# YaqiXia/Voltrix-SpMM

Hardware: AMD Instinct MI355X
Metric: spmm_gflops (higher is better)
Workload: dtype f16

## Files before the change

### include/voltrix_capi.h

```cpp
#ifndef VOLTRIX_CAPI_H_
#define VOLTRIX_CAPI_H_

#include <stdint.h>

#ifdef __cplusplus
extern "C" {
#endif

#define VOLTRIX_ABI_VERSION 2

#define VOLTRIX_CSR_AUTO (-1)
#define VOLTRIX_SLAB_AUTO (-1)
#define VOLTRIX_BLK_H 16
#define VOLTRIX_BLK_W 8

enum voltrix_rc {
  VOLTRIX_OK = 0,
  VOLTRIX_ERR_BAD_SHAPE = 1,
  VOLTRIX_ERR_LAUNCH = 2,
  VOLTRIX_ERR_BAD_CONFIG = 3,
  VOLTRIX_ERR_OVERFLOW = 4,
  VOLTRIX_ERR_DUPLICATE = 5
};

// ... 18 lines not shown
                                  int embedding_dim, void* input, void* output, int fs, int depth, int waves,
                                  void* window_order, void* out_scale, void* stream, int* return_code);

void voltrix_launch_spmm_f16(void* blk_offsets, void* hspa_packed, void* hind, int num_nodes, int num_edges,
                             int embedding_dim, void* input, void* output, void* stream, int* return_code);
void voltrix_launch_spmm_f16_tile(void* blk_offsets, void* hspa_packed, void* hind, int num_nodes, int num_edges,
                                  int embedding_dim, void* input, void* output, int fs, int depth, int waves,
                                  void* window_order, void* out_scale, void* stream, int* return_code);

int64_t voltrix_spmm_f32_workspace_bytes(int64_t input_rows, int embedding_dim);
void voltrix_launch_spmm_f32_as_f16(void* blk_offsets, void* hspa_packed, void* hind, int num_nodes, int num_edges,
                                    int embedding_dim, void* input, int64_t input_rows, void* output, void* workspace,
                                    void* stream, int* return_code);

void voltrix_launch_spmm_bf16(void* blk_offsets, void* hspa_packed, void* hind, int num_nodes, int num_edges,
                              int embedding_dim, void* input, void* output, void* stream, int* return_code);
void voltrix_launch_spmm_bf16_tile(void* blk_offsets, void* hspa_packed, void* hind, int num_nodes, int num_edges,
                                   int embedding_dim, void* input, void* output, int fs, int depth, int waves,
                                   void* window_order, void* out_scale, void* stream, int* return_code);

void voltrix_launch_spmm_f16_sched(void* blk_offsets, void* hspa_packed, void* hind, int num_nodes, int num_edges,
                                   int embedding_dim, void* input, void* output, int fs, int depth, int waves,
                                   void* window_order, void* out_scale, int atomic_out, void* units, void* unit_ptr,
                                   int max_units_per_xcd, void* partials, void* row_map, int units_per_wave, void* stream,
                                   int* return_code);
void voltrix_launch_spmm_bf16_sched(void* blk_offsets, void* hspa_packed, void* hind, int num_nodes, int num_edges,
                                    int embedding_dim, void* input, void* output, int fs, int depth, int waves,
                                    void* window_order, void* out_scale, int atomic_out, void* units, void* unit_ptr,
                                    int max_units_per_xcd, void* partials, void* row_map, int units_per_wave, void* stream,
                                    int* return_code);
void voltrix_launch_combine_partials(void* cuts, int num_cuts, void* partials, void* output, int num_nodes,
                                     int embedding_dim, int accumulate, void* row_map, void* stream, int* return_code);

int64_t voltrix_unit_table_workspace_bytes(int num_nodes);
int64_t voltrix_unit_table_fill_workspace_bytes(int64_t num_units);
void voltrix_launch_unit_table_count(void* blk_offsets, int num_nodes, int max_stages, void* xcd_ptr, void* workspace,
                                     void* header, void* stream, int* return_code);
void voltrix_launch_unit_table_fill(void* blk_offsets, int num_nodes, void* xcd_ptr, void* workspace, void* fill_workspace,
                                    int num_units, int num_cuts, int top, void* units, void* unit_ptr, void* cuts,
                                    void* stream, int* return_code);

int64_t voltrix_stream_table_workspace_bytes(int num_nodes);
int64_t voltrix_stream_table_fill_workspace_bytes(int64_t num_units);
void voltrix_launch_stream_table_count(void* blk_offsets, void* hspa_packed, void* hind, int num_nodes, int run_cost,
                                       int cut_stages, void* workspace, void* header, void* stream, int* return_code);
void voltrix_launch_stream_table_fill(void* blk_offsets, int num_nodes, void* workspace, void* fill_workspace, int num_units,
                                      int num_cuts, int run_bound, int run_cost, void* units, void* cuts, void* runs,
                                      void* run_ptr, void* header2, void* stream, int* return_code);
void voltrix_launch_spmm_stream_f16(void* hspa_packed, void* hind, int num_nodes, int embedding_dim, void* input,
                                    int64_t input_rows, void* output, void* units, void* runs, void* run_ptr,
                                    int max_runs_per_xcd, void* partials, void* out_scale, int fs, int depth, int waves,
                                    int slab_policy, void* stream, int* return_code);
void voltrix_launch_spmm_stream_bf16(void* hspa_packed, void* hind, int num_nodes, int embedding_dim, void* input,
                                     int64_t input_rows, void* output, void* units, void* runs, void* run_ptr,
                                     int max_runs_per_xcd, void* partials, void* out_scale, int fs, int depth, int waves,
                                     int slab_policy, void* stream, int* return_code);

void voltrix_launch_window_order(void* blk_offsets, int num_nodes, int chunk, void* order_out, void* stream,
                                 int* return_code);

#define VOLTRIX_PANEL_KSTEPS_PIPELINED 17
void voltrix_launch_spmm_panel_f16(void* panel_ptr, void* panel_cols, void* panel_bits, void* panel_order, void* xcd_ptr,
                                   int max_panels_per_xcd, int num_nodes, int embedding_dim, void* input, int64_t input_rows, void* output,
                                   int accumulate, int fs, int depth, int waves, int row_blocks, int ksteps,
                                   int slab_policy, void* out_scale, void* stream, int* return_code);
void voltrix_launch_spmm_panel_bf16(void* panel_ptr, void* panel_cols, void* panel_bits, void* panel_order, void* xcd_ptr,
                                    int max_panels_per_xcd, int num_nodes, int embedding_dim, void* input, int64_t input_rows, void* output,
                                    int accumulate, int fs, int depth, int waves, int row_blocks, int ksteps,
                                    int slab_policy, void* out_scale, void* stream, int* return_code);

void voltrix_launch_spmm_panel_parts_f16(void* panel_ptr, void* panel_cols, void* panel_bits, void* parts, int num_parts,
                                         void* xcd_ptr, int max_parts_per_xcd, void* partials, int num_nodes, int embedding_dim,
                                         void* input, int64_t input_rows, void* output, int accumulate, int fs, int depth,
                                         int waves, int row_blocks, int ksteps, int slab_policy, void* out_scale, void* stream,
                                         int* return_code);
void voltrix_launch_spmm_panel_parts_bf16(void* panel_ptr, void* panel_cols, void* panel_bits, void* parts, int num_parts,
                                          void* xcd_ptr, int max_parts_per_xcd, void* partials, int num_nodes, int embedding_dim,
                                          void* input, int64_t input_rows, void* output, int accumulate, int fs, int depth,
                                          int waves, int row_blocks, int ksteps, int slab_policy, void* out_scale, void* stream,
                                          int* return_code);
void voltrix_launch_combine_panel_partials(void* cuts, int num_cuts, void* partials, void* output, int num_nodes,
                                           int embedding_dim, int panel_rows, int accumulate, void* stream, int* return_code);

void voltrix_launch_xcd_ranges_of_work(void* work, int num_items, int align, void* xcd_ptr, void* stream, int* return_code);
void voltrix_launch_xcd_ranges_of_windows(void* blk_offsets, int num_nodes, int align, void* xcd_ptr, void* stream,
                                          int* return_code);
void voltrix_launch_xcd_ranges_of_panels(void* panel_ptr, void* resid_blk_offsets, int num_nodes, int panel_rows,
                                         int kstep_cost_x10, void* xcd_ptr, void* window_xcd_ptr, void* stream,
                                         int* return_code);
int64_t voltrix_panel_parts_workspace_bytes(int num_panels);
void voltrix_launch_panel_parts_count(void* panel_ptr, int num_panels, int cap, void* panel_xcd_ptr, void* workspace,
                                      void* header, void* stream, int* return_code);
void voltrix_launch_panel_parts_fill(void* panel_ptr, int num_panels, int cap, void* panel_xcd_ptr, void* workspace,
                                     void* parts, void* part_xcd_ptr, void* cuts, void* stream, int* return_code);

void voltrix_launch_spmm_fused_f16(void* panel_ptr, void* panel_cols, void* panel_bits, void* panel_order, void* xcd_ptr,
                                   int max_panels_per_xcd, void* wave_ptr, void* records, int num_nodes, int embedding_dim, void* input,
                                   void* output, int fs, int depth, int pace_blocks, void* out_scale, void* stream,
                                   int* return_code);
void voltrix_launch_spmm_fused_bf16(void* panel_ptr, void* panel_cols, void* panel_bits, void* panel_order, void* xcd_ptr,
                                    int max_panels_per_xcd, void* wave_ptr, void* records, int num_nodes, int embedding_dim, void* input,
                                    void* output, int fs, int depth, int pace_blocks, void* out_scale, void* stream,
                                   int* return_code);

void voltrix_fused_panel_geometry(int* waves, int* row_blocks);
int64_t voltrix_fused_records_workspace_bytes(int num_nodes);
void voltrix_launch_fused_records_count(void* blk_offsets, void* hspa_packed, int num_nodes, void* workspace, void* wave_ptr,
                                        void* stream, int* return_code);
void voltrix_launch_fused_records_fill(void* blk_offsets, void* hspa_packed, void* hind, int num_nodes, void* wave_ptr,
                                       int64_t num_records, void* records, void* stream, int* return_code);

int64_t voltrix_panel_plan_workspace_bytes(int num_nodes, int waves, int row_blocks);
void voltrix_launch_panel_plan_count(void* node_pointer, void* edge_list, int num_nodes, int num_cols, int64_t num_edges,
                                     int waves, int row_blocks, int tau, void* workspace, void* panel_ptr,
                                     void* resid_node_pointer, void* status, void* stream, int* return_code);
void voltrix_launch_panel_plan_fill(void* node_pointer, void* edge_list, int num_nodes, int num_cols, int64_t num_edges,
                                    int waves, int row_blocks, int tau, void* workspace, void* panel_ptr,
                                    void* resid_node_pointer, int64_t total_ksteps, void* resid_edge_list,
                                    void* panel_cols, void* panel_bits, void* stream, int* return_code);

void voltrix_launch_panel_order(void* panel_ptr, int num_panels, int group, void* xcd_ptr, void* order_out, void* stream,
                                int* return_code);

void voltrix_spmm_default_tile(int embedding_dim, int is_f16, int* fs, int* depth, int* waves);

int voltrix_spmm_num_tiles(int is_f16);
void voltrix_spmm_tile_at(int is_f16, int index, int* fs, int* depth, int* waves);

void voltrix_launch_cast_f32_f16(void* src, void* dst, int64_t count, void* stream, int* return_code);

void voltrix_launch_cast_f32_f16_scaled(void* src, void* dst, int64_t count, void* scale, void* stream,
                                        int* return_code);

void voltrix_launch_spmm_csr_rows(void* indptr, void* indices, int num_rows, int embedding_dim, void* input, int dtype, void* output,
                                  int xcd_ranges, void* stream, int* return_code);

void voltrix_launch_spmm_csr_rows_weighted(void* indptr, void* indices, void* values, int num_rows, int embedding_dim, void* input, int dtype,
                                           void* output, int xcd_ranges, void* stream, int* return_code);

void voltrix_launch_scatter_values(void* values, void* slots, void* plane, int64_t count, int dtype, void* stream, int* return_code);

void voltrix_launch_sddmm_csr(void* indptr, void* indices, int num_rows, int64_t nnz, int embedding_dim, void* x, int x_dtype, void* y,
                              int y_dtype, void* out, void* stream, int* return_code);

int64_t voltrix_edge_softmax_workspace_bytes(int num_rows, int64_t nnz);
void voltrix_launch_edge_softmax_csr(void* indptr, int num_rows, int64_t nnz, void* scores, float scale, void* out, void* workspace,
                                     void* stream, int* return_code);

void voltrix_launch_edge_softmax_backward_csr(void* indptr, int num_rows, int64_t nnz, void* alpha, void* grad_alpha, float scale,
                                              void* grad_scores, void* workspace, void* stream, int* return_code);

void voltrix_launch_sddmm_heads_csr(void* indptr, void* indices, int num_rows, int64_t nnz, int heads, int head_dim, void* x, int x_dtype,
                                    void* y, int y_dtype, void* out, void* stream, int* return_code);

int64_t voltrix_edge_softmax_heads_workspace_bytes(int num_rows, int64_t nnz, int heads);
void voltrix_launch_edge_softmax_heads_csr(void* indptr, int num_rows, int64_t nnz, int heads, void* scores, float scale, void* out,
                                           void* workspace, void* stream, int* return_code);
void voltrix_launch_edge_softmax_heads_backward_csr(void* indptr, int num_rows, int64_t nnz, int heads, void* alpha, void* grad_alpha,
                                                    float scale, void* grad_scores, void* workspace, void* stream, int* return_code);

void voltrix_launch_spmm_csr_heads(void* indptr, void* indices, void* values, int num_rows, int heads, int head_dim, void* input,
                                   int dtype, void* output, void* stream, int* return_code);

void voltrix_launch_gat_score_csr(void* indptr, void* indices, int num_rows, int64_t nnz, int heads, void* el, void* er, float slope,
                                  void* out, void* stream, int* return_code);

// ... 99 lines not shown
```

### voltrix-spmm_amd/csrc/capi_common.hpp

```cpp
#pragma once

#include <hip/hip_runtime.h>

#include "voltrix/spmm_kernels.hpp"
#include "voltrix_capi.h"

namespace voltrix_capi {

template <int FS, int D, int W, int EB>
constexpr bool tile_ok() {
  const int stage = 32 * FS * EB;
  const int wave_lds = D * stage + (2 * D + 1) * 256;
  return (long long)W * wave_lds <= 160 * 1024 && (1 + stage / 1024) * (D - 1) <= 63 && !(EB == 4 && FS == 256);
}

struct TileId {
  int fs, depth, waves;
};

#define VOLTRIX_TILE_SPACE(X)                                                                          \
  X(32, 2, 1) X(32, 2, 2) X(32, 2, 4) X(32, 3, 1) X(32, 3, 2) X(32, 3, 4) X(32, 4, 1) X(32, 4, 2) X(32, 4, 4)       \
  X(64, 2, 1) X(64, 2, 2) X(64, 2, 4) X(64, 3, 1) X(64, 3, 2) X(64, 3, 4) X(64, 4, 1) X(64, 4, 2) X(64, 4, 4)       \
  X(128, 2, 1) X(128, 2, 2) X(128, 2, 4) X(128, 3, 1) X(128, 3, 2) X(128, 3, 4) X(128, 4, 1) X(128, 4, 2) X(128, 4, 4) \
  X(256, 2, 1) X(256, 2, 2) X(256, 2, 4) X(256, 3, 1) X(256, 3, 2) X(256, 3, 4) X(256, 4, 1) X(256, 4, 2) X(256, 4, 4) \
  X(32, 2, 8) X(32, 3, 8) X(32, 4, 8) X(64, 2, 8) X(64, 3, 8) X(64, 4, 8) X(128, 2, 8) X(128, 3, 8) X(128, 4, 8)

template <int EB>
inline int num_tiles() {
  int n = 0;
#define X(FS, D, W) n += tile_ok<FS, D, W, EB>() ? 1 : 0;
  VOLTRIX_TILE_SPACE(X)
#undef X
  return n;
}

template <int EB>
inline bool tile_at(int index, TileId* out) {
  int n = 0;
#define X(FS, D, W)                      \
  if (tile_ok<FS, D, W, EB>()) {         \
    if (n == index) {                    \
      *out = TileId{FS, D, W};           \
      return true;                       \
    }                                    \
    ++n;                                 \
  }
  VOLTRIX_TILE_SPACE(X)
#undef X
  return false;
}

template <int FS, int D, int W, int EB, class In, bool BF16 = false>
inline int launch_if_ok(const int* blk_offsets, const uint32_t* hspa_packed, const int* hind, int num_nodes,
                        int embedding_dim, const In* input, float* output, hipStream_t stream, const int* order,
                        const float* out_scale, int atomic_out, const int* units, const int* unit_ptr,
                        int max_units_per_xcd, float* partials, const int* row_map, int units_per_wave) {
  if constexpr (tile_ok<FS, D, W, EB>()) {
    return voltrix::launch_spmm_tc16<voltrix::SpmmTile<FS, D, W, EB, BF16>>(blk_offsets, hspa_packed, hind, num_nodes,
                                                                       embedding_dim, input, output, stream, order,
                                                                       out_scale, atomic_out, units, unit_ptr,
                                                                       max_units_per_xcd, partials, row_map, nullptr,
                                                                       units_per_wave);
  } else {
    return voltrix::kErrBadConfig;
  }
}

template <int EB, class In, bool BF16 = false>
inline int dispatch_spmm(int fs, int depth, int waves, const int* blk_offsets, const uint32_t* hspa_packed,
                         const int* hind, int num_nodes, int embedding_dim, const In* input, float* output,
                         hipStream_t stream, const int* order, const float* out_scale = nullptr,
                         int atomic_out = 0, const int* units = nullptr, const int* unit_ptr = nullptr,
                         int max_units_per_xcd = 0, float* partials = nullptr, const int* row_map = nullptr,
                         int units_per_wave = 1) {
#define X(FS, D, W)                                  \
  if (fs == FS && depth == D && waves == W)          \
    return launch_if_ok<FS, D, W, EB, In, BF16>(blk_offsets, hspa_packed, hind, num_nodes, embedding_dim, input, output, stream, order, out_scale, atomic_out, units, unit_ptr, max_units_per_xcd, partials, row_map, units_per_wave);
  VOLTRIX_TILE_SPACE(X)
#undef X
  return voltrix::kErrBadConfig;
}

inline TileId default_tile(int embedding_dim, bool is_f16) {
  TileId t;
  if (is_f16) {
    t.fs = embedding_dim <= 32 ? 32 : (embedding_dim <= 64 ? 64 : 128);
    t.depth = t.fs == 32 ? 4 : 3;
    t.waves = 4;
  } else {
    t.fs = embedding_dim <= 32 ? 32 : 64;
    t.depth = 3;
    t.waves = 1;
  }
  return t;
}

}
```

### voltrix-spmm_amd/csrc/capi_spmm_bf16.hip

```cpp
#include "capi_common.hpp"

using namespace voltrix_capi;

extern "C" {

void voltrix_launch_spmm_bf16_tile(void* blk_offsets, void* hspa_packed, void* hind, int num_nodes, int num_edges,
                                   int embedding_dim, void* input, void* output, int fs, int depth, int waves,
                                   void* window_order, void* out_scale, void* stream, int* return_code) {
  (void)num_edges;
  *return_code = dispatch_spmm<2, voltrix::bfloat16_bits, true>(
      fs, depth, waves, static_cast<const int*>(blk_offsets), static_cast<const uint32_t*>(hspa_packed),
      static_cast<const int*>(hind), num_nodes, embedding_dim, static_cast<const voltrix::bfloat16_bits*>(input),
      static_cast<float*>(output), static_cast<hipStream_t>(stream), static_cast<const int*>(window_order),
      static_cast<const float*>(out_scale));
}

void voltrix_launch_spmm_bf16_sched(void* blk_offsets, void* hspa_packed, void* hind, int num_nodes, int num_edges,
                                    int embedding_dim, void* input, void* output, int fs, int depth, int waves,
                                    void* window_order, void* out_scale, int atomic_out,
                                    void* units, void* unit_ptr, int max_units_per_xcd, void* partials, void* row_map,
                                   int units_per_wave, void* stream,
                                    int* return_code) {
  (void)num_edges;
  *return_code = dispatch_spmm<2, voltrix::bfloat16_bits, true>(
      fs, depth, waves, static_cast<const int*>(blk_offsets), static_cast<const uint32_t*>(hspa_packed),
      static_cast<const int*>(hind), num_nodes, embedding_dim, static_cast<const voltrix::bfloat16_bits*>(input),
      static_cast<float*>(output), static_cast<hipStream_t>(stream), static_cast<const int*>(window_order),
      static_cast<const float*>(out_scale), atomic_out,
                                            static_cast<const int*>(units), static_cast<const int*>(unit_ptr),
                                            max_units_per_xcd, static_cast<float*>(partials), static_cast<const int*>(row_map),
                                            units_per_wave);
}

void voltrix_launch_spmm_bf16(void* blk_offsets, void* hspa_packed, void* hind, int num_nodes, int num_edges,
                              int embedding_dim, void* input, void* output, void* stream, int* return_code) {
  const TileId t = default_tile(embedding_dim, true);
  voltrix_launch_spmm_bf16_tile(blk_offsets, hspa_packed, hind, num_nodes, num_edges, embedding_dim, input, output,
                                t.fs, t.depth, t.waves, nullptr, nullptr, stream, return_code);
}

}
```

### voltrix-spmm_amd/csrc/capi_spmm_f16.hip

```cpp
#include "capi_common.hpp"

using namespace voltrix_capi;

extern "C" {

void voltrix_launch_spmm_f16_tile(void* blk_offsets, void* hspa_packed, void* hind, int num_nodes, int num_edges,
                                  int embedding_dim, void* input, void* output, int fs, int depth, int waves,
                                  void* window_order, void* out_scale, void* stream, int* return_code) {
  (void)num_edges;
  *return_code = dispatch_spmm<2, _Float16>(fs, depth, waves, static_cast<const int*>(blk_offsets),
                                            static_cast<const uint32_t*>(hspa_packed), static_cast<const int*>(hind),
                                            num_nodes, embedding_dim, static_cast<const _Float16*>(input),
                                            static_cast<float*>(output), static_cast<hipStream_t>(stream),
                                            static_cast<const int*>(window_order),
                                            static_cast<const float*>(out_scale));
}

void voltrix_launch_spmm_f16_sched(void* blk_offsets, void* hspa_packed, void* hind, int num_nodes, int num_edges,
                                   int embedding_dim, void* input, void* output, int fs, int depth, int waves,
                                   void* window_order, void* out_scale, int atomic_out,
                                   void* units, void* unit_ptr, int max_units_per_xcd, void* partials, void* row_map,
                                   int units_per_wave, void* stream,
                                   int* return_code) {
  (void)num_edges;
  *return_code = dispatch_spmm<2, _Float16>(fs, depth, waves, static_cast<const int*>(blk_offsets),
                                            static_cast<const uint32_t*>(hspa_packed), static_cast<const int*>(hind),
                                            num_nodes, embedding_dim, static_cast<const _Float16*>(input),
                                            static_cast<float*>(output), static_cast<hipStream_t>(stream),
                                            static_cast<const int*>(window_order),
                                            static_cast<const float*>(out_scale), atomic_out,
                                            static_cast<const int*>(units), static_cast<const int*>(unit_ptr),
                                            max_units_per_xcd, static_cast<float*>(partials), static_cast<const int*>(row_map),
                                            units_per_wave);
}

void voltrix_launch_combine_partials(void* cuts, int num_cuts, void* partials, void* output, int num_nodes,
                                     int embedding_dim, int accumulate, void* row_map, void* stream, int* return_code) {
  *return_code = voltrix::combine_partials(static_cast<const int*>(cuts), num_cuts, static_cast<const float*>(partials),
                                           static_cast<float*>(output), num_nodes, embedding_dim, accumulate,
                                           static_cast<hipStream_t>(stream), static_cast<const int*>(row_map));
}

void voltrix_launch_spmm_f16(void* blk_offsets, void* hspa_packed, void* hind, int num_nodes, int num_edges,
                             int embedding_dim, void* input, void* output, void* stream, int* return_code) {
  const TileId t = default_tile(embedding_dim, true);
  voltrix_launch_spmm_f16_tile(blk_offsets, hspa_packed, hind, num_nodes, num_edges, embedding_dim, input, output, t.fs,
                               t.depth, t.waves, nullptr, nullptr, stream, return_code);
}

int64_t voltrix_spmm_f32_workspace_bytes(int64_t input_rows, int embedding_dim) {
  if (input_rows < 0 || embedding_dim < 0) return -1;
  return 16 + input_rows * (int64_t)embedding_dim * 2;
}

void voltrix_launch_spmm_f32_as_f16(void* blk_offsets, void* hspa_packed, void* hind, int num_nodes, int num_edges,
                                    int embedding_dim, void* input, int64_t input_rows, void* output, void* workspace,
                                    void* stream, int* return_code) {
  if (input_rows < 0 || workspace == nullptr || ((uintptr_t)workspace & 15) || embedding_dim % 8 != 0) {
    *return_code = voltrix::kErrBadShape;
    return;
  }
  float* const scale = static_cast<float*>(workspace);
  _Float16* const operand = reinterpret_cast<_Float16*>(static_cast<char*>(workspace) + 16);
  *return_code = voltrix::cast_f32_to_f16_scaled(static_cast<const float*>(input), operand,
                                                 input_rows * (int64_t)embedding_dim, scale,
                                                 static_cast<hipStream_t>(stream));
  if (*return_code != voltrix::kOk) return;
  const TileId t = default_tile(embedding_dim, true);
  voltrix_launch_spmm_f16_tile(blk_offsets, hspa_packed, hind, num_nodes, num_edges, embedding_dim, operand, output, t.fs,
                               t.depth, t.waves, nullptr, scale, stream, return_code);
}

void voltrix_launch_window_order(void* blk_offsets, int num_nodes, int chunk, void* order_out, void* stream,
                                 int* return_code) {
  *return_code = voltrix::launch_window_order(static_cast<const int*>(blk_offsets), num_nodes, chunk,
                                              static_cast<int*>(order_out), static_cast<hipStream_t>(stream));
}

void voltrix_launch_cast_f32_f16(void* src, void* dst, int64_t count, void* stream, int* return_code) {
  *return_code = voltrix::cast_f32_to_f16(static_cast<const float*>(src), static_cast<_Float16*>(dst), count,
                                          static_cast<hipStream_t>(stream));
}

void voltrix_launch_cast_f32_f16_scaled(void* src, void* dst, int64_t count, void* scale, void* stream,
                                        int* return_code) {
  *return_code = voltrix::cast_f32_to_f16_scaled(static_cast<const float*>(src), static_cast<_Float16*>(dst), count,
                                                 static_cast<float*>(scale), static_cast<hipStream_t>(stream));
}

void voltrix_launch_scale_rows(void* src, void* scale, void* dst, int64_t rows, int num_feats, int dtype, void* stream,
                               int* return_code) {
  *return_code = voltrix::scale_rows(src, static_cast<const float*>(scale), dst, rows, num_feats, dtype,
                                     static_cast<hipStream_t>(stream));
}

}

namespace voltrix_capi {
int num_tiles_f16() { return num_tiles<2>(); }
bool tile_at_f16(int i, TileId* t) { return tile_at<2>(i, t); }
}
```

### voltrix-spmm_amd/csrc/capi_spmm_panel.hip

```cpp
#include <hip/hip_runtime.h>

#include "voltrix/panel_plan.hpp"
#include "voltrix/spmm_panel_kernels.hpp"
#include "voltrix_capi.h"

namespace {

#define VOLTRIX_PANEL_SPACE(X)                                                                       \
  X(128, 3, 8, 4, 1) X(128, 4, 8, 4, 1) X(128, 6, 8, 4, 1) X(128, 8, 8, 4, 1) X(128, 4, 4, 4, 1) X(128, 6, 4, 4, 1) X(128, 8, 4, 4, 1) \
  X(128, 4, 8, 2, 1) X(128, 6, 8, 2, 1) X(128, 8, 8, 2, 1) X(128, 6, 4, 2, 1)                                    \
  X(64, 4, 4, 4, 1) X(64, 6, 4, 4, 1) X(64, 4, 8, 4, 2) X(64, 6, 8, 4, 2) X(64, 6, 4, 4, 2)                      \
  X(32, 4, 4, 4, 2) X(32, 6, 4, 4, 2) X(32, 6, 8, 4, 2) X(64, 6, 4, 2, 2) X(64, 6, 8, 2, 2) X(32, 6, 4, 2, 2) X(32, 6, 8, 2, 2) \
  X(128, 3, 4, 4, 1) X(128, 4, 4, 2, 1)

constexpr int kPipelined = 17;
static_assert(kPipelined == VOLTRIX_PANEL_KSTEPS_PIPELINED, "include/voltrix_capi.h");
#define VOLTRIX_PANEL_PIPE_SPACE(X) X(128, 3, 8, 4) X(128, 4, 8, 4) X(128, 4, 8, 2) X(128, 6, 8, 2) X(64, 4, 8, 4) X(64, 6, 8, 4)

template <bool BF16>
int dispatch(int fs, int depth, int waves, int rb, int ks, const int* panel_ptr, const int* panel_cols,
             const uint32_t* panel_bits, const int* panel_order, int num_nodes, int embedding_dim, const void* input,
             float* output, int accumulate, const float* out_scale, hipStream_t stream, int64_t input_rows,
             int slab_policy, const int* xcd_ptr, int max_panels_per_xcd, const int* parts = nullptr, int num_parts = 0,
             float* partials = nullptr) {
#define X(FS, D, W, RB, KS)                                                                                          \
  if (fs == FS && depth == D && waves == W && rb == RB && ks == KS)                                                  \
    return voltrix::launch_spmm_panel<voltrix::PanelTile<FS, D, W, RB, KS, BF16>>(                                   \
        panel_ptr, panel_cols, panel_bits, panel_order, num_nodes, embedding_dim, input, output, accumulate, out_scale, \
        stream, 0, 0, input_rows, slab_policy, xcd_ptr, max_panels_per_xcd, parts, num_parts, partials);
  VOLTRIX_PANEL_SPACE(X)
#undef X
#define X(FS, D, W, RB)                                                                                              \
  if (fs == FS && depth == D && waves == W && rb == RB && ks == kPipelined)                                           \
    return voltrix::launch_spmm_panel<voltrix::PanelTile<FS, D, W, RB, 1, BF16, true>>(                               \
        panel_ptr, panel_cols, panel_bits, panel_order, num_nodes, embedding_dim, input, output, accumulate, out_scale, \
        stream, 0, 0, input_rows, slab_policy, xcd_ptr, max_panels_per_xcd, parts, num_parts, partials);
  VOLTRIX_PANEL_PIPE_SPACE(X)
#undef X
  return voltrix::kErrBadConfig;
}

}

extern "C" {

void voltrix_launch_spmm_panel_f16(void* panel_ptr, void* panel_cols, void* panel_bits, void* panel_order, void* xcd_ptr,
                                   int max_panels_per_xcd, int num_nodes, int embedding_dim, void* input, int64_t input_rows, void* output,
                                   int accumulate, int fs, int depth, int waves, int row_blocks, int ksteps,
                                   int slab_policy, void* out_scale, void* stream, int* return_code) {
  *return_code = dispatch<false>(fs, depth, waves, row_blocks, ksteps, static_cast<const int*>(panel_ptr),
                                 static_cast<const int*>(panel_cols), static_cast<const uint32_t*>(panel_bits),
                                 static_cast<const int*>(panel_order), num_nodes, embedding_dim, input,
                                 static_cast<float*>(output), accumulate, static_cast<const float*>(out_scale),
                                 static_cast<hipStream_t>(stream), input_rows, slab_policy,
                                 static_cast<const int*>(xcd_ptr), max_panels_per_xcd);
}

void voltrix_launch_spmm_panel_bf16(void* panel_ptr, void* panel_cols, void* panel_bits, void* panel_order, void* xcd_ptr,
                                    int max_panels_per_xcd, int num_nodes, int embedding_dim, void* input, int64_t input_rows, void* output,
                                    int accumulate, int fs, int depth, int waves, int row_blocks, int ksteps,
                                    int slab_policy, void* out_scale, void* stream, int* return_code) {
  *return_code = dispatch<true>(fs, depth, waves, row_blocks, ksteps, static_cast<const int*>(panel_ptr),
                                static_cast<const int*>(panel_cols), static_cast<const uint32_t*>(panel_bits),
                                static_cast<const int*>(panel_order), num_nodes, embedding_dim, input,
                                static_cast<float*>(output), accumulate, static_cast<const float*>(out_scale),
                                static_cast<hipStream_t>(stream), input_rows, slab_policy,
                                static_cast<const int*>(xcd_ptr), max_panels_per_xcd);
}

void voltrix_launch_spmm_panel_parts_f16(void* panel_ptr, void* panel_cols, void* panel_bits, void* parts, int num_parts,
                                         void* xcd_ptr, int max_parts_per_xcd, void* partials, int num_nodes, int embedding_dim,
                                         void* input, int64_t input_rows, void* output, int accumulate, int fs, int depth,
                                         int waves, int row_blocks, int ksteps, int slab_policy, void* out_scale, void* stream,
                                         int* return_code) {
  *return_code = parts == nullptr ? voltrix::kErrBadShape
                                  : dispatch<false>(fs, depth, waves, row_blocks, ksteps, static_cast<const int*>(panel_ptr),
                                                    static_cast<const int*>(panel_cols), static_cast<const uint32_t*>(panel_bits),
                                                    nullptr, num_nodes, embedding_dim, input, static_cast<float*>(output),
                                                    accumulate, static_cast<const float*>(out_scale),
                                                    static_cast<hipStream_t>(stream), input_rows, slab_policy,
                                                    static_cast<const int*>(xcd_ptr), max_parts_per_xcd,
                                                    static_cast<const int*>(parts), num_parts, static_cast<float*>(partials));
}

void voltrix_launch_spmm_panel_parts_bf16(void* panel_ptr, void* panel_cols, void* panel_bits, void* parts, int num_parts,
                                          void* xcd_ptr, int max_parts_per_xcd, void* partials, int num_nodes, int embedding_dim,
                                          void* input, int64_t input_rows, void* output, int accumulate, int fs, int depth,
                                          int waves, int row_blocks, int ksteps, int slab_policy, void* out_scale, void* stream,
                                          int* return_code) {
  *return_code = parts == nullptr ? voltrix::kErrBadShape
                                  : dispatch<true>(fs, depth, waves, row_blocks, ksteps, static_cast<const int*>(panel_ptr),
                                                   static_cast<const int*>(panel_cols), static_cast<const uint32_t*>(panel_bits),
                                                   nullptr, num_nodes, embedding_dim, input, static_cast<float*>(output),
                                                   accumulate, static_cast<const float*>(out_scale),
                                                   static_cast<hipStream_t>(stream), input_rows, slab_policy,
                                                   static_cast<const int*>(xcd_ptr), max_parts_per_xcd,
                                                   static_cast<const int*>(parts), num_parts, static_cast<float*>(partials));
}

void voltrix_launch_combine_panel_partials(void* cuts, int num_cuts, void* partials, void* output, int num_nodes,
                                           int embedding_dim, int panel_rows, int accumulate, void* stream, int* return_code) {
  *return_code = voltrix::launch_combine_panel_partials(static_cast<const int*>(cuts), num_cuts,
                                                        static_cast<const float*>(partials), static_cast<float*>(output),
                                                        num_nodes, embedding_dim, panel_rows, accumulate,
                                                        static_cast<hipStream_t>(stream));
}

void voltrix_launch_panel_order(void* panel_ptr, int num_panels, int group, void* xcd_ptr, void* order_out, void* stream,
                                int* return_code) {
  *return_code = voltrix::panel_order(static_cast<const int*>(panel_ptr), num_panels, group, static_cast<int*>(order_out),
                                      static_cast<hipStream_t>(stream), static_cast<const int*>(xcd_ptr));
}

int64_t voltrix_panel_plan_workspace_bytes(int num_nodes, int waves, int row_blocks) {
  return voltrix::panel_plan_workspace_bytes(num_nodes, waves, row_blocks);
}

void voltrix_launch_panel_plan_count(void* node_pointer, void* edge_list, int num_nodes, int num_cols, int64_t num_edges,
                                     int waves, int row_blocks, int tau, void* workspace, void* panel_ptr,
                                     void* resid_node_pointer, void* status, void* stream, int* return_code) {
  *return_code = voltrix::panel_plan_count(static_cast<const int*>(node_pointer), static_cast<const int*>(edge_list),
                                           num_nodes, num_cols, num_edges, waves, row_blocks, tau, workspace,
                                           static_cast<int*>(panel_ptr), static_cast<int*>(resid_node_pointer),
                                           static_cast<int*>(status), static_cast<hipStream_t>(stream));
}

void voltrix_launch_panel_plan_fill(void* node_pointer, void* edge_list, int num_nodes, int num_cols, int64_t num_edges,
                                    int waves, int row_blocks, int tau, void* workspace, void* panel_ptr,
                                    void* resid_node_pointer, int64_t total_ksteps, void* resid_edge_list,
                                    void* panel_cols, void* panel_bits, void* stream, int* return_code) {
  *return_code = voltrix::panel_plan_fill(static_cast<const int*>(node_pointer), static_cast<const int*>(edge_list),
                                          num_nodes, num_cols, num_edges, waves, row_blocks, tau, workspace,
                                          static_cast<const int*>(panel_ptr), static_cast<const int*>(resid_node_pointer),
                                          total_ksteps, static_cast<int*>(resid_edge_list), static_cast<int*>(panel_cols),
                                          static_cast<uint32_t*>(panel_bits), static_cast<hipStream_t>(stream));
}

}
```

### voltrix-spmm_amd/voltrix/capi.py

```python
from __future__ import annotations

import ctypes
import os
import subprocess

_PKG = os.path.dirname(os.path.abspath(__file__))
_ROOT = os.path.dirname(_PKG)
LIB_PATH = os.path.join(_ROOT, "lib", "libvoltrix_hip.so")
CSRC_DIR = os.path.join(_ROOT, "csrc")

_lib = None

_P, _I, _L, _F, _D, _RC_P = ctypes.c_void_p, ctypes.c_int, ctypes.c_int64, ctypes.c_float, ctypes.c_double, ctypes.POINTER(ctypes.c_int)
_U32, _U64 = ctypes.c_uint32, ctypes.c_uint64
SIGNATURES = {
    "voltrix_abi_version": (_I, []),
    "voltrix_launch_preprocess": (None, [_P, _P, _I, _P, _P, _P, _P, _RC_P]),
    "voltrix_launch_hmat_gen": (None, [_P, _P, _P, _P, _P, _P, _I, _I, _I, _P, _P, _RC_P]),
    "voltrix_launch_hmat_packed_swizzle": (None, [_I, _P, _P, _P, _RC_P]),
    "voltrix_launch_spmm": (None, [_P, _P, _P, _I, _I, _I, _P, _P, _P, _RC_P]),
    "voltrix_launch_spmm_f32_tile": (None, [_P, _P, _P, _I, _I, _I, _P, _P, _I, _I, _I, _P, _P, _P, _RC_P]),
    "voltrix_launch_spmm_f16": (None, [_P, _P, _P, _I, _I, _I, _P, _P, _P, _RC_P]),
    "voltrix_launch_spmm_f16_tile": (None, [_P, _P, _P, _I, _I, _I, _P, _P, _I, _I, _I, _P, _P, _P, _RC_P]),
    "voltrix_spmm_f32_workspace_bytes": (_L, [_L, _I]),
    "voltrix_launch_spmm_f32_as_f16": (None, [_P, _P, _P, _I, _I, _I, _P, _L, _P, _P, _P, _RC_P]),
    "voltrix_launch_spmm_f16_sched": (None, [_P, _P, _P, _I, _I, _I, _P, _P, _I, _I, _I, _P, _P, _I, _P, _P, _I, _P, _P, _I, _P, _RC_P]),
    "voltrix_launch_spmm_bf16_sched": (None, [_P, _P, _P, _I, _I, _I, _P, _P, _I, _I, _I, _P, _P, _I, _P, _P, _I, _P, _P, _I, _P, _RC_P]),
    "voltrix_launch_combine_partials": (None, [_P, _I, _P, _P, _I, _I, _I, _P, _P, _RC_P]),
    "voltrix_stream_table_workspace_bytes": (_L, [_I]),
    "voltrix_stream_table_fill_workspace_bytes": (_L, [_L]),
    "voltrix_launch_stream_table_count": (None, [_P, _P, _P, _I, _I, _I, _P, _P, _P, _RC_P]),
    "voltrix_launch_stream_table_fill": (None, [_P, _I, _P, _P, _I, _I, _I, _I, _P, _P, _P, _P, _P, _P, _RC_P]),
    "voltrix_launch_spmm_stream_f16": (None, [_P, _P, _I, _I, _P, _L, _P, _P, _P, _P, _I, _P, _P, _I, _I, _I, _I, _P, _RC_P]),
    "voltrix_launch_spmm_stream_bf16": (None, [_P, _P, _I, _I, _P, _L, _P, _P, _P, _P, _I, _P, _P, _I, _I, _I, _I, _P, _RC_P]),
    "voltrix_launch_spmm_panel_f16": (None, [_P, _P, _P, _P, _P, _I, _I, _I, _P, _L, _P, _I, _I, _I, _I, _I, _I, _I, _P, _P, _RC_P]),
    "voltrix_launch_spmm_panel_bf16": (None, [_P, _P, _P, _P, _P, _I, _I, _I, _P, _L, _P, _I, _I, _I, _I, _I, _I, _I, _P, _P, _RC_P]),
    "voltrix_launch_spmm_panel_parts_f16": (None, [_P, _P, _P, _P, _I, _P, _I, _P, _I, _I, _P, _L, _P, _I, _I, _I, _I, _I, _I, _I, _P, _P, _RC_P]),
    "voltrix_launch_spmm_panel_parts_bf16": (None, [_P, _P, _P, _P, _I, _P, _I, _P, _I, _I, _P, _L, _P, _I, _I, _I, _I, _I, _I, _I, _P, _P, _RC_P]),
    "voltrix_launch_combine_panel_partials": (None, [_P, _I, _P, _P, _I, _I, _I, _I, _P, _RC_P]),
    "voltrix_launch_xcd_ranges_of_work": (None, [_P, _I, _I, _P, _P, _RC_P]),
    "voltrix_launch_xcd_ranges_of_windows": (None, [_P, _I, _I, _P, _P, _RC_P]),
    "voltrix_launch_xcd_ranges_of_panels": (None, [_P, _P, _I, _I, _I, _P, _P, _P, _RC_P]),
    "voltrix_panel_parts_workspace_bytes": (_L, [_I]),
    "voltrix_launch_panel_parts_count": (None, [_P, _I, _I, _P, _P, _P, _P, _RC_P]),
    "voltrix_launch_panel_parts_fill": (None, [_P, _I, _I, _P, _P, _P, _P, _P, _P, _RC_P]),
    "voltrix_launch_spmm_fused_f16": (None, [_P, _P, _P, _P, _P, _I, _P, _P, _I, _I, _P, _P, _I, _I, _I, _P, _P, _RC_P]),
    "voltrix_launch_spmm_fused_bf16": (None, [_P, _P, _P, _P, _P, _I, _P, _P, _I, _I, _P, _P, _I, _I, _I, _P, _P, _RC_P]),
    "voltrix_fused_panel_geometry": (None, [_RC_P, _RC_P]),
    "voltrix_fused_records_workspace_bytes": (_L, [_I]),
    "voltrix_launch_fused_records_count": (None, [_P, _P, _I, _P, _P, _P, _RC_P]),
    "voltrix_launch_fused_records_fill": (None, [_P, _P, _P, _I, _P, _L, _P, _P, _RC_P]),
    "voltrix_panel_plan_workspace_bytes": (_L, [_I, _I, _I]),
    "voltrix_launch_panel_plan_count": (None, [_P, _P, _I, _I, _L, _I, _I, _I, _P, _P, _P, _P, _P, _RC_P]),
    "voltrix_launch_panel_plan_fill": (None, [_P, _P, _I, _I, _L, _I, _I, _I, _P, _P, _P, _L, _P, _P, _P, _P, _RC_P]),
    "voltrix_launch_panel_order": (None, [_P, _I, _I, _P, _P, _P, _RC_P]),
    "voltrix_spmm_default_tile": (None, [_I, _I, _RC_P, _RC_P, _RC_P]),
    "voltrix_spmm_num_tiles": (_I, [_I]),
    "voltrix_spmm_tile_at": (None, [_I, _I, _RC_P, _RC_P, _RC_P]),
    "voltrix_launch_window_order": (None, [_P, _I, _I, _P, _P, _RC_P]),
    "voltrix_launch_spmm_bf16": (None, [_P, _P, _P, _I, _I, _I, _P, _P, _P, _RC_P]),
    "voltrix_launch_spmm_bf16_tile": (None, [_P, _P, _P, _I, _I, _I, _P, _P, _I, _I, _I, _P, _P, _P, _RC_P]),
    "voltrix_launch_cast_f32_f16": (None, [_P, _P, _L, _P, _RC_P]),
    "voltrix_launch_cast_f32_f16_scaled": (None, [_P, _P, _L, _P, _P, _RC_P]),
    "voltrix_launch_scale_rows": (None, [_P, _P, _P, _L, _I, _I, _P, _RC_P]),
    "voltrix_launch_spmm_csr_rows": (None, [_P, _P, _I, _I, _P, _I, _P, _I, _P, _RC_P]),
    "voltrix_launch_spmm_csr_rows_weighted": (None, [_P, _P, _P, _I, _I, _P, _I, _P, _I, _P, _RC_P]),
    "voltrix_launch_scatter_values": (None, [_P, _P, _P, _L, _I, _P, _RC_P]),
    "voltrix_launch_sddmm_csr": (None, [_P, _P, _I, _L, _I, _P, _I, _P, _I, _P, _P, _RC_P]),
    "voltrix_edge_softmax_workspace_bytes": (_L, [_I, _L]),
    "voltrix_launch_edge_softmax_csr": (None, [_P, _I, _L, _P, _F, _P, _P, _P, _RC_P]),
    "voltrix_launch_edge_softmax_backward_csr": (None, [_P, _I, _L, _P, _P, _F, _P, _P, _P, _RC_P]),
    "voltrix_launch_sddmm_heads_csr": (None, [_P, _P, _I, _L, _I, _I, _P, _I, _P, _I, _P, _P, _RC_P]),
    "voltrix_edge_softmax_heads_workspace_bytes": (_L, [_I, _L, _I]),
    "voltrix_launch_edge_softmax_heads_csr": (None, [_P, _I, _L, _I, _P, _F, _P, _P, _P, _RC_P]),
    "voltrix_launch_edge_softmax_heads_backward_csr": (None, [_P, _I, _L, _I, _P, _P, _F, _P, _P, _P, _RC_P]),
    "voltrix_launch_spmm_csr_heads": (None, [_P, _P, _P, _I, _I, _I, _P, _I, _P, _P, _RC_P]),
    "voltrix_launch_gat_score_csr": (None, [_P, _P, _I, _L, _I, _P, _P, _F, _P, _P, _RC_P]),
    "voltrix_gat_score_workspace_bytes": (_L, [_I, _L, _I]),
    "voltrix_launch_gat_score_rowsum_csr": (None, [_P, _P, _P, _I, _L, _I, _P, _P, _P, _F, _P, _P, _P, _RC_P]),
    "voltrix_launch_gatv2_score_csr": (None, [_P, _P, _I, _L, _I, _I, _P, _P, _I, _P, _F, _P, _P, _RC_P]),
    "voltrix_launch_gatv2_rowsum_csr": (None, [_P, _P, _P, _I, _L, _I, _I, _P, _P, _I, _P, _F, _P, _P, _RC_P]),
    "voltrix_launch_attn_aggregate_csr": (None, [_P, _P, _P, _I, _L, _I, _I, _P, _I, _F, _P, _P, _P, _P, _RC_P]),
    "voltrix_launch_attn_aggregate_grad_scores_csr": (None, [_P, _P, _I, _L, _I, _I, _P, _P, _I, _P, _P, _P, _P, _F, _P, _P, _RC_P]),
    "voltrix_launch_attn_aggregate_grad_feat_csr": (None, [_P, _P, _P, _I, _L, _I, _I, _P, _I, _P, _P, _P, _F, _P, _P, _RC_P]),
    "voltrix_launch_dropout_mask": (None, [_L, _I, _U32, _U64, _U64, _P, _P, _RC_P]),
    "voltrix_launch_attn_aggregate_dropout_csr": (None, [_P, _P, _P, _I, _L, _I, _I, _P, _I, _F, _P, _P, _P, _P, _F, _P, _RC_P]),
    "voltrix_launch_attn_aggregate_dropout_grad_scores_csr": (None, [_P, _P, _I, _L, _I, _I, _P, _P, _I, _P, _P, _P, _P, _F, _P, _P, _F, _P, _RC_P]),
    "voltrix_launch_attn_aggregate_dropout_grad_feat_csr": (None, [_P, _P, _P, _I, _L, _I, _I, _P, _I, _P, _P, _P, _F, _P, _P, _F, _P, _RC_P]),
    "voltrix_launch_spmm_csr_reduce": (None, [_P, _P, _I, _I, _P, _I, _I, _P, _P, _P, _RC_P]),
    "voltrix_launch_spmm_csr_reduce_backward": (None, [_P, _P, _P, _I, _L, _I, _P, _P, _P, _P, _RC_P]),
    "voltrix_launch_sample_neighbors": (None, [_P, _P, _I, _P, _I, _P, _L, _I, _I, _U64, _U64, _P, _P, _P, _RC_P]),
    "voltrix_launch_block_mark": (None, [_P, _L, _I, _P, _P, _RC_P]),
    "voltrix_launch_block_mark_seeds": (None, [_P, _I, _I, _P, _P, _RC_P]),
    "voltrix_launch_block_relabel": (None, [_P, _L, _P, _I, _P, _P, _I, _I, _P, _P, _P, _RC_P]),
    "voltrix_launch_subgraph_count": (None, [_P, _P, _I, _P, _I, _P, _I, _I, _P, _P, _RC_P]),
    "voltrix_launch_subgraph_fill": (None, [_P, _P, _I, _P, _I, _P, _I, _I, _P, _L, _P, _P, _P, _RC_P]),
    "voltrix_launch_random_walk": (None, [_P, _P, _I, _P, _I, _I, _U64, _U64, _P, _P, _I, _P, _RC_P]),
    "voltrix_launch_negative_sample": (None, [_P, _P, _I, _I, _L, _P, _I, _I, _I, _I, _I, _U64, _U64, _P, _P, _RC_P]),
    "voltrix_launch_edge_endpoints": (None, [_P, _P, _I, _L, _P, _I, _P, _P, _P, _RC_P]),
    "voltrix_csr_preprocess_workspace_bytes": (_L, [_I, _I, _L, _I]),
    "voltrix_launch_csr_window_count": (None, [_P, _P, _I, _I, _L, _I, _P, _P, _P, _P, _P, _RC_P]),
    "voltrix_launch_csr_fill": (None, [_P, _P, _I, _I, _L, _I, _P, _P, _P, _P, _P, _RC_P]),
    "voltrix_unit_table_workspace_bytes": (_L, [_I]),
    "voltrix_unit_table_fill_workspace_bytes": (_L, [_L]),
    "voltrix_launch_unit_table_count": (None, [_P, _I, _I, _P, _P, _P, _P, _RC_P]),
    "voltrix_launch_unit_table_fill": (None, [_P, _I, _P, _P, _P, _I, _I, _I, _P, _P, _P, _P, _RC_P]),
    "voltrix_csr_transpose_workspace_bytes": (_L, [_L]),
    "voltrix_launch_csr_transpose": (None, [_P, _P, _I, _I, _L, _P, _P, _P, _P, _RC_P]),
    "voltrix_launch_bfs_seed": (None, [_I, _I, _P, _P, _P, _P, _P, _RC_P]),
    "voltrix_launch_bfs_levels": (None, [_P, _P, _P, _P, _I, _I, _P, _P, _P, _P, _I, _P, _RC_P]),
    "voltrix_cm_rank_workspace_bytes": (_L, [_L]),
    "voltrix_launch_cm_rank": (None, [_P, _P, _P, _P, _I, _I, _P, _P, _P, _P, _P, _RC_P, _I, _I, _P, _P, _RC_P]),
    "voltrix_launch_chol_inv_transposed": (None, [_P, _I, _D, _P, _P, _RC_P]),
}
SYMBOLS = tuple(SIGNATURES)


def build(force: bool = False) -> str:
    cmd = ["make", "-s", "-C", CSRC_DIR, "-j4"]
    if force:
        subprocess.check_call(["make", "-s", "-C", CSRC_DIR, "clean"])
    subprocess.check_call(cmd)
# ... 62 lines not shown
    import torch

    global _CODES
    if _CODES is None:
        _CODES = {torch.float32: 0, torch.float16: 1, torch.bfloat16: 2}
    return _CODES[dtype]


def _timed(label: str):
    import functools
    import inspect

    def decorate(fn):
        stream_index = list(inspect.signature(fn).parameters).index("stream")

        @functools.wraps(fn)
        def wrapper(*args, **kwargs):
            from .utils import KernelTimer

            if KernelTimer.active is None:
                return fn(*args, **kwargs)
            stream = kwargs.get("stream")
            if stream is None and len(args) > stream_index:
                stream = args[stream_index]
            with KernelTimer.active.bracket(label, stream):
                return fn(*args, **kwargs)

        wrapper.timer_label, wrapper.stream_index = label, stream_index
        return wrapper

    return decorate


def default_tile(embedding_dim: int, is_f16: bool):
    fs, d, w = ctypes.c_int(), ctypes.c_int(), ctypes.c_int()
    lib().voltrix_spmm_default_tile(embedding_dim, int(is_f16), fs, d, w)
    return fs.value, d.value, w.value


def tiles(is_f16: bool):
    out = []
    for i in range(lib().voltrix_spmm_num_tiles(int(is_f16))):
        fs, d, w = ctypes.c_int(), ctypes.c_int(), ctypes.c_int()
        lib().voltrix_spmm_tile_at(int(is_f16), i, fs, d, w)
        out.append((fs.value, d.value, w.value))
    return out


CSR_PATHS = {None: -1, "auto": -1, "sort": 0, "bitmap": 1, "mixed": 2}
SLAB_AUTO, SLAB_ONE_GRID, SLAB_LAUNCHES = -1, 0, 1


def csr_preprocess_workspace_bytes(num_nodes: int, num_cols: int, num_edges: int, path=None) -> int:
    return int(lib().voltrix_csr_preprocess_workspace_bytes(num_nodes, num_cols, num_edges, CSR_PATHS[path]))


@_timed("csr_window_count")
def launch_csr_window_count(indptr, indices, num_nodes, num_cols, workspace, block_partition, pointer1, status,
                            stream, path=None) -> None:
    _checked("voltrix_launch_csr_window_count", indptr.data_ptr(), indices.data_ptr(), num_nodes, num_cols, indices.numel(),
             CSR_PATHS[path], workspace.data_ptr(), block_partition.data_ptr(), pointer1.data_ptr(), status.data_ptr(), stream)


@_timed("csr_fill")
def launch_csr_fill(indptr, indices, num_nodes, num_cols, workspace, pointer1, hspa_packed, hind, stream, path=None) -> None:
    _checked("voltrix_launch_csr_fill", indptr.data_ptr(), indices.data_ptr(), num_nodes, num_cols, indices.numel(), CSR_PATHS[path],
             workspace.data_ptr(), pointer1.data_ptr(), hspa_packed.data_ptr(), hind.data_ptr(), stream)


@_timed("spmm")
def launch_spmm(blk_offsets, hspa_packed, hind, num_nodes, num_edges, embedding_dim, input_ptr, output_ptr, is_f16,
                tile, stream, window_order=0, out_scale=0) -> int:
    if is_f16 == "bf16":
        name = "voltrix_launch_spmm_bf16_tile"
    else:
        name = "voltrix_launch_spmm_f16_tile" if is_f16 else "voltrix_launch_spmm_f32_tile"
    return _call(name, blk_offsets, hspa_packed, hind, num_nodes, num_edges, embedding_dim, input_ptr, output_ptr, tile[0], tile[1],
                 tile[2], window_order, out_scale, stream)


@_timed("spmm")
def launch_spmm_sched(blk_offsets, hspa_packed, hind, num_nodes, num_edges, embedding_dim, input_ptr, output_ptr, tile,
                      stream, window_order=0, out_scale=0, atomic_out=False, bf16=False, table=None, partials=0,
                      row_map=0, units_per_wave=1) -> int:
    units, unit_ptr, max_units = (table.units.data_ptr(), table.unit_ptr.data_ptr(), table.max_units_per_xcd) if table is not None \
        else (None, None, 0)
    return _call("voltrix_launch_spmm_bf16_sched" if bf16 else "voltrix_launch_spmm_f16_sched", blk_offsets, hspa_packed, hind,
                 num_nodes, num_edges, embedding_dim, input_ptr, output_ptr, tile[0], tile[1], tile[2], window_order, out_scale,
                 int(atomic_out), units, unit_ptr, max_units, partials, row_map, int(units_per_wave), stream)


@_timed("combine_partials")
def launch_combine_partials(table, partials_ptr, output_ptr, num_nodes, embedding_dim, accumulate, stream,
                            row_map=0) -> int:
    return _call("voltrix_launch_combine_partials", table.cuts.data_ptr(), table.num_cuts, partials_ptr, output_ptr, num_nodes,
                 embedding_dim, int(accumulate), row_map, stream)


def build_unit_table(blk_offsets, num_nodes: int, max_stages: int = 0, stream=None, xcd_ptr=None):
    import torch

    dev = blk_offsets.device
    stream = _stream_of(stream)
    workspace = torch.empty(max(16, int(lib().voltrix_unit_table_workspace_bytes(num_nodes))), dtype=torch.uint8, device=dev)
    header = torch.empty(8, dtype=torch.int32, device=dev)
    _checked("voltrix_launch_unit_table_count", blk_offsets.data_ptr(), num_nodes, int(max_stages), _opt(xcd_ptr),
             workspace.data_ptr(), header.data_ptr(), stream)
    head = [int(v) for v in header.tolist()]
    num_units, num_cuts, top = head[0], head[1], head[5]
    units = torch.empty((num_units, 4), dtype=torch.int32, device=dev)
    cuts = torch.empty((num_cuts, 4), dtype=torch.int32, device=dev)
    unit_ptr = torch.empty(9, dtype=torch.int32, device=dev)
    fill_ws = torch.empty(max(16, int(lib().voltrix_unit_table_fill_workspace_bytes(num_units))), dtype=torch.uint8, device=dev)
    _checked("voltrix_launch_unit_table_fill", blk_offsets.data_ptr(), num_nodes, _opt(xcd_ptr), workspace.data_ptr(),
             fill_ws.data_ptr(), num_units, num_cuts, top, units.data_ptr(), unit_ptr.data_ptr(), cuts.data_ptr(), stream)
    return units, unit_ptr, cuts, head


def build_stream_table(blk_offsets, hspa_packed, hind, num_nodes: int, run_cost: int = 0, cut_stages: int = 0, stream=None):
    import torch

    dev = blk_offsets.device
    stream = _stream_of(stream)
    workspace = torch.empty(max(16, int(lib().voltrix_stream_table_workspace_bytes(num_nodes))), dtype=torch.uint8, device=dev)
    header = torch.empty(8, dtype=torch.int32, device=dev)
    _checked("voltrix_launch_stream_table_count", blk_offsets.data_ptr(), hspa_packed.data_ptr(), hind.data_ptr(), num_nodes,
             int(run_cost), int(cut_stages), workspace.data_ptr(), header.data_ptr(), stream)
    num_units, num_cuts, num_slots, run_bound, rcost, cut = [int(v) for v in header.tolist()][:6]
    units = torch.empty((num_units, 8), dtype=torch.int32, device=dev)
    cuts = torch.empty((num_cuts, 4), dtype=torch.int32, device=dev)
    runs = torch.empty((max(1, run_bound), 4), dtype=torch.int32, device=dev)
    run_ptr = torch.empty(9, dtype=torch.int32, device=dev)
    header2 = torch.empty(4, dtype=torch.int32, device=dev)
    fill_ws = torch.empty(max(16, int(lib().voltrix_stream_table_fill_workspace_bytes(num_units))), dtype=torch.uint8, device=dev)
    _checked("voltrix_launch_stream_table_fill", blk_offsets.data_ptr(), num_nodes, workspace.data_ptr(), fill_ws.data_ptr(),
             num_units, num_cuts, run_bound, max(2, rcost), units.data_ptr(), cuts.data_ptr(), runs.data_ptr(), run_ptr.data_ptr(),
             header2.data_ptr(), stream)
    num_runs, max_runs, oversized = [int(v) for v in header2.tolist()][:3]
    assert oversized == 0, "stream table with a run of more than 64 units (run_cost > 128?): the kernel cannot walk it"
    return units, runs[:num_runs], run_ptr, cuts, (num_units, num_cuts, num_slots, num_runs, max_runs, rcost, cut)


def launch_spmm_stream(hspa_packed, hind, num_nodes: int, embedding_dim: int, feat, output, table, partials, out_scale=None,
                       tile=(0, 0, 0), stream=None, input_rows: int = 0, slab_policy: int = -1) -> int:
    import torch

    stream = _stream_of(stream)
    name = "voltrix_launch_spmm_stream_bf16" if feat.dtype == torch.bfloat16 else "voltrix_launch_spmm_stream_f16"
    from .utils import timed_launch

    with timed_launch("spmm_stream", stream):
        return _call(name, hspa_packed.data_ptr(), hind.data_ptr(), num_nodes, embedding_dim, feat.data_ptr(), int(input_rows),
                     output.data_ptr(), table.units.data_ptr(), table.runs.data_ptr(), table.run_ptr.data_ptr(),
                     table.max_runs_per_xcd, partials.data_ptr(), _opt(out_scale), tile[0], tile[1], tile[2], int(slab_policy), stream)


def xcd_ranges_of_work(work, align: int = 1, stream=None):
    import torch

    out = torch.empty(9, dtype=torch.int32, device=work.device)
    _checked("voltrix_launch_xcd_ranges_of_work", work.data_ptr(), work.numel(), int(align), out.data_ptr(), _stream_of(stream))
    return out


def xcd_ranges_of_windows(blk_offsets, num_nodes: int, align: int = 1, stream=None):
    import torch

    out = torch.empty(9, dtype=torch.int32, device=blk_offsets.device)
    _checked("voltrix_launch_xcd_ranges_of_windows", blk_offsets.data_ptr(), num_nodes, int(align), out.data_ptr(), _stream_of(stream))
    return out


def xcd_ranges_of_panels(panel_ptr, resid_blk_offsets, num_nodes: int, panel_rows: int, kstep_cost_x10: int, stream=None):
    import torch

    dev = panel_ptr.device
    out, out_w = torch.empty(9, dtype=torch.int32, device=dev), torch.empty(9, dtype=torch.int32, device=dev)
    _checked("voltrix_launch_xcd_ranges_of_panels", panel_ptr.data_ptr(), resid_blk_offsets.data_ptr(), num_nodes, panel_rows,
             int(kstep_cost_x10), out.data_ptr(), out_w.data_ptr(), _stream_of(stream))
    return out, out_w


def build_panel_parts(panel_ptr, cap: int, panel_xcd_ptr=None, stream=None):
    import torch

    dev = panel_ptr.device
    num_panels = panel_ptr.numel() - 1
    stream = _stream_of(stream)
    workspace = torch.empty(max(16, int(lib().voltrix_panel_parts_workspace_bytes(num_panels))), dtype=torch.uint8, device=dev)
    header = torch.empty(8, dtype=torch.int32, device=dev)
    _checked("voltrix_launch_panel_parts_count", panel_ptr.data_ptr(), num_panels, int(cap), _opt(panel_xcd_ptr), workspace.data_ptr(),
             header.data_ptr(), stream)
    head = [int(v) for v in header.tolist()]
    parts = torch.empty((head[0], 4), dtype=torch.int32, device=dev)
    cuts = torch.empty((max(1, head[1]), 4), dtype=torch.int32, device=dev)
    part_xcd_ptr = torch.empty(9, dtype=torch.int32, device=dev)
    _checked("voltrix_launch_panel_parts_fill", panel_ptr.data_ptr(), num_panels, int(cap), _opt(panel_xcd_ptr), workspace.data_ptr(),
             parts.data_ptr(), part_xcd_ptr.data_ptr(), cuts.data_ptr(), stream)
    return parts, part_xcd_ptr, cuts[:head[1]], head


def spmm_f32_workspace_bytes(input_rows: int, embedding_dim: int) -> int:
    return int(lib().voltrix_spmm_f32_workspace_bytes(input_rows, embedding_dim))


@_timed("spmm_f32_as_f16")
def launch_spmm_f32_as_f16(blk_offsets, hspa_packed, hind, num_nodes, num_edges, embedding_dim, feat, output, workspace,
                           stream) -> int:
    return _call("voltrix_launch_spmm_f32_as_f16", blk_offsets.data_ptr(), hspa_packed.data_ptr(), hind.data_ptr(), num_nodes,
                 num_edges, embedding_dim, feat.data_ptr(), feat.shape[0], output.data_ptr(), workspace.data_ptr(), stream)


@_timed("spmm_panel")
def launch_spmm_panel(plan, input_ptr, output_ptr, embedding_dim, accumulate, bf16, tile, out_scale, stream,
                      input_rows: int = 0, slab_policy: int = SLAB_AUTO, partials_ptr: int = 0) -> int:
    panel = (plan.panel_ptr.data_ptr(), plan.panel_cols.data_ptr(), plan.panel_bits.data_ptr())
    launch = (plan.num_nodes, embedding_dim, input_ptr, input_rows, output_ptr, int(accumulate), tile[0], tile[1], plan.waves,
              plan.row_blocks, tile[2], slab_policy, out_scale, stream)
    parts = getattr(plan, "parts", None)
    if parts is not None:
        return _call("voltrix_launch_spmm_panel_parts_bf16" if bf16 else "voltrix_launch_spmm_panel_parts_f16", *panel,
                     parts.parts.data_ptr(), parts.num_parts, parts.xcd_ptr.data_ptr(), parts.max_parts_per_xcd, partials_ptr, *launch)
    xcd_ptr = getattr(plan, "xcd_ptr", None)
    return _call("voltrix_launch_spmm_panel_bf16" if bf16 else "voltrix_launch_spmm_panel_f16", *panel, _opt(plan.panel_order),
                 _opt(xcd_ptr), plan.max_panels_per_xcd if xcd_ptr is not None else 0, *launch)


def launch_combine_panel_partials(parts, partials_ptr, output_ptr, num_nodes, embedding_dim, panel_rows, accumulate,
                                  stream) -> int:
    return _call("voltrix_launch_combine_panel_partials", parts.cuts.data_ptr(), parts.num_cuts, partials_ptr, output_ptr, num_nodes,
                 embedding_dim, panel_rows, int(accumulate), stream)


@_timed("spmm_fused")
def launch_spmm_fused(plan, fused, input_ptr, output_ptr, embedding_dim, bf16, tile, out_scale, stream,
                      pace_blocks: int = 0) -> int:
    xcd_ptr = getattr(plan, "xcd_ptr", None)
    return _call("voltrix_launch_spmm_fused_bf16" if bf16 else "voltrix_launch_spmm_fused_f16", plan.panel_ptr.data_ptr(),
                 plan.panel_cols.data_ptr(), plan.panel_bits.data_ptr(), _opt(plan.panel_order), _opt(xcd_ptr),
                 plan.max_panels_per_xcd if xcd_ptr is not None else 0, fused.wave_ptr.data_ptr(), fused.records.data_ptr(),
                 plan.num_nodes, embedding_dim, input_ptr, output_ptr, tile[0], tile[1], int(pace_blocks), out_scale, stream)


def fused_panel_geometry():
    waves, row_blocks = ctypes.c_int(0), ctypes.c_int(0)
    lib().voltrix_fused_panel_geometry(waves, row_blocks)
    assert waves.value * row_blocks.value * 16 == 512, (waves.value, row_blocks.value)
    return waves.value, row_blocks.value


def build_fused_records(blk_offsets, hspa_packed, hind, num_nodes: int, stream=None):
    import torch

    dev = blk_offsets.device
    stream = _stream_of(stream)
    num_waves = fused_panel_geometry()[0] * ((num_nodes + 511) // 512)
    workspace = torch.empty(max(16, int(lib().voltrix_fused_records_workspace_bytes(num_nodes))), dtype=torch.uint8, device=dev)
    wave_ptr = torch.empty(num_waves + 1, dtype=torch.int32, device=dev)
    _checked("voltrix_launch_fused_records_count", blk_offsets.data_ptr(), hspa_packed.data_ptr(), num_nodes, workspace.data_ptr(),
             wave_ptr.data_ptr(), stream)
    num_records = int(wave_ptr[-1])
    assert 0 <= num_records <= 4 * (hspa_packed.numel() // 16 + 1), num_records
    records = torch.empty((num_records + 1, 64), dtype=torch.int32, device=dev).view(torch.uint32)
    _checked("voltrix_launch_fused_records_fill", blk_offsets.data_ptr(), hspa_packed.data_ptr(), hind.data_ptr(), num_nodes,
             wave_ptr.data_ptr(), num_records, records.data_ptr(), stream)
    return wave_ptr, records, num_records


def launch_panel_order(panel_ptr, num_panels: int, order_out, stream, group: int = 1, xcd_ptr=None) -> None:
    _checked("voltrix_launch_panel_order", panel_ptr.data_ptr(), num_panels, group, _opt(xcd_ptr), order_out.data_ptr(), stream)


def panel_plan_workspace_bytes(num_nodes: int, waves: int, row_blocks: int) -> int:
    return int(lib().voltrix_panel_plan_workspace_bytes(num_nodes, waves, row_blocks))


def launch_panel_plan_count(indptr, indices, num_nodes, num_cols, waves, row_blocks, tau, workspace, panel_ptr,
                            resid_indptr, status, stream) -> int:
    return _call("voltrix_launch_panel_plan_count", indptr.data_ptr(), indices.data_ptr(), num_nodes, num_cols, indices.numel(), waves,
                 row_blocks, tau, workspace.data_ptr(), panel_ptr.data_ptr(), resid_indptr.data_ptr(), status.data_ptr(), stream)


def launch_panel_plan_fill(indptr, indices, num_nodes, num_cols, waves, row_blocks, tau, workspace, panel_ptr,
                           resid_indptr, total_ksteps, resid_indices, panel_cols, panel_bits, stream) -> None:
    _checked("voltrix_launch_panel_plan_fill", indptr.data_ptr(), indices.data_ptr(), num_nodes, num_cols, indices.numel(), waves,
             row_blocks, tau, workspace.data_ptr(), panel_ptr.data_ptr(), resid_indptr.data_ptr(), total_ksteps,
             resid_indices.data_ptr(), panel_cols.data_ptr(), panel_bits.data_ptr(), stream)


@_timed("window_order")
def launch_window_order(blk_offsets, num_nodes, order_out, stream, chunk: int = 256) -> None:
    _checked("voltrix_launch_window_order", blk_offsets.data_ptr(), num_nodes, chunk, order_out.data_ptr(), stream)


@_timed("cast_f32_f16")
def launch_cast_f32_f16(src, dst, stream) -> None:
    _checked("voltrix_launch_cast_f32_f16", src.data_ptr(), dst.data_ptr(), src.numel(), stream)


@_timed("cast_f32_f16_scaled")
def launch_cast_f32_f16_scaled(src, dst, scale, stream) -> None:
    _checked("voltrix_launch_cast_f32_f16_scaled", src.data_ptr(), dst.data_ptr(), src.numel(), scale.data_ptr(), stream)




@_timed("spmm_csr_rows")
def launch_spmm_csr_rows(indptr, indices, num_rows: int, feat, output, stream, xcd_ranges: int = 0, values=None) -> None:
    import torch

    assert indptr.dtype == torch.int32 and indices.dtype == torch.int32 and indptr.numel() == num_rows + 1
    assert feat.dim() == 2 and feat.is_contiguous() and output.is_contiguous() and output.dtype == torch.float32
# ... 477 lines not shown
```

### voltrix-spmm_amd/voltrix/hybrid.py

```python
from __future__ import annotations

import contextlib
import contextvars
import dataclasses
import os

import torch

from . import capi

DEFAULT_WAVES = 8
DEFAULT_ROW_BLOCKS = 4
DEFAULT_TAU = 3
KSTEP = 32
FUSED_WAVES = 4
FUSED_ROW_BLOCKS = 8


@dataclasses.dataclass
class PanelParts:
    parts: torch.Tensor
    cuts: torch.Tensor
    xcd_ptr: torch.Tensor
    max_parts_per_xcd: int
# ... 327 lines not shown
                     num_nodes=num_nodes, waves=waves, row_blocks=row_blocks, tau=tau, num_ksteps=total_ksteps,
                     num_shared_edges=indices.numel() - num_resid, num_resid_edges=num_resid)
    return resid_indptr, resid_indices, plan


def build_panel_plan_torch(indptr: torch.Tensor, indices: torch.Tensor, num_nodes: int, num_cols: int = None,
                           waves: int = DEFAULT_WAVES, row_blocks: int = DEFAULT_ROW_BLOCKS, tau: int = DEFAULT_TAU):
    assert indptr.device == indices.device and indptr.dtype == torch.int32 and indices.dtype == torch.int32
    assert waves in (4, 8) and row_blocks in (2, 4) and tau >= 1
    device = indptr.device
    num_cols = num_nodes if num_cols is None else int(num_cols)
    p = waves * row_blocks * 16
    num_panels = (num_nodes + p - 1) // p
    resid_indptr, resid_indices, pc, rp, inv = split_shared_columns(indptr, indices, num_nodes, num_cols, p, tau)

    su_panel = pc // num_cols
    su_col = pc % num_cols
    cnt = torch.bincount(su_panel, minlength=num_panels)
    nks = (cnt + KSTEP - 1) // KSTEP
    panel_ptr = torch.zeros(num_panels + 1, dtype=torch.int64, device=device)
    panel_ptr[1:] = torch.cumsum(nks, 0)
    total_ksteps = int(panel_ptr[-1].item())
    assert total_ksteps < 2 ** 26, "k-step offsets are int32 (x 32 columns)"
    col_start = torch.cumsum(cnt, 0) - cnt
    rank = torch.arange(pc.numel(), device=device, dtype=torch.int64) - col_start[su_panel]
    slot = (panel_ptr[su_panel] + rank // KSTEP) * KSTEP + rank % KSTEP

    panel_of_kstep = torch.repeat_interleave(torch.arange(num_panels, device=device), nks)
    first_col = torch.zeros(num_panels, dtype=torch.int64, device=device)
    has = cnt > 0
    first_col[has] = su_col[col_start[has]]
    panel_cols = torch.zeros(KSTEP * (total_ksteps + 2), dtype=torch.int64, device=device)
    panel_cols[:KSTEP * total_ksteps] = first_col[panel_of_kstep].repeat_interleave(KSTEP)
    panel_cols[slot] = su_col

    e_slot = slot[inv]
    k = e_slot % KSTEP
    v = rp // (16 * row_blocks)
    j = (rp % (16 * row_blocks)) // 16
    word = (e_slot // KSTEP) * (waves * 64) + v * 64 + (k // 8) * 16 + (rp % 16)
    bits = torch.zeros((total_ksteps + 1) * waves * 64, dtype=torch.int64, device=device)
    bits.index_add_(0, word, torch.ones_like(word) << (16 * (k % 2) + 4 * j + (k % 8) // 2))
    panel_bits = ((bits + 2 ** 31) % 2 ** 32 - 2 ** 31).to(torch.int32).view(torch.uint32)

    plan = PanelPlan(panel_ptr=panel_ptr.to(torch.int32), panel_cols=panel_cols.to(torch.int32), panel_bits=panel_bits,
                     panel_order=None, num_nodes=num_nodes, waves=waves, row_blocks=row_blocks, tau=tau,
                     num_ksteps=total_ksteps, num_shared_edges=int(rp.numel()),
                     num_resid_edges=int(resid_indices.numel()))
    return resid_indptr, resid_indices, plan


KSTEPS_PIPELINED = 17


def default_panel_tile(embedding_dim: int, waves: int, row_blocks: int = DEFAULT_ROW_BLOCKS):
    if embedding_dim <= 32:
        return (32, 6, 2)
    if embedding_dim <= 64:
        return (64, 6, 2)
    if waves == 8:
        return (128, 3, 1) if row_blocks == 4 else (128, 4, KSTEPS_PIPELINED)
    return (128, 4, 1)


PANEL_DOMINATED_RATIO = 2.0
PANEL_DOMINATED_ROW_BLOCKS = 2


def panel_dominated(plan: "PanelPlan") -> bool:
    resid_stages = max(1.0, plan.num_resid_edges / 32.0)
    return plan.num_ksteps * KSTEP_COST_IN_STAGES >= PANEL_DOMINATED_RATIO * resid_stages


_SIDE_STREAMS = {}


def side_stream(device) -> "torch.cuda.Stream":
    key = device.index if device.index is not None else torch.cuda.current_device()
    if key not in _SIDE_STREAMS:
        _SIDE_STREAMS[key] = torch.cuda.Stream(device=device)
    return _SIDE_STREAMS[key]


def run_two_level(plan: PanelPlan, operand: torch.Tensor, output: torch.Tensor, run_window, out_scale=None,
                  tile=None, concurrent: bool = True) -> None:
    def finish(pending):
        if pending is not None:
            pending.run()

    if plan.num_ksteps == 0:
        finish(run_window(False))
        return
    if not concurrent:
        finish(run_window(False))
        launch_panel(plan, operand, output, accumulate=1, out_scale=out_scale, tile=tile)
        return
    from .utils import timed_launch

    main = torch.cuda.current_stream()
    side = side_stream(operand.device)
    with timed_launch("zero_fill", main):
        output.zero_()
    fork = torch.cuda.Event()
    fork.record(main)
    side.wait_event(fork)
    pending_panel = launch_panel(plan, operand, output, accumulate=2, out_scale=out_scale, tile=tile,
                                 stream=side.cuda_stream, defer_combine=True)
    join = torch.cuda.Event()
    join.record(side)
    pending = run_window(True)
    main.wait_event(join)
    finish(pending)
    finish(pending_panel)


class PendingPanelCombine:

    def __init__(self, plan, partials, output, num_feats, accumulate):
        self.plan, self.partials, self.output, self.num_feats, self.accumulate = plan, partials, output, num_feats, accumulate

    def run(self, raw_stream: int = None):
        from .utils import timed_launch

        current = torch.cuda.current_stream()
        with timed_launch("combine_panel_partials", current) if raw_stream is None else contextlib.nullcontext():
            rc = capi.launch_combine_panel_partials(self.plan.parts, self.partials.data_ptr(), self.output.data_ptr(),
                                                    self.plan.num_nodes, self.num_feats, self.plan.panel_rows,
                                                    self.accumulate, current.cuda_stream if raw_stream is None else raw_stream)
        capi.check(rc, "voltrix_launch_combine_panel_partials")
        self.partials = None


def launch_panel(plan: PanelPlan, feat: torch.Tensor, output: torch.Tensor, accumulate, out_scale=None,
                 tile=None, stream=None, slab_policy: int = None, defer_combine: bool = False):
    assert feat.is_cuda and feat.is_contiguous() and feat.dtype in (torch.float16, torch.bfloat16)
    assert output.is_cuda and output.is_contiguous() and output.dtype == torch.float32
    f = feat.shape[1]
    assert output.shape == (plan.num_nodes, f)
    tile = tile or default_panel_tile(f, plan.waves, plan.row_blocks)
    assert tile is not None, f"no panel tile for F={f} with {plan.waves} waves"
    stream = torch.cuda.current_stream().cuda_stream if stream is None else stream
    if slab_policy is None:
        from .jit_kernels import spmm as _spmm_wrapper

        slab_policy = _spmm_wrapper.SLAB_POLICY
    parts = plan.parts
    partials = None
    if parts is not None and parts.num_slots > 0:
        partials = torch.empty(parts.num_slots * plan.panel_rows * f, dtype=torch.float32, device=feat.device)
    rc = capi.launch_spmm_panel(plan, feat.data_ptr(), output.data_ptr(), f, int(accumulate),
                                feat.dtype == torch.bfloat16, tile, out_scale.data_ptr() if out_scale is not None else 0,
                                stream, input_rows=feat.shape[0], slab_policy=slab_policy,
                                partials_ptr=partials.data_ptr() if partials is not None else 0)
    capi.check(rc, "voltrix_launch_spmm_panel")
    if partials is None:
        return None
    pending = PendingPanelCombine(plan, partials, output, f, 1 if int(accumulate) else 0)
    if defer_combine:
        return pending
    pending.run(None if stream == torch.cuda.current_stream().cuda_stream else stream)
    return None


def default_fused_tile(embedding_dim: int):
    if embedding_dim <= 32:
        return (32, 4)
    if embedding_dim <= 64:
        return (64, 4)
    return (128, 3)


FUSED_PACE_BLOCKS = 0


def fused_enabled() -> bool:
    return os.getenv("VOLTRIX_FUSED", "0") in ("1", "on")


def launch_fused(plan: PanelPlan, fused: FusedRecords, feat: torch.Tensor, output: torch.Tensor, out_scale=None,
                 tile=None, stream=None, pace_blocks: int = None) -> None:
    assert feat.is_cuda and feat.is_contiguous() and feat.dtype in (torch.float16, torch.bfloat16)
    assert output.is_cuda and output.is_contiguous() and output.dtype == torch.float32
    assert plan.waves == DEFAULT_WAVES and plan.row_blocks == DEFAULT_ROW_BLOCKS, "the fused kernel owns 8 x 4 x 16-row panels"
    f = feat.shape[1]
    assert output.shape == (plan.num_nodes, f)
    tile = tile or default_fused_tile(f)
    stream = torch.cuda.current_stream().cuda_stream if stream is None else stream
    pace_blocks = FUSED_PACE_BLOCKS if pace_blocks is None else pace_blocks
    rc = capi.launch_spmm_fused(plan, fused, feat.data_ptr(), output.data_ptr(), f, feat.dtype == torch.bfloat16, tile,
                                out_scale.data_ptr() if out_scale is not None else 0, stream, pace_blocks)
    capi.check(rc, "voltrix_launch_spmm_fused")


def min_shared_fraction() -> float:
    default = "0.38" if hybrid_mode() == "auto" else "0.2"
    return float(os.getenv("VOLTRIX_HYBRID_MIN_SHARE", default))


_MODE_OVERRIDE = contextvars.ContextVar("voltrix_hybrid_mode", default=None)


@contextlib.contextmanager
def mode_override(value: str):
    token = _MODE_OVERRIDE.set(value)
    try:
        yield
    finally:
        _MODE_OVERRIDE.reset(token)


def hybrid_mode() -> str:
    v = _MODE_OVERRIDE.get()
    v = os.getenv("VOLTRIX_HYBRID", "auto") if v is None else v
    if v in ("0", "", "off"):
        return "off"
    if v in ("1", "on"):
        return "on"
    return "tune" if v == "tune" else "auto"


AUTO_MIN_EDGES = 1 << 22
AUTO_MIN_MEAN_DEGREE = 64
AUTO_MIN_ROWS = 110_000


def handle_bytes(tensors) -> int:
    return int(sum(t.numel() * t.element_size() for t in tensors if isinstance(t, torch.Tensor)))


def two_level_bytes(two: "TwoLevelHandle") -> int:
    plan = two.plan
    total = handle_bytes((two.blk_offsets, two.hspa_packed, two.hind, plan.panel_ptr, plan.panel_cols, plan.panel_bits,
                          plan.panel_order))
    if two.fused is not None:
        total += two.fused.nbytes()
    return total
```

### voltrix-spmm_amd/voltrix/include/voltrix/spmm_kernels.hpp

```cpp
#pragma once

#include <hip/hip_runtime.h>

#include <cstdint>
#include <cstdlib>
#include <mutex>
#include <type_traits>
#include <utility>
#include <vector>

#include "voltrix/traits.hpp"

#ifndef VOLTRIX_DIAG
#define VOLTRIX_DIAG 0
#endif


namespace voltrix {

typedef _Float16 half8_t __attribute__((ext_vector_type(8)));
typedef __bf16 bf16x8_t __attribute__((ext_vector_type(8)));
typedef uint16_t bfloat16_bits;
typedef float float4_t __attribute__((ext_vector_type(4)));
typedef unsigned uint2_t __attribute__((ext_vector_type(2)));
// ... 85 lines not shown
               : [m] "s"(m)
               : "vcc", "scc", "memory");
  __builtin_amdgcn_sched_barrier(0);
}

__device__ __forceinline__ void wait_lgkmcnt0() {
  asm volatile("s_waitcnt lgkmcnt(0)" ::: "memory");
  __builtin_amdgcn_sched_barrier(0);
}
__device__ __forceinline__ unsigned lds_read_b32(unsigned addr) {
  unsigned v;
  asm volatile("ds_read_b32 %0, %1" : "=v"(v) : "v"(addr) : "memory");
  return v;
}
template <int OFF>
__device__ __forceinline__ unsigned lds_read_b32_off(unsigned addr) {
  unsigned v;
  asm volatile("ds_read_b32 %0, %1 offset:%2" : "=v"(v) : "v"(addr), "n"(OFF) : "memory");
  return v;
}
template <int STRIDE, int N, int... I>
__device__ __forceinline__ void lds_read_b32_strided(unsigned addr, int (&out)[N], std::integer_sequence<int, I...>) {
  ((out[I] = (int)lds_read_b32_off<STRIDE * I>(addr)), ...);
}
__device__ __forceinline__ uint2_t lds_read_b64(unsigned addr) {
  uint2_t v;
  asm volatile("ds_read_b64 %0, %1" : "=v"(v) : "v"(addr) : "memory");
  return v;
}
__device__ __forceinline__ uint4_t lds_read_b128(unsigned addr) {
  uint4_t v;
  asm volatile("ds_read_b128 %0, %1" : "=v"(v) : "v"(addr) : "memory");
  return v;
}
template <int OFF>
__device__ __forceinline__ uint2_t lds_read_tr16_b64(unsigned addr) {
  uint2_t v;
  asm volatile("ds_read_b64_tr_b16 %0, %1 offset:%2" : "=v"(v) : "v"(addr), "n"(OFF) : "memory");
  return v;
}
__device__ __forceinline__ void dma_b128(const void* src, unsigned lds_byte_addr) {
  __builtin_amdgcn_global_load_lds((gas_ptr)src, (lds_ptr)(uintptr_t)lds_byte_addr, 16, 0, 0);
}
__device__ __forceinline__ void dma_b32(const void* src, unsigned lds_byte_addr) {
  __builtin_amdgcn_global_load_lds((gas_ptr)src, (lds_ptr)(uintptr_t)lds_byte_addr, 4, 0, 0);
}
__device__ __forceinline__ void dma_b32_nt(const void* src, unsigned lds_byte_addr) {
  __builtin_amdgcn_global_load_lds((gas_ptr)src, (lds_ptr)(uintptr_t)lds_byte_addr, 4, 0, 2);
}
__device__ __forceinline__ void dma_b128_nt(const void* src, unsigned lds_byte_addr) {
  __builtin_amdgcn_global_load_lds((gas_ptr)src, (lds_ptr)(uintptr_t)lds_byte_addr, 16, 0, 2);
}

template <int SLOTS>
__device__ __forceinline__ constexpr int slot_swizzle(int r) {
  const int ident = (r & 3) | (((r >> 3) & 1) << 2);
  return SLOTS >= 8 ? ident : (SLOTS == 4 ? (ident >> 1) : (ident >> 2));
}

constexpr float kAScaleInv = 0.5f;
__device__ __forceinline__ half8_t nibbles_to_half8_x2(unsigned nl, unsigned nh) {
  unsigned zl, zh;
  asm("v_lshl_or_b32 %0, %1, 15, %1" : "=v"(zl) : "v"(nl));
  asm("v_lshl_or_b32 %0, %1, 15, %1" : "=v"(zh) : "v"(nh));
  uint4_t r;
  r[0] = (zl << 14) & 0x40004000u;
  r[1] = (zl << 12) & 0x40004000u;
  r[2] = (zh << 14) & 0x40004000u;
  r[3] = (zh << 12) & 0x40004000u;
  return __builtin_bit_cast(half8_t, r);
}

template <int OFF, int AUX = 0>
__device__ __forceinline__ void dma_b128_off(const void* src, unsigned lds_byte_addr) {
  __builtin_amdgcn_global_load_lds((gas_ptr)((const char*)src - OFF), (lds_ptr)(uintptr_t)lds_byte_addr, 16, OFF, AUX);
}

__device__ __forceinline__ float lds_read_f32(unsigned addr) {
  float v;
  asm volatile("ds_read_b32 %0, %1" : "=v"(v) : "v"(addr) : "memory");
  return v;
}

template <class Tag = void>
inline int ensure_dynamic_lds(const void* kernel, int bytes) {
  if (bytes <= 64 * 1024) return kOk;
  struct Seen { const void* k; int dev; };
  static std::mutex mu;
  static std::vector<Seen> seen;
  int dev = 0;
  if (hipGetDevice(&dev) != hipSuccess) return kErrLaunch;
  static thread_local Seen last = {nullptr, -1};
  if (last.k == kernel && last.dev == dev) return kOk;
  std::lock_guard<std::mutex> lock(mu);
  for (const Seen& s : seen)
    if (s.k == kernel && s.dev == dev) {
      last = s;
      return kOk;
    }
  if (hipFuncSetAttribute(kernel, hipFuncAttributeMaxDynamicSharedMemorySize, bytes) != hipSuccess) return kErrBadConfig;
  seen.push_back(Seen{kernel, dev});
  last = seen.back();
  return kOk;
}

template <class T>
struct SpmmArgs {
  using in_t = typename std::conditional<T::EB == 4, float,
                                         typename std::conditional<T::BF16, bfloat16_bits, _Float16>::type>::type;
  const int* blk_offsets;
  const uint32_t* hspa_packed;
  const int* hind;
  const in_t* input;
  float* output;
  int num_nodes;
  int num_windows;
  int F;
  int num_slabs;
  int windows_per_xcd;
  const int* window_order;
  const float* out_scale;
  const int4* units;
  const int* unit_ptr;
  float* partials;
  const in_t* values;
  const int* row_map;
  int slab_major;
  int slab_first;
  int meta_nt;
  int atomic_out;
};

template <int I, int N, class Fn>
__device__ __forceinline__ void static_for(Fn&& fn) {
  if constexpr (I < N) {
    fn(std::integral_constant<int, I>{});
    static_for<I + 1, N>(fn);
  }
}

template <class T, int NU>
__device__ __forceinline__ void spmm_tc16_body(const SpmmArgs<T>& a) {
  static_assert(NU == 1 || NU == 2, "units per wave");
  constexpr int FS = T::FS, D = T::DEPTH, MS = T::META_SLOTS, EB = T::EB;
  constexpr int ROW_BYTES = T::ROW_BYTES, STAGE_BYTES = T::STAGE_BYTES, NDMA = T::DMA_PER_STAGE;
  constexpr int RPD = T::ROWS_PER_DMA, LPR = T::LANES_PER_ROW, SLOTS = T::SLOTS;

  extern __shared__ __attribute__((aligned(16))) char smem[];
  const int lane = threadIdx.x & (kWave - 1);
  const int wave = __builtin_amdgcn_readfirstlane((int)(threadIdx.x / kWave));
  const unsigned long long diag_t0 = (VOLTRIX_DIAG & 8) ? __builtin_amdgcn_s_memrealtime() : 0ull;

  const int xcd = blockIdx.x % kNumXcd;
  int w_begin = xcd * a.windows_per_xcd;
  int w_count = (a.num_windows - w_begin) < a.windows_per_xcd ? (a.num_windows - w_begin) : a.windows_per_xcd;
  if (a.units) {
    w_begin = a.unit_ptr[xcd];
    w_count = a.unit_ptr[xcd + 1] - w_begin;
  }
  __builtin_amdgcn_s_setprio(3);
  const int wave_pos = (int)(blockIdx.x / kNumXcd) * T::WAVES + wave;
  const int pairs_per_slab = (w_count + 1) / 2;
  if (w_count <= 0 || (NU == 1 ? wave_pos >= w_count * a.num_slabs : wave_pos >= pairs_per_slab * a.num_slabs)) return;
  const int lu = NU == 1 ? wave_pos : (wave_pos / pairs_per_slab) * w_count + 2 * (wave_pos % pairs_per_slab);
  int w[NU], st0[NU], st_step[NU], slot[NU];
  int kb0[NU], kb1[NU], nst_u[NU], h_safe[NU];
  bool present[NU];
  int nst_max = 0;
#pragma unroll
  for (int p = 0; p < NU; ++p) {
    present[p] = NU == 1 || (lu % w_count) + p < w_count;
    const int lup = present[p] ? lu + p : lu;
    const int wpos = w_begin + ((a.slab_major || NU == 2) ? lup % w_count : lup / a.num_slabs);
    st0[p] = 0;
    st_step[p] = 1;
    slot[p] = -1;
    if (a.units) {
      const int4 u = a.units[wpos];
      w[p] = u.x;
      st0[p] = u.y;
      st_step[p] = u.z;
      slot[p] = u.w;
    } else {
      w[p] = a.window_order ? a.window_order[wpos] : wpos;
    }
    kb0[p] = a.blk_offsets[w[p]];
    kb1[p] = a.blk_offsets[w[p] + 1];
    const int nblk = kb1[p] - kb0[p];
    const int nst_window = (nblk + kTcbPerStage - 1) / kTcbPerStage;
    nst_u[p] = st0[p] < nst_window ? (nst_window - st0[p] + st_step[p] - 1) / st_step[p] : 0;
    if (nblk == 1) {
      const uint4 w4 = *reinterpret_cast<const uint4*>(a.hspa_packed + 4ll * kb0[p]);
      if ((w4.x | w4.y | w4.z | w4.w) == 0u) nst_u[p] = 0;
    }
    if (!present[p]) nst_u[p] = 0;
    h_safe[p] = a.hind[8ll * kb0[p]];
    nst_max = nst_u[p] > nst_max ? nst_u[p] : nst_max;
  }
  const int nst = NU * nst_max;
  const int fs0 = (a.slab_first + (int)((a.slab_major || NU == 2) ? lu / w_count : lu % a.num_slabs)) * FS;
  const int F = a.F;
  auto stage_of = [&](int t) -> int { return st0[t % NU] + st_step[t % NU] * (t / NU); };
  auto stage_block = [&](int t) -> int { return kb0[t % NU] + kTcbPerStage * stage_of(t); };
  auto stage_end = [&](int t) -> int { return kb1[t % NU]; };

  float4_t acc[NU][SLOTS];
#pragma unroll
  for (int p = 0; p < NU; ++p)
#pragma unroll
    for (int s = 0; s < SLOTS; ++s) acc[p][s] = float4_t{0.f, 0.f, 0.f, 0.f};

  const unsigned lds0 = (unsigned)(uintptr_t)(lds_ptr)smem + (unsigned)wave * T::WAVE_LDS;
  const unsigned meta0 = lds0 + D * STAGE_BYTES;

  if (nst > 0) {

    const int k32 = lane & 31;
    const int kblk = k32 >> 3, kcol = k32 & 7;
    const unsigned colmask = 0x11111111u << (kcol & 3);
    const unsigned vword_off = 128 + 4 * (4 * kblk + 2 * (kcol >> 2));
    const int g = lane >> 4, R = lane & 15;
    const unsigned a_shift = 4 * (R & 7);
// ... 208 lines not shown
          wlo[bm] = lds_read_b32(mt + 128 + 4 * (4 * bm + (R >> 3)));
          whi[bm] = lds_read_b32(mt + 128 + 4 * (4 * bm + 2 + (R >> 3)));
        }
        const int z = g & 1;
        const unsigned lbase = lds0 + dslot * STAGE_BYTES + g * ROW_BYTES + 4 * R;
        const unsigned base_e = lbase + 64 * z, base_o = lbase - 64 * z;
        float bv[8][SLOTS];
#pragma unroll
        for (int m = 0; m < 8; ++m) {
#pragma unroll
          for (int s = 0; s < SLOTS; ++s) {
            bv[m][s] = lds_read_f32(((s & 1) ? base_o : base_e) + (4 * m * ROW_BYTES + 64 * s));
          }
        }
        wait_lgkmcnt0();

        issue_meta(t + 2 * D, mslot_2d);
        if (more) {
          if (tail_stage) rows_from_columns(sanitise(t + D, hraw, vw), hr);
          issue_data(dslot, hr);
        }

#pragma unroll
        for (int m = 0; m < 8; ++m) {
          const int bm = m >> 1;
          unsigned word = (m & 1) ? whi[bm] : wlo[bm];
          if (stage_block(t) + bm >= kb1 || !live) word = 0u;
          const float av = ((word >> (a_shift + g)) & 1u) ? 1.0f : 0.0f;
#pragma unroll
          for (int s = 0; s < SLOTS; ++s) acc[P][s] = __builtin_amdgcn_mfma_f32_16x16x4f32(av, bv[m][s], acc[P][s], 0, 0, 0);
        }
      }

      dslot = dslot + 1 == D ? 0 : dslot + 1;
      mslot = mslot + 1 == MS ? 0 : mslot + 1;
      mslot_d = mslot_d + 1 == MS ? 0 : mslot_d + 1;
      mslot_2d = mslot_2d + 1 == MS ? 0 : mslot_2d + 1;
    };
    int t = 0;
    if constexpr (NU == 2) {
      for (; t + 1 < nst - D; t += 2) {
        wait_vmcnt<T::vm_behind(D - 1)>();
        step(t, std::true_type{}, std::integral_constant<int, 0>{});
        wait_vmcnt<T::vm_behind(D - 1)>();
        step(t + 1, std::true_type{}, std::integral_constant<int, 1>{});
      }
      if (t < nst - D) {
        wait_vmcnt<T::vm_behind(D - 1)>();
        step(t, std::true_type{}, std::integral_constant<int, 0>{});
      }
      static_for<0, D>([&](auto ic) {
        constexpr int I = decltype(ic)::value;
        if (nst - D + I >= 0) {
          wait_vmcnt<T::vm_behind(D - 1 - I)>();
          step(nst - D + I, std::false_type{}, std::integral_constant<int, (D + I) & 1>{});
        }
      });
    } else {
      for (; t < nst - D; ++t) {
        wait_vmcnt<T::vm_behind(D - 1)>();
        step(t, std::true_type{}, std::integral_constant<int, 0>{});
      }
      for (; t < nst; ++t) {
        switch (nst - 1 - t) {
          case 0: wait_vmcnt<T::vm_behind(0)>(); break;
          case 1: wait_vmcnt<T::vm_behind(1)>(); break;
          case 2: wait_vmcnt<T::vm_behind(2)>(); break;
          case 3: wait_vmcnt<T::vm_behind(3)>(); break;
          case 4: wait_vmcnt<T::vm_behind(4)>(); break;
          default: wait_vmcnt<T::vm_behind(D - 1)>(); break;
        }
        step(t, std::false_type{}, std::integral_constant<int, 0>{});
      }
    }
    wait_vmcnt<0>();
  }

  if (VOLTRIX_DIAG & 4) {
    if (acc[0][0][0] == 12345.678f) a.output[0] = acc[0][0][0];
    return;
  }
  const float oscale = ((EB == 2 && !T::WEIGHTED) ? kAScaleInv : 1.0f) * (a.out_scale ? *a.out_scale : 1.0f);
  const int ocol0 = fs0 + (lane & 15);
#pragma unroll
  for (int p = 0; p < NU; ++p) {
    if (!present[p]) continue;
    const bool dead = NU > 1 && nst_u[p] == 0;
    if (slot[p] >= 0) {
      float* const tile = a.partials + (long long)slot[p] * (kBlkH * (long long)F) + (long long)(4 * (lane >> 4)) * F;
#pragma unroll
      for (int s = 0; s < SLOTS; ++s) {
        const int col = ocol0 + 16 * s;
        if (col < F) {
#pragma unroll
          for (int j = 0; j < 4; ++j) tile[(long long)j * F + col] = dead ? 0.f : acc[p][s][j] * oscale;
        }
      }
      continue;
    }
    const int orow0 = w[p] * kBlkH + 4 * (lane >> 4);
    int orow[4];
#pragma unroll
    for (int j = 0; j < 4; ++j) {
      orow[j] = orow0 + j;
      if (a.row_map && !(VOLTRIX_DIAG & 8)) orow[j] = a.row_map[orow[j]];
      if (orow[j] >= a.num_nodes) orow[j] = -1;
    }
#pragma unroll
    for (int s = 0; s < SLOTS; ++s) {
      const int col = ocol0 + 16 * s;
      if (col < F) {
#pragma unroll
        for (int j = 0; j < 4; ++j) {
          const int row = orow[j];
          if (row >= 0) {
            float* const dst = a.output + ((long long)row * F + col);
            const float v = dead ? 0.f : acc[p][s][j] * oscale;
            if (a.atomic_out)
              unsafeAtomicAdd(dst, v);
            else
              *dst = v;
          }
        }
      }
    }
  }
  if ((VOLTRIX_DIAG & 8) && a.row_map && lane == 0) {
    int* const stamp = const_cast<int*>(a.row_map) + 4ll * ((long long)blockIdx.x * T::WAVES + wave);
    stamp[0] = (int)__builtin_amdgcn_s_getreg((31 << 11) | 20);
    stamp[1] = (int)__builtin_amdgcn_s_getreg((31 << 11) | 4);
    stamp[2] = (int)(unsigned)diag_t0;
    stamp[3] = (int)(unsigned)__builtin_amdgcn_s_memrealtime();
  }
}

template <class T>
static __global__ __launch_bounds__(T::THREADS) void spmm_tc16_kernel(const SpmmArgs<T> a) {
  spmm_tc16_body<T, 1>(a);
}

template <class T>
static __global__ __launch_bounds__(T::THREADS) __attribute__((amdgpu_num_vgpr(160)))
void spmm_tc16_pair_kernel(const SpmmArgs<T> a) {
  spmm_tc16_body<T, 2>(a);
}

inline int slab_major_order(int num_slabs, int slab_row_bytes) { return num_slabs > 1 && slab_row_bytes >= 128; }

enum SlabPolicy : int { kSlabAuto = -1, kSlabOneGrid = 0, kSlabLaunches = 1 };
inline int slab_launch_group(int num_slabs, int slab_row_bytes, long long rows, int policy = kSlabAuto) {
  if (policy == kSlabOneGrid || slab_row_bytes < 128) return 0;
  if (policy == kSlabAuto && rows * 256 > (256ll << 20)) return 0;
  const int group = slab_row_bytes >= 256 ? 1 : 256 / slab_row_bytes;
  return num_slabs > group ? group : 0;
}

template <class T>
inline int launch_spmm_tc16(const int* blk_offsets, const uint32_t* hspa_packed, const int* hind, int num_nodes,
                            int embedding_dim, const void* input ,
                            float* output, hipStream_t stream, const int* window_order = nullptr,
                            const float* out_scale = nullptr, int atomic_out = 0,
                            const int* units = nullptr , const int* unit_ptr = nullptr ,
                            int max_units_per_xcd = 0, float* partials = nullptr, const int* row_map = nullptr,
                            const void* values = nullptr ,
                            int units_per_wave = 1 ,
                            int slab_first = 0, int slab_count = 0 ,
                            long long input_rows = 0 ,
                            int slab_policy = kSlabAuto) {
  if (num_nodes < 0 || embedding_dim < 0) return kErrBadShape;
  if (num_nodes == 0 || embedding_dim == 0) return kOk;
  if (embedding_dim % (16 / T::EB) != 0) return kErrBadShape;
  if (((uintptr_t)input & 15) || ((uintptr_t)hspa_packed & 15)) return kErrBadShape;
  SpmmArgs<T> a;
  a.blk_offsets = blk_offsets;
  a.hspa_packed = hspa_packed;
  a.hind = hind;
  a.input = static_cast<const typename SpmmArgs<T>::in_t*>(input);
  a.output = output;
  a.num_nodes = num_nodes;
  a.num_windows = (num_nodes + kBlkH - 1) / kBlkH;
  a.F = embedding_dim;
  const int total_slabs = (embedding_dim + T::FS - 1) / T::FS;
  if (slab_first < 0 || slab_count < 0 || slab_first + slab_count > total_slabs) return kErrBadShape;
  if (const int group = slab_count == 0 ? slab_launch_group(total_slabs, T::FS * T::EB,
                                                            input_rows > 0 ? input_rows : (long long)num_nodes, slab_policy)
                                        : 0) {
    for (int s = 0; s < total_slabs; s += group) {
      const int rc = launch_spmm_tc16<T>(blk_offsets, hspa_packed, hind, num_nodes, embedding_dim, input, output, stream,
                                         window_order, out_scale, atomic_out, units, unit_ptr, max_units_per_xcd, partials,
                                         row_map, values, units_per_wave, s, total_slabs - s < group ? total_slabs - s : group);
      if (rc != kOk) return rc;
    }
    return kOk;
  }
  a.slab_first = slab_count > 0 ? slab_first : 0;
  a.num_slabs = slab_count > 0 ? slab_count : total_slabs;
  a.windows_per_xcd = (a.num_windows + kNumXcd - 1) / kNumXcd;
  a.window_order = window_order;
  a.out_scale = out_scale;
  a.atomic_out = atomic_out;
  a.meta_nt = total_slabs == 1;
  a.slab_major = slab_major_order(a.num_slabs, T::FS * T::EB);
  a.units = reinterpret_cast<const int4*>(units);
  a.unit_ptr = unit_ptr;
  a.partials = partials;
  a.row_map = row_map;
  a.values = static_cast<const typename SpmmArgs<T>::in_t*>(values);
  if (T::WEIGHTED && (values == nullptr || ((uintptr_t)values & 15))) return kErrBadShape;
  if (units != nullptr) {
    if (unit_ptr == nullptr || max_units_per_xcd < 0 || ((uintptr_t)units & 15)) return kErrBadShape;
    if (max_units_per_xcd == 0) return kOk;
    a.windows_per_xcd = max_units_per_xcd;
  }
  if ((long long)a.windows_per_xcd * a.num_slabs > 0x3FFFFFFFll) return kErrBadShape;
  if constexpr (T::EB == 2 && !T::WEIGHTED && T::FS <= 128) {
    if (units_per_wave == 2 && units != nullptr && (a.num_slabs == 1 || a.slab_major)) {
      const long long pairs = ((long long)a.windows_per_xcd + 1) / 2 * a.num_slabs;
      const long long blocks_per_xcd = (pairs + T::WAVES - 1) / T::WAVES;
      const long long grid = blocks_per_xcd * kNumXcd;
      if (grid > 0x7FFFFFFFll) return kErrBadShape;
      const int lds_rc = ensure_dynamic_lds(reinterpret_cast<const void*>(&spmm_tc16_pair_kernel<T>), T::BLOCK_LDS);
      if (lds_rc != kOk) return lds_rc;
      hipLaunchKernelGGL(spmm_tc16_pair_kernel<T>, dim3((unsigned)grid), dim3(T::THREADS), T::BLOCK_LDS, stream, a);
      return hipGetLastError() == hipSuccess ? kOk : kErrLaunch;
    }
  }
  const long long blocks_per_xcd = ((long long)a.windows_per_xcd * a.num_slabs + T::WAVES - 1) / T::WAVES;
  const long long grid = blocks_per_xcd * kNumXcd;
  if (grid > 0x7FFFFFFFll) return kErrBadShape;
  const int lds_rc = ensure_dynamic_lds(reinterpret_cast<const void*>(&spmm_tc16_kernel<T>), T::BLOCK_LDS);
  if (lds_rc != kOk) return lds_rc;
  hipLaunchKernelGGL(spmm_tc16_kernel<T>, dim3((unsigned)grid), dim3(T::THREADS), T::BLOCK_LDS, stream, a);
  return hipGetLastError() == hipSuccess ? kOk : kErrLaunch;
}

static __global__ __launch_bounds__(256) void combine_partials_kernel(const int4* __restrict__ cuts,
                                                                     const float* __restrict__ partials,
                                                                     float* __restrict__ output, const int num_nodes,
                                                                     const int F, const int accumulate,
                                                                     const int* __restrict__ row_map) {
  const int4 c = cuts[blockIdx.x];
  const int f4 = F / 4;
  const long long tile4 = (long long)kBlkH * f4;
  const float4* src = reinterpret_cast<const float4*>(partials) + (long long)c.y * tile4;
  for (int i = threadIdx.x; i < (int)tile4; i += 256) {
    int row = c.x * kBlkH + i / f4;
    if (row_map) row = row_map[row];
    if (row < 0 || row >= num_nodes) continue;
    float4 sum = src[i];
    int u = 1;
    for (; u + 8 <= c.z; u += 8) {
      float4 p[8];
#pragma unroll
      for (int k = 0; k < 8; ++k) p[k] = src[(long long)(u + k) * tile4 + i];
#pragma unroll
      for (int k = 0; k < 8; ++k) {
        sum.x += p[k].x;
        sum.y += p[k].y;
        sum.z += p[k].z;
        sum.w += p[k].w;
      }
    }
    for (; u < c.z; ++u) {
      const float4 p = src[(long long)u * tile4 + i];
      sum.x += p.x;
      sum.y += p.y;
      sum.z += p.z;
      sum.w += p.w;
    }
    float4* const dst = reinterpret_cast<float4*>(output + (long long)row * F) + (i % f4);
    if (accumulate) {
      const float4 d = *dst;
      sum.x += d.x;
      sum.y += d.y;
      sum.z += d.z;
      sum.w += d.w;
    }
    *dst = sum;
  }
}

inline int combine_partials(const int* cuts, int num_cuts, const float* partials, float* output, int num_nodes,
                            int embedding_dim, int accumulate, hipStream_t stream, const int* row_map = nullptr) {
  if (num_cuts < 0 || num_nodes < 0 || embedding_dim < 0 || (embedding_dim % 4) != 0) return kErrBadShape;
  if (num_cuts == 0 || num_nodes == 0 || embedding_dim == 0) return kOk;
  if (((uintptr_t)cuts & 15) || ((uintptr_t)partials & 15) || ((uintptr_t)output & 15)) return kErrBadShape;
  hipLaunchKernelGGL(combine_partials_kernel, dim3((unsigned)num_cuts), dim3(256), 0, stream,
                     reinterpret_cast<const int4*>(cuts), partials, output, num_nodes, embedding_dim, accumulate, row_map);
  return hipGetLastError() == hipSuccess ? kOk : kErrLaunch;
}

constexpr int kOrderMaxChunk = 4096;

static __global__ __launch_bounds__(256) void window_order_kernel(const int* __restrict__ blk_offsets,
                                                                 const int num_windows, const int windows_per_xcd,
                                                                 const int chunk, const int chunks_per_xcd,
                                                                 int* __restrict__ order) {
  __shared__ unsigned long long keys[kOrderMaxChunk];
  const int xcd = blockIdx.x / chunks_per_xcd, c = blockIdx.x % chunks_per_xcd;
  const int x_begin = xcd * windows_per_xcd;
  const int x_end = (x_begin + windows_per_xcd < num_windows) ? x_begin + windows_per_xcd : num_windows;
  const int begin = x_begin + c * chunk;
  const int end = (begin + chunk < x_end) ? begin + chunk : x_end;
  const int n = end - begin;
  if (n <= 0) return;
  int P = 1;
  while (P < n) P <<= 1;
  for (int i = threadIdx.x; i < P; i += 256) {
    unsigned long long k = ~0ull;
    if (i < n) {
      const unsigned nblk = (unsigned)(blk_offsets[begin + i + 1] - blk_offsets[begin + i]);
      k = ((unsigned long long)(0xFFFFFFFFu - nblk) << 32) | (unsigned)i;
    }
    keys[i] = k;
  }
  __syncthreads();
  for (int k = 2; k <= P; k <<= 1) {
    for (int j = k >> 1; j > 0; j >>= 1) {
      for (int i = threadIdx.x; i < P; i += 256) {
        const int l = i ^ j;
        if (l > i) {
          const unsigned long long x = keys[i], y = keys[l];
          const bool up = (i & k) == 0;
          if ((x > y) == up) {
            keys[i] = y;
            keys[l] = x;
          }
        }
      }
      __syncthreads();
    }
  }
  for (int i = threadIdx.x; i < n; i += 256) order[begin + i] = begin + (int)(keys[i] & 0xFFFFFFFFu);
}

inline int launch_window_order(const int* blk_offsets, int num_nodes, int chunk, int* order, hipStream_t stream) {
  if (num_nodes < 0 || chunk < 1 || chunk > kOrderMaxChunk) return kErrBadShape;
  const int num_windows = (num_nodes + kBlkH - 1) / kBlkH;
  if (num_windows == 0) return kOk;
  const int windows_per_xcd = (num_windows + kNumXcd - 1) / kNumXcd;
  const int chunks_per_xcd = (windows_per_xcd + chunk - 1) / chunk;
  hipLaunchKernelGGL(window_order_kernel, dim3(kNumXcd * chunks_per_xcd), dim3(256), 0, stream, blk_offsets, num_windows,
                     windows_per_xcd, chunk, chunks_per_xcd, order);
  return hipGetLastError() == hipSuccess ? kOk : kErrLaunch;
}

static __global__ __launch_bounds__(256) void cast_f32_to_f16_kernel(const float* __restrict__ src, _Float16* __restrict__ dst,
                                                              const long long n8) {
  typedef _Float16 h8 __attribute__((ext_vector_type(8)));
  const long long stride = (long long)gridDim.x * blockDim.x;
  for (long long i = (long long)blockIdx.x * blockDim.x + threadIdx.x; i < n8; i += stride) {
    const float4 x = reinterpret_cast<const float4*>(src)[2 * i];
    const float4 y = reinterpret_cast<const float4*>(src)[2 * i + 1];
    h8 o = {(_Float16)x.x, (_Float16)x.y, (_Float16)x.z, (_Float16)x.w,
            (_Float16)y.x, (_Float16)y.y, (_Float16)y.z, (_Float16)y.w};
    reinterpret_cast<h8*>(dst)[i] = o;
  }
}

inline int cast_f32_to_f16(const float* src, _Float16* dst, long long n, hipStream_t stream) {
  if (n < 0 || (n % 8) != 0 || ((uintptr_t)src & 15) || ((uintptr_t)dst & 15)) return kErrBadShape;
  if (n == 0) return kOk;
  const long long n8 = n / 8;
  const int blocks = (int)(n8 / 256 + 1 < 256 * 16 ? n8 / 256 + 1 : 256 * 16);
  hipLaunchKernelGGL(cast_f32_to_f16_kernel, dim3(blocks), dim3(256), 0, stream, src, dst, n8);
  return hipGetLastError() == hipSuccess ? kOk : kErrLaunch;
}

template <typename T, int V>
static __global__ __launch_bounds__(256) void scale_rows_kernel(const T* __restrict__ src, const float* __restrict__ scale,
                                                                T* __restrict__ dst, const long long chunks, const int chunks_per_row) {
// ... 140 lines not shown
```

### voltrix-spmm_amd/voltrix/include/voltrix/spmm_panel_kernels.hpp

```cpp
#pragma once

#include <hip/hip_runtime.h>

#include <cstdint>
#include <type_traits>

#include "voltrix/spmm_kernels.hpp"

#ifndef VOLTRIX_PANEL_DIAG
#define VOLTRIX_PANEL_DIAG 0
#endif
namespace voltrix {


template <int FS_, int DEPTH_, int WAVES_, int RB_, int KS_ = 1, bool BF16_ = false, bool PIPE_ = false>
struct PanelTile {
  static constexpr int FS = FS_, DEPTH = DEPTH_, WAVES = WAVES_, RB = RB_, KS = KS_;
  static constexpr bool BF16 = BF16_, PIPE = PIPE_;
  static_assert(!PIPE || (KS == 1 && FS >= 32), "pipelined loop: one k-step per ring slot");
  static_assert(FS == 32 || FS == 64 || FS == 128, "feature slab");
  static_assert(RB >= 1 && RB <= 4, "a lane's adjacency word holds four row blocks");
  static_assert(KS == 1 || KS == 2, "one index DMA covers 64 columns");
  static_assert(DEPTH >= 3 && DEPTH <= 8, "ring depth");
  static constexpr int PANEL_ROWS = WAVES * RB * 16;
  static constexpr int THREADS = WAVES * kWave;
  static constexpr int ROW_BYTES = FS * 2;
  static constexpr int KSTEP_BYTES = kStageK * ROW_BYTES;
  static constexpr int STAGE_BYTES = KS * KSTEP_BYTES;
  static constexpr int NDMA = STAGE_BYTES / 1024;
  static_assert(NDMA % WAVES == 0 || WAVES % NDMA == 0, "row DMAs per step vs waves");
  static constexpr int DPW = NDMA >= WAVES ? NDMA / WAVES : 1;
  static constexpr int ROWS_PER_DMA = 1024 / ROW_BYTES;
  static constexpr int LANES_PER_ROW = ROW_BYTES / 16;
  static constexpr int SLOTS = FS / 16;
  static constexpr int BITS_BYTES = KS * WAVES * 256;
  static constexpr int META_BYTES = BITS_BYTES + 256;
  static constexpr int META_SLOTS = PIPE ? 2 * DEPTH : 2 * DEPTH - 1;
  static constexpr int NBITS_DMA = BITS_BYTES / 1024;
  static_assert(BITS_BYTES % 1024 == 0 && NBITS_DMA + 1 <= WAVES, "metadata DMA roles");
  static constexpr int VM_PER_STEP = DPW + 1;
  static constexpr int VM_PER_STEP_PLAIN = DPW;
  static constexpr int DATA_LDS = DEPTH * STAGE_BYTES;
  static constexpr int BLOCK_LDS = DATA_LDS + META_SLOTS * META_BYTES;
  static_assert(BLOCK_LDS <= 160 * 1024, "LDS per CU");
  static_assert(VM_PER_STEP * (DEPTH - 2) <= 63, "vmcnt is a 6-bit counter on gfx9");
};

__device__ __forceinline__ half8_t adjacency_to_half8_x2(unsigned w, int p0) {
  uint4_t r;
#pragma unroll
  for (int i = 0; i < 4; ++i) {
    const int p = p0 + i;
    r[i] = (p <= 14 ? (w << (14 - p)) : (w >> (p - 14))) & 0x40004000u;
  }
  return __builtin_bit_cast(half8_t, r);
}

template <class T>
struct PanelArgs {
  using in_t = typename std::conditional<T::BF16, bfloat16_bits, _Float16>::type;
  const int* panel_ptr;
  const int* panel_cols;
  const uint32_t* panel_bits;
  const int* panel_order;
  const int* xcd_ptr;
  const int* parts;
  float* partials;
  const in_t* input;
  float* output;
  const float* out_scale;
  int num_nodes;
  int num_panels;
  int panels_per_xcd;
  int F;
  int meta_nt;
  int slab_first;
  int accumulate;
};

template <class T>
static __global__ __launch_bounds__(T::THREADS) void spmm_panel_kernel(const PanelArgs<T> a) {
  constexpr int FS = T::FS, D = T::DEPTH, MS = T::META_SLOTS, KS = T::KS, RB = T::RB;
  constexpr int ROW_BYTES = T::ROW_BYTES, STAGE_BYTES = T::STAGE_BYTES, DPW = T::DPW;
  constexpr int RPD = T::ROWS_PER_DMA, LPR = T::LANES_PER_ROW, SLOTS = T::SLOTS;

  extern __shared__ __attribute__((aligned(16))) char smem[];
  const int wave = __builtin_amdgcn_readfirstlane((int)(threadIdx.x / kWave));

  const int xcd = blockIdx.x % kNumXcd;
  const int pos = (a.xcd_ptr ? a.xcd_ptr[xcd] : xcd * a.panels_per_xcd) + (int)(blockIdx.x / kNumXcd);
  const int pos_end = a.xcd_ptr ? a.xcd_ptr[xcd + 1]
                                : ((xcd + 1) * a.panels_per_xcd < a.num_panels ? (xcd + 1) * a.panels_per_xcd : a.num_panels);
  if (pos >= pos_end) return;
  int panel, ks0, nks, slot = -1;
  if (a.parts) {
    const int4_t part = *reinterpret_cast<const int4_t*>(a.parts + 4 * (long long)pos);
    panel = part[0];
    ks0 = a.panel_ptr[panel] + part[1];
    nks = part[2];
    slot = part[3];
  } else {
    panel = a.panel_order ? a.panel_order[pos] : pos;
    ks0 = a.panel_ptr[panel];
    nks = a.panel_ptr[panel + 1] - ks0;
  }
  const int fs0 = (a.slab_first + blockIdx.y) * FS;
  const int F = a.F;
  const int lane = threadIdx.x & (kWave - 1);

  const int ngroups = (nks + KS - 1) / KS;
  if (ngroups == 0 && a.accumulate && slot < 0) return;

  float4_t acc[RB][SLOTS];
#pragma unroll
  for (int j = 0; j < RB; ++j)
#pragma unroll
    for (int s = 0; s < SLOTS; ++s) acc[j][s] = float4_t{0.f, 0.f, 0.f, 0.f};

  const unsigned data0 = (unsigned)(uintptr_t)(lds_ptr)smem;
  const unsigned meta0 = data0 + T::DATA_LDS;
  const bool meta_wave = wave <= T::NBITS_DMA;

  if (ngroups > 0) {
    const unsigned row_bytes = (unsigned)F * 2u;
    const int dma0 = (wave * DPW) % T::NDMA;
    const char* cbase[DPW];
    unsigned hr_off[DPW];
#pragma unroll
    for (int d = 0; d < DPW; ++d) {
      const int r = (dma0 + d) * RPD + lane / LPR;
      const int c = lane % LPR;
      int col = fs0 + (((c >> 1) ^ slot_swizzle<SLOTS>(r & 31)) * 16) + (c & 1) * 8;
      col = col < F ? col : fs0;
      unsigned long long cb = (unsigned long long)((const char*)a.input + (long long)col * 2);
      asm volatile("" : "+v"(cb));
      cbase[d] = (const char*)cb;
      hr_off[d] = T::BITS_BYTES + 4 * r;
    }
    const int* const cols_base = a.panel_cols + (long long)ks0 * kStageK;
    auto issue_meta = [&](int s, int ms) {
      const int sc = s < ngroups ? s : ngroups - 1;
      const unsigned dst = meta0 + (unsigned)ms * T::META_BYTES;
      int ml = lane;
      asm volatile("" : "+v"(ml));
      if (wave < T::NBITS_DMA) {
        const char* src = (const char*)(a.panel_bits + (long long)(ks0 + sc * KS) * (T::WAVES * kWave)) + wave * 1024 + ml * 16;
        if (a.meta_nt) dma_b128_nt(src, dst + wave * 1024); else dma_b128(src, dst + wave * 1024);
      } else if (wave == T::NBITS_DMA) {
        const int* src = cols_base + (long long)sc * (KS * kStageK) + ml;
        if (a.meta_nt) dma_b32_nt(src, dst + T::BITS_BYTES); else dma_b32(src, dst + T::BITS_BYTES);
      }
    };
    auto issue_rows = [&](int ms, int ds) {
      const unsigned mslot = meta0 + (unsigned)ms * T::META_BYTES;
      const unsigned dst = data0 + (unsigned)ds * STAGE_BYTES + (unsigned)dma0 * 1024u;
      unsigned hrow[DPW];
#pragma unroll
      for (int d = 0; d < DPW; ++d) hrow[d] = lds_read_b32(mslot + hr_off[d]);
      wait_lgkmcnt0();
#pragma unroll
// ... 169 lines not shown
      };
      if (meta_wave) wait_steps(std::integral_constant<int, T::VM_PER_STEP>{});
      else wait_steps(std::integral_constant<int, T::VM_PER_STEP_PLAIN>{});
      if (!(VOLTRIX_PANEL_DIAG & 4))
        __builtin_amdgcn_s_barrier();
      __builtin_amdgcn_sched_barrier(0);

      if (t + D - 1 < ngroups) {
        issue_rows(ms_r, ds_r);
        if (!(VOLTRIX_PANEL_DIAG & 16)) issue_meta(t + 2 * D - 2, ms_m);
      }

      const unsigned mt = meta0 + (unsigned)ms_t * T::META_BYTES;
      const unsigned dt = data0 + (unsigned)ds_t * STAGE_BYTES + rd_off;
      ds_t = ds_t + 1 == D ? 0 : ds_t + 1;
      ds_r = ds_r + 1 == D ? 0 : ds_r + 1;
      ms_t = ms_t + 1 == MS ? 0 : ms_t + 1;
      ms_r = ms_r + 1 == MS ? 0 : ms_r + 1;
      ms_m = ms_m + 1 == MS ? 0 : ms_m + 1;
#pragma unroll
      for (int k = 0; k < KS; ++k) {
        if (t * KS + k < nks) {
          const unsigned aw = lds_read_b32(mt + 256 * (k * T::WAVES + wave) + 4 * lane);
          unsigned taddr[SLOTS];
          taddr[0] = dt + k * T::KSTEP_BYTES;
#pragma unroll
          for (int b = 0; (1 << b) < SLOTS; ++b)
#pragma unroll
            for (int s = (1 << b); s < (2 << b) && s < SLOTS; ++s) taddr[s] = taddr[s - (1 << b)] + tr_delta[b];
          uint2_t blo[SLOTS], bhi[SLOTS];
#pragma unroll
          for (int s = 0; s < SLOTS; ++s) {
            if (VOLTRIX_PANEL_DIAG & 8) {
              blo[s] = uint2_t{taddr[s], 1u};
              bhi[s] = uint2_t{taddr[s], 2u};
              continue;
            }
            blo[s] = lds_read_tr16_b64<0>(taddr[s]);
            bhi[s] = lds_read_tr16_b64<4 * ROW_BYTES>(taddr[s]);
          }
          wait_lgkmcnt0();
#pragma unroll
          for (int j = 0; j < RB; ++j) {
            const half8_t afrag = adjacency_to_half8_x2(aw, 4 * j);
#pragma unroll
            for (int s = 0; s < SLOTS; ++s) {
              const uint4_t bq = {blo[s][0], blo[s][1], bhi[s][0], bhi[s][1]};
              if (VOLTRIX_PANEL_DIAG & 1) {
                asm volatile("" ::"v"(afrag), "v"(bq));
                continue;
              }
              if constexpr (T::BF16)
                acc[j][s] = __builtin_amdgcn_mfma_f32_16x16x32_bf16(__builtin_bit_cast(bf16x8_t, afrag),
                                                                    __builtin_bit_cast(bf16x8_t, bq), acc[j][s], 0, 0, 0);
              else
                acc[j][s] = __builtin_amdgcn_mfma_f32_16x16x32_f16(afrag, __builtin_bit_cast(half8_t, bq), acc[j][s], 0,
                                                                   0, 0);
            }
          }
        }
      }
    }
    }
    wait_vmcnt<0>();
  }

  const float oscale = kAScaleInv * (a.out_scale ? *a.out_scale : 1.0f);
  const int ocol0 = fs0 + (lane & 15);
  if (slot >= 0) {
    float* const tile = a.partials + (long long)slot * T::PANEL_ROWS * F;
    const int trow0 = wave * (RB * 16) + 4 * (lane >> 4);
#pragma unroll
    for (int j = 0; j < RB; ++j)
#pragma unroll
      for (int s = 0; s < SLOTS; ++s)
#pragma unroll
        for (int i = 0; i < 4; ++i) {
          const int col = ocol0 + 16 * s;
          if (col < F) tile[(long long)(trow0 + 16 * j + i) * F + col] = acc[j][s][i] * oscale;
        }
    return;
  }
  const int prow0 = panel * T::PANEL_ROWS + wave * (RB * 16) + 4 * (lane >> 4);
  if (a.accumulate == 2) {
#pragma unroll
    for (int j = 0; j < RB; ++j) {
#pragma unroll
      for (int s = 0; s < SLOTS; ++s) {
#pragma unroll
        for (int i = 0; i < 4; ++i) {
          const int row = prow0 + 16 * j + i, col = ocol0 + 16 * s;
          if (col < F && row < a.num_nodes) unsafeAtomicAdd(a.output + ((long long)row * F + col), acc[j][s][i] * oscale);
        }
      }
    }
    return;
  }
#pragma unroll
  for (int j = 0; j < RB; ++j) {
    float prev[SLOTS][4];
#pragma unroll
    for (int s = 0; s < SLOTS; ++s) {
#pragma unroll
      for (int i = 0; i < 4; ++i) {
        const int row = prow0 + 16 * j + i, col = ocol0 + 16 * s;
        prev[s][i] = (a.accumulate && col < F && row < a.num_nodes) ? a.output[(long long)row * F + col] : 0.0f;
      }
    }
#pragma unroll
    for (int s = 0; s < SLOTS; ++s) {
#pragma unroll
      for (int i = 0; i < 4; ++i) {
        const int row = prow0 + 16 * j + i, col = ocol0 + 16 * s;
        if (col < F && row < a.num_nodes) a.output[(long long)row * F + col] = prev[s][i] + acc[j][s][i] * oscale;
      }
    }
  }
}

static __global__ __launch_bounds__(256) void combine_panel_partials_kernel(const int* __restrict__ cuts,
                                                                            const float* __restrict__ partials,
                                                                            float* __restrict__ output, int num_nodes, int F,
                                                                            int panel_rows, int accumulate) {
  const int4_t cut = *reinterpret_cast<const int4_t*>(cuts + 4 * (long long)blockIdx.x);
  const int panel = cut[0], first = cut[1], pieces = cut[2];
  const int f4 = F / 4;
  const long long tile = (long long)panel_rows * F;
  for (int e = threadIdx.x; e < 16 * f4; e += 256) {
    const int r = blockIdx.y * 16 + e / f4, c = 4 * (e % f4);
    const long long row = (long long)panel * panel_rows + r;
    if (row >= num_nodes) continue;
    const float* src = partials + (long long)first * tile + (long long)r * F + c;
    float4_t sum = *reinterpret_cast<const float4_t*>(src);
    for (int j = 1; j < pieces; ++j) sum += *reinterpret_cast<const float4_t*>(src + j * tile);
    float4_t* dst = reinterpret_cast<float4_t*>(output + row * F + c);
    *dst = accumulate ? *dst + sum : sum;
  }
}

inline int launch_combine_panel_partials(const int* cuts, int num_cuts, const float* partials, float* output, int num_nodes,
                                         int embedding_dim, int panel_rows, int accumulate, hipStream_t stream) {
  if (num_cuts < 0 || num_nodes < 0 || embedding_dim < 0 || panel_rows < 16 || panel_rows % 16 != 0) return kErrBadShape;
  if (num_cuts == 0 || num_nodes == 0 || embedding_dim == 0) return kOk;
  if (embedding_dim % 4 != 0 || cuts == nullptr || partials == nullptr || output == nullptr) return kErrBadShape;
  hipLaunchKernelGGL(combine_panel_partials_kernel, dim3((unsigned)num_cuts, (unsigned)(panel_rows / 16)), dim3(256), 0, stream,
                     cuts, partials, output, num_nodes, embedding_dim, panel_rows, accumulate);
  return hipGetLastError() == hipSuccess ? kOk : kErrLaunch;
}

template <class T>
inline int launch_spmm_panel(const int* panel_ptr, const int* panel_cols, const uint32_t* panel_bits,
                             const int* panel_order, int num_nodes, int embedding_dim, const void* input, float* output,
                             int accumulate, const float* out_scale, hipStream_t stream, int slab_first = 0,
                             int slab_count = 0 ,
                             long long input_rows = 0 ,
                             int slab_policy = kSlabAuto, const int* xcd_ptr = nullptr ,
                             int max_panels_per_xcd = 0 ,
                             const int* parts = nullptr , int num_parts = 0,
                             float* partials = nullptr) {
  if (num_nodes < 0 || embedding_dim < 0 || accumulate < 0 || accumulate > 2) return kErrBadShape;
  if (parts != nullptr && num_parts < 1) return kErrBadShape;
  if (num_nodes == 0 || embedding_dim == 0) return kOk;
  if (embedding_dim % 8 != 0 || ((uintptr_t)input & 15)) return kErrBadShape;
  PanelArgs<T> a;
  a.panel_ptr = panel_ptr;
  a.panel_cols = panel_cols;
  a.panel_bits = panel_bits;
  a.panel_order = panel_order;
  a.input = static_cast<const typename PanelArgs<T>::in_t*>(input);
  a.output = output;
  a.out_scale = out_scale;
  a.num_nodes = num_nodes;
  a.num_panels = (num_nodes + T::PANEL_ROWS - 1) / T::PANEL_ROWS;
  a.parts = parts;
  a.partials = partials;
  if (parts != nullptr) a.num_panels = num_parts;
  a.panels_per_xcd = (a.num_panels + kNumXcd - 1) / kNumXcd;
  a.xcd_ptr = nullptr;
  if (xcd_ptr != nullptr) {
    if (max_panels_per_xcd < 1 || max_panels_per_xcd > a.num_panels) return kErrBadShape;
    a.xcd_ptr = xcd_ptr;
    a.panels_per_xcd = max_panels_per_xcd;
  }
  a.F = embedding_dim;
  a.accumulate = accumulate;
  const int total_slabs = (embedding_dim + T::FS - 1) / T::FS;
  if (slab_first < 0 || slab_count < 0 || slab_first + slab_count > total_slabs) return kErrBadShape;
  if (const int group = slab_count == 0 ? slab_launch_group(total_slabs, T::ROW_BYTES,
                                                            input_rows > 0 ? input_rows : (long long)num_nodes, slab_policy)
                                        : 0) {
    for (int s = 0; s < total_slabs; s += group) {
      const int rc = launch_spmm_panel<T>(panel_ptr, panel_cols, panel_bits, panel_order, num_nodes, embedding_dim, input,
                                          output, accumulate, out_scale, stream, s,
                                          total_slabs - s < group ? total_slabs - s : group, input_rows, slab_policy, xcd_ptr,
                                          max_panels_per_xcd, parts, num_parts, partials);
      if (rc != kOk) return rc;
    }
    return kOk;
  }
  const int slabs = slab_count > 0 ? slab_count : total_slabs;
  a.slab_first = slab_count > 0 ? slab_first : 0;
  a.meta_nt = total_slabs == 1;
  const int lds_rc = ensure_dynamic_lds(reinterpret_cast<const void*>(&spmm_panel_kernel<T>), T::BLOCK_LDS);
  if (lds_rc != kOk) return lds_rc;
  hipLaunchKernelGGL(spmm_panel_kernel<T>, dim3((unsigned)(a.panels_per_xcd * kNumXcd), (unsigned)slabs),
                     dim3(T::THREADS), T::BLOCK_LDS, stream, a);
  return hipGetLastError() == hipSuccess ? kOk : kErrLaunch;
}

}
```

### voltrix-spmm_amd/voltrix/jit_kernels/spmm.py

```python
import contextlib
import contextvars
import ctypes
import os
import warnings
from typing import Callable, NamedTuple

import torch

from ..jit.compiler import hash_to_hex
from ..jit.template import map_ctype
from ..project import TUNE_SPACE_FLAG
from ..schedule import balanced_xcd_windows, default_max_stages, stream_tables, unit_table
from .tuner import jit_tuner

_TUNE_SPACE_OVERRIDE = contextvars.ContextVar("voltrix_tune_space", default=None)


def tune_space_mode() -> str:
    return _TUNE_SPACE_OVERRIDE.get() or os.getenv(TUNE_SPACE_FLAG, "default")


@contextlib.contextmanager
def tune_space(mode: str):
    token = _TUNE_SPACE_OVERRIDE.set(mode)
# ... 272 lines not shown
        ("cuts_p", torch.int32),
        ("num_cuts_p", int),
        ("partials_p", torch.float32),
        ("combine_now", int),
        ("row_map", torch.int32),
        ("has_row_map", int),
        ("values", dtype),
        ("input_rows", int),
        ("slab_policy", int),
        ("s_units", torch.int32),
        ("s_runs", torch.int32),
        ("s_run_ptr", torch.int32),
        ("s_max_runs", int),
        ("cuts_s", torch.int32),
        ("num_cuts_s", int),
        ("partials_s", torch.float32),
        ("stream", torch.cuda.Stream),
    )


def _pair_max_stages(blk_offsets: torch.Tensor, num_nodes: int) -> int:
    return max(8, int(PAIR_UNIT_FACTOR * default_max_stages(blk_offsets, num_nodes) / 1.5))


def handle_unit_table(blk_offsets: torch.Tensor, hspa_packed: torch.Tensor, num_nodes: int, pairs: bool = False,
                      xcd_ptr: torch.Tensor = None):
    def build():
        ranges = xcd_ptr if xcd_ptr is not None else balanced_xcd_windows(blk_offsets, num_nodes)
        return unit_table(blk_offsets, num_nodes, _pair_max_stages(blk_offsets, num_nodes) if pairs else None, xcd_ptr=ranges)

    key = (blk_offsets.data_ptr(), num_nodes, xcd_ptr.data_ptr() if xcd_ptr is not None else 0)
    return _cached_on(hspa_packed, "_voltrix_unit_table_pairs" if pairs else "_voltrix_unit_table", key, build)


def handle_stream_table(blk_offsets: torch.Tensor, hspa_packed: torch.Tensor, hind: torch.Tensor, num_nodes: int):
    return _cached_on(hspa_packed, "_voltrix_stream_table", (blk_offsets.data_ptr(), num_nodes),
                      lambda: stream_tables(blk_offsets, hspa_packed, hind, num_nodes))


def graph_bucket_keys(blk_offsets: torch.Tensor, num_nodes: int, keys: dict):
    import math

    num_windows = (num_nodes + 15) // 16
    if num_windows == 0:
        return None

    def bucket():
        nblk = (blk_offsets[1:num_windows + 1] - blk_offsets[:num_windows]).float()
        sample = nblk[:: max(1, num_windows // (1 << 20))]
        q = torch.quantile(sample, torch.tensor([0.25, 0.5, 0.75], device=nblk.device))
        stats = torch.cat([q, nblk.mean()[None], nblk.std(unbiased=False)[None]]).tolist()

        def half_octave(v):
            return int(round(2 * math.log2(max(v, 1.0))))

        return {"log2_rows": int(round(math.log2(max(num_nodes, 1)))),
                "log2_mean_blocks_x2": half_octave(stats[3]),
                "quartiles_x2": [half_octave(v) for v in stats[:3]],
                "cv_x4": int(round(4 * stats[4] / max(stats[3], 1e-9)))}

    out = {k: v for k, v in keys.items() if k not in ("feature_hash", "device")}
    try:
        out["arch"] = torch.cuda.get_device_properties(blk_offsets.device).gcnArchName.split(":")[0]
    except (AttributeError, RuntimeError):
        out["arch"] = keys.get("device", "unknown")
    out["graph_bucket"] = str(_cached_on(blk_offsets, "_voltrix_bucket", (blk_offsets.data_ptr(), num_nodes), bucket))
    if isinstance(out.get("embedding_dim"), int) and out["embedding_dim"] > 128:
        return [out, dict(out, embedding_dim="wide")]
    return out


_UNIT_SCALE = {}


def unit_scale(device) -> torch.Tensor:
    key = (device.type, device.index if device.index is not None else torch.cuda.current_device())
    if key not in _UNIT_SCALE:
        _UNIT_SCALE[key] = torch.tensor([1.0, 0.0], dtype=torch.float32, device=device)
    return _UNIT_SCALE[key]


class PendingCombine:

    def __init__(self, table, partials, output, num_nodes, embedding_dim, accumulate, row_map=None):
        self.table, self.partials, self.output, self.row_map = table, partials, output, row_map
        self.num_nodes, self.embedding_dim, self.accumulate = num_nodes, embedding_dim, accumulate

    def run(self, stream=None):
        from .. import capi

        stream = torch.cuda.current_stream().cuda_stream if stream is None else stream
        rc = capi.launch_combine_partials(self.table, self.partials.data_ptr(), self.output.data_ptr(), self.num_nodes,
                                          self.embedding_dim, self.accumulate, stream,
                                          self.row_map.data_ptr() if self.row_map is not None else 0)
        capi.check(rc, "voltrix_launch_combine_partials")


def _raw_stream(device) -> int:
    try:
        return torch._C._cuda_getCurrentRawStream(device.index if device.index is not None else torch.cuda.current_device())
    except AttributeError:
        return torch.cuda.current_stream(device).cuda_stream


class _TableSchedule(NamedTuple):
    fields: tuple
    partials: str
    handle_table: Callable
    range_table: Callable
    combine_rows: bool

    def launch_args(self, table, embedding_dim, device):
        out = {arg: getattr(table, attr) for arg, attr in self.fields}
        out[self.partials] = torch.empty(max(1, table.num_slots) * 16 * embedding_dim, dtype=torch.float32, device=device)
        return out


_UNIT_FIELDS = ("units", "unit_ptr", "max_units_per_xcd", "cuts", "num_cuts")
TABLE_SCHEDULES = {
    SCHED_UNITS: _TableSchedule(
        tuple(zip(_UNIT_FIELDS, _UNIT_FIELDS)), "partials",
        lambda blk, hspa, hind, n, xcd_ptr: handle_unit_table(blk, hspa, n, xcd_ptr=xcd_ptr),
        lambda blk, hspa, hind, n, full: unit_table(blk, n), combine_rows=True),
    SCHED_PAIRS: _TableSchedule(
        tuple((f + "_p", f) for f in _UNIT_FIELDS), "partials_p",
        lambda blk, hspa, hind, n, xcd_ptr: handle_unit_table(blk, hspa, n, pairs=True, xcd_ptr=xcd_ptr),
        lambda blk, hspa, hind, n, full: unit_table(blk, n, _pair_max_stages(blk, n)), combine_rows=True),
    SCHED_STREAM: _TableSchedule(
        (("s_units", "units"), ("s_runs", "runs"), ("s_run_ptr", "run_ptr"), ("s_max_runs", "max_runs_per_xcd"), ("cuts_s", "cuts"),
         ("num_cuts_s", "num_cuts")), "partials_s",
        lambda blk, hspa, hind, n, xcd_ptr: handle_stream_table(blk, hspa, hind, n),
        lambda blk, hspa, hind, n, full: stream_tables(blk, hspa, hind, n, cut_stages=full.cut_stages), combine_rows=False),
}
_ORDER_ARGS = {1: "win_order_a", 2: "win_order_b", 3: "win_order_c"}


def _pack(arg_defs, named):
    names = [name for name, _ in arg_defs]
    assert named.keys() == set(names), f"missing {set(names) - named.keys()}, unknown {named.keys() - set(names)}"
    return tuple(named[name] for name in names)


_NOT_KEPT = frozenset(("input", "output", "out_scale", "values", "hspa_packed") + tuple(s.partials for s in TABLE_SCHEDULES.values()))


def plan_keepalive(named) -> tuple:
    return tuple(value for name, value in named.items() if name not in _NOT_KEPT and isinstance(value, torch.Tensor))


class _LaunchPlan:
    __slots__ = ("fn", "cargs", "generation", "operand_index", "partials_index", "partials_floats", "combine_table", "combine_args",
                 "device", "keepalive")
    PATCHED = ("input", "output", "out_scale", "values", "stream")

    def launch(self, input, output, out_scale, values, defer_combine):
        i_input, i_output, i_scale, i_values, i_stream = self.operand_index
        cargs = list(self.cargs)
        cargs[i_input] = ctypes.c_void_p(input.data_ptr())
        cargs[i_output] = ctypes.c_void_p(output.data_ptr())
        cargs[i_scale] = ctypes.c_void_p(out_scale.data_ptr())
        cargs[i_values] = ctypes.c_void_p((values if values is not None else input).data_ptr())
        partials = None
        if self.partials_index is not None:
            partials = torch.empty(self.partials_floats, dtype=torch.float32, device=input.device)
            cargs[self.partials_index] = ctypes.c_void_p(partials.data_ptr())
        cargs[i_stream] = ctypes.c_void_p(_raw_stream(self.device))
        rc = ctypes.c_int(-1)
        self.fn(*cargs, ctypes.byref(rc))
        assert rc.value == 0, f"spmm_kernel failed with return code {rc.value}"
        if self.combine_table is not None:
            pending = PendingCombine(self.combine_table, partials, output, *self.combine_args)
            if defer_combine:
                return pending
        return None


def spmm_kernel(blk_offsets, hspa_packed, hind, num_nodes, num_edges, embedding_dim, input, output, out_scale=None,
                atomic_out=False, beside_panel=False, defer_combine=False, row_map=None, values=None, xcd_ptr=None):
    from ..utils import KernelTimer

    plan_key = (blk_offsets.data_ptr(), hind.data_ptr(), num_nodes, embedding_dim, input.dtype, input.shape[0], bool(atomic_out),
                bool(beside_panel), bool(defer_combine), row_map.data_ptr() if row_map is not None else 0,
                values.data_ptr() if values is not None else 0, xcd_ptr.data_ptr() if xcd_ptr is not None else 0,
                getattr(hspa_packed, "hash_tag", None), tune_space_mode(), SLAB_POLICY)
    plans = getattr(hspa_packed, "_voltrix_plans", None)
    plan = plans.get(plan_key) if plans is not None else None
    if plan is not None and plan.generation == jit_tuner.generation and KernelTimer.active is None:
        assert input.is_contiguous() and output.is_contiguous() and input.shape[1] == embedding_dim
        assert output.shape[0] == num_nodes and output.shape[1] == embedding_dim and output.dtype == torch.float32
        return plan.launch(input, output, out_scale if out_scale is not None else unit_scale(input.device), values, defer_combine)

    assert blk_offsets.is_cuda and blk_offsets.dtype == torch.int32
    assert hspa_packed.is_cuda and hspa_packed.dtype == torch.uint32
    assert hind.is_cuda and hind.dtype == torch.int32
    assert input.is_cuda and input.dtype in (torch.float, torch.float16, torch.bfloat16) and input.is_contiguous()
    assert output.is_cuda and output.dtype == torch.float and output.is_contiguous()
    assert input.dim() == 2 and input.shape[1] == embedding_dim
    assert output.shape[0] == num_nodes and output.shape[1] == embedding_dim
    elem_bytes = input.element_size()
    assert embedding_dim % (16 // elem_bytes) == 0, "embedding_dim must keep rows 16-byte aligned (voltrix.spmm pads)"
    if out_scale is None:
        out_scale = unit_scale(input.device)
    assert out_scale.is_cuda and out_scale.dtype == torch.float32 and out_scale.numel() >= 1
    if row_map is not None:
        assert row_map.is_cuda and row_map.dtype == torch.int32 and row_map.numel() == 16 * ((num_nodes + 15) // 16)

    if values is not None:
        assert values.is_cuda and values.dtype == input.dtype and elem_bytes == 2 and values.is_contiguous()
        assert values.numel() * 4 == hspa_packed.numel() * 128, "value plane: 128 values per TC block"
    short_windows = hspa_packed.numel() // 4 <= STREAM_MAX_BLOCKS_PER_WINDOW * ((num_nodes + 15) // 16)
    space = tile_space(embedding_dim, elem_bytes, input.dtype == torch.bfloat16,
                       TWO_LEVEL_LDS_BUDGET if beside_panel else None, weighted=values is not None,
                       stream_ok=not atomic_out and row_map is None and (short_windows or tune_space_mode() == "stream"),
                       shallow_ok=short_windows)
    keys = {
        "feature_hash": feature_hash(hspa_packed),
        "embedding_dim": embedding_dim,
        "dtype": str(input.dtype),
        "device": torch.cuda.get_device_name(input.device),
        "two_level": bool(beside_panel),
        "weighted": values is not None,
    }
    if row_map is not None:
        keys["row_map"] = True
    chosen = jit_tuner.tuned_point("spmm_kernel", keys).get("SCHED") if jit_tuner.is_tuned("spmm_kernel", keys) else None
    tables = {sched: desc.handle_table(blk_offsets, hspa_packed, hind, num_nodes, xcd_ptr) for sched, desc in TABLE_SCHEDULES.items()
              if (chosen == sched if chosen is not None else any(p["SCHED"] == sched for p in space))}
    needs_orders = chosen is None or chosen in ORDER_CHUNKS

    def orders(blk, n):
        return {arg: window_order(blk, hspa_packed, n, sched) if needs_orders else blk for sched, arg in _ORDER_ARGS.items()}

    arg_defs = arg_defs_for(input.dtype)
    named = dict(blk_offsets=blk_offsets, hspa_packed=hspa_packed, hind=hind, num_nodes=num_nodes, num_edges=num_edges,
                 embedding_dim=embedding_dim, input=input, output=output, **orders(blk_offsets, num_nodes), out_scale=out_scale,
                 atomic_out=int(bool(atomic_out)), combine_now=int(not defer_combine),
                 row_map=row_map if row_map is not None else blk_offsets, has_row_map=int(row_map is not None),
                 values=values if values is not None else input, input_rows=int(input.shape[0]), slab_policy=int(SLAB_POLICY),
                 stream=torch.cuda.current_stream())
    types = dict(arg_defs)
    for sched, desc in TABLE_SCHEDULES.items():
        if sched in tables:
            named.update(desc.launch_args(tables[sched], embedding_dim, input.device))
        else:
            named.update({arg: 0 if types[arg] is int else blk_offsets for arg, _ in desc.fields}, **{desc.partials: out_scale})
    args = _pack(arg_defs, named)
    tune_named = named
    if len(space) > 1 and chosen is None and (atomic_out or defer_combine):
        tune_named = dict(named, output=torch.zeros_like(output) if atomic_out else output, combine_now=1)
    tune_args = _pack(arg_defs, tune_named)

    def sample_args():
        num_windows = (num_nodes + 15) // 16
        ranges = sample_ranges(num_windows, int(blk_offsets[num_windows]))
        if len(ranges) == 1 and ranges[0] == (0, num_windows):
            return [tune_args], 1.0
        out_full = tune_named["output"]
        launches, covered = [], 0
        for w0, w1 in ranges:
            sub = blk_offsets[w0:w1 + 1]
            n_sub = min(num_nodes, 16 * w1) - 16 * w0
            covered += w1 - w0
            a = dict(tune_named, blk_offsets=sub, num_nodes=n_sub, **orders(sub, n_sub),
                     output=out_full if row_map is not None else out_full[16 * w0:16 * w0 + n_sub],
                     combine_now=1)
            for sched, table in tables.items():
                desc = TABLE_SCHEDULES[sched]
                a.update(desc.launch_args(desc.range_table(sub, hspa_packed, hind, n_sub, table), embedding_dim, input.device))
            if row_map is not None:
                a["row_map"] = row_map[16 * w0:16 * w1]
            launches.append(_pack(arg_defs, a))
        return launches, covered / max(1, num_windows)

    staged = tune_space_mode() != "full"

    def tune(use_store=True):
        return jit_tuner.compile_and_tune(
            name="spmm_kernel", keys=keys, space=space, includes=includes, arg_defs=arg_defs, template=template, args=tune_args,
            kernel_tag="spmm", bench=sweep_bench, bucket_keys=lambda: graph_bucket_keys(blk_offsets, num_nodes, keys),
            use_store=use_store, sample_args=sample_args, stages=sweep_stages if staged else None, budget_s=sweep_budget_s)

    runtime = tune()
    rc = runtime(*args)
    signature = jit_tuner._signature("spmm_kernel", keys)
    if rc != 0 and signature in jit_tuner.unvalidated:
        jit_tuner.forget("spmm_kernel", keys)
        runtime = tune(use_store=False)
        rc = runtime(*args)
    jit_tuner.unvalidated.discard(signature)
    assert rc == 0, f"spmm_kernel failed with return code {rc}"
    sched = jit_tuner.tuned_point("spmm_kernel", keys).get("SCHED")
    table = tables.get(sched)
    combine_args = None
    if defer_combine and table is not None and table.num_cuts > 0:
        combine_args = (num_nodes, embedding_dim) + ((bool(atomic_out), row_map) if TABLE_SCHEDULES[sched].combine_rows else (False, None))
    fn, kernel_args = runtime.launcher()
    names = [name for name, _ in kernel_args]
    plan = _LaunchPlan()
    plan.fn, plan.generation, plan.device = fn, jit_tuner.generation, input.device
    plan.cargs = [map_ctype(named[name]) for name in names]
    plan.operand_index = tuple(names.index(name) for name in _LaunchPlan.PATCHED)
    plan.keepalive = plan_keepalive(named) + tuple(tables.values()) + ((xcd_ptr,) if xcd_ptr is not None else ())
    has_partials = table is not None and table.num_slots > 0
    plan.partials_index = names.index(TABLE_SCHEDULES[sched].partials) if has_partials else None
    plan.partials_floats = table.num_slots * 16 * embedding_dim if has_partials else 0
    plan.combine_table, plan.combine_args = (table, combine_args) if combine_args is not None else (None, None)
    try:
# ... 9 lines not shown
```

### voltrix-spmm_amd/voltrix/spmm/spmm.py

```python
import math
import os

import torch

from ..jit_kernels import (
    csr_fused_preprocess_kernel,
    hmat_gen_kernel,
    hmat_packed_swizzle_kernel,
    preprocess_kernel,
    spmm_kernel,
)
from .. import capi, hybrid, sidecar
from ..project import CSR_PATH_FLAG, FP32_MODE_FLAG, PREPROCESS_FLAG
from ..utils import aligned16, padded_last_dim, piece_width

BLK_H = 16
BLK_W = 8


def csr_preprocess(indptr: torch.Tensor, indices: torch.Tensor, num_nodes: int, num_cols: int = None):
    assert indptr.is_cpu and indptr.dtype == torch.int32
    assert indices.is_cpu and indices.dtype == torch.int32
    assert indptr.numel() == num_nodes + 1

    if preprocess_mode()[0] != "reference":
        return csr_preprocess_device(indptr.contiguous().cuda(), indices.contiguous().cuda(), num_nodes, num_cols)

    num_edges = indices.numel()
    num_row_windows = math.ceil(num_nodes / BLK_H)
    edge_to_column = torch.zeros(num_edges, dtype=torch.int32)
    edge_to_row = torch.zeros(num_edges, dtype=torch.int32)
    block_partition = torch.zeros(num_row_windows, dtype=torch.int32)
    pointer1 = torch.zeros(block_partition.numel() + 1, dtype=torch.int32)
    preprocess_kernel(edge_list=indices.contiguous(), node_pointer=indptr.contiguous(),
                      block_partition=block_partition, edge_to_column=edge_to_column, edge_to_row=edge_to_row,
                      pointer1=pointer1)

    total_blocks = int(pointer1[-1].item())
    hspa = torch.empty(total_blocks * BLK_H * BLK_W, dtype=torch.float32, device="cuda")
    hind = torch.empty(total_blocks * BLK_W, dtype=torch.int32, device="cuda")
    hspa_packed = torch.empty(hspa.numel() // 32, dtype=torch.uint32, device="cuda")

    indptr_d, indices_d = indptr.cuda(), indices.cuda()
    edge_to_column, edge_to_row = edge_to_column.cuda(), edge_to_row.cuda()
    block_partition, pointer1 = block_partition.cuda(), pointer1.cuda()
    hmat_gen_kernel(node_pointer=indptr_d, edge_list=indices_d, block_partition=block_partition,
                    edge_to_column=edge_to_column, edge_to_row=edge_to_row, pointer1=pointer1, hspa=hspa, hind=hind)
    hmat_packed_swizzle_kernel(block_partition=block_partition, pointer1=pointer1, hspa=hspa, hspa_packed=hspa_packed)
    sidecar.register(hspa_packed, None)
    return pointer1, hspa_packed, hind


def preprocess_mode():
    mode, _, path = os.getenv(PREPROCESS_FLAG, "fused").partition(":")
    assert mode in ("fused", "reference") and (path or "auto") in ("auto", "sort", "bitmap", "mixed"), \
        f"{PREPROCESS_FLAG}={os.getenv(PREPROCESS_FLAG)}"
    return mode, (path or None)


def csr_preprocess_device(indptr: torch.Tensor, indices: torch.Tensor, num_nodes: int, num_cols: int = None):
    assert indptr.is_cuda and indptr.dtype == torch.int32 and indices.is_cuda and indices.dtype == torch.int32
    assert indptr.numel() == num_nodes + 1
    indptr, indices = indptr.contiguous(), indices.contiguous()
    path = preprocess_mode()[1]
    pointer1, hspa_packed, hind, _ = csr_fused_preprocess_kernel(indptr, indices, num_nodes, num_cols, path=path)
    mode = hybrid.hybrid_mode()
    big_enough = (indices.numel() >= hybrid.AUTO_MIN_EDGES and num_nodes >= hybrid.AUTO_MIN_ROWS
                  and indices.numel() >= hybrid.AUTO_MIN_MEAN_DEGREE * max(1, num_nodes))
    two = None
    if mode == "on" or (mode in ("auto", "tune") and big_enough):
        two = _build_two_level(indptr, indices, num_nodes, num_cols)
    sidecar.register(hspa_packed, two)
    if two is None:
        _attach_csr_side_car(hspa_packed, indptr, indices, num_nodes, num_cols)
    return pointer1, hspa_packed, hind


CSR_MAX_BLOCKS_PER_WINDOW = 48
CSR_MAX_EDGES = 1 << 26


def csr_path_mode() -> str:
    v = os.getenv(CSR_PATH_FLAG, "auto")
    return "off" if v in ("0", "off") else ("on" if v in ("1", "on") else "auto")


def _attach_csr_side_car(hspa_packed, indptr, indices, num_nodes, num_cols) -> None:
    if csr_path_mode() == "off" or num_nodes == 0 or indices.numel() == 0 or indices.numel() > CSR_MAX_EDGES:
        return
    windows = (num_nodes + 15) // 16
    if hspa_packed.numel() // 4 > CSR_MAX_BLOCKS_PER_WINDOW * windows:
        return
    cols = num_nodes if num_cols is None else int(num_cols)
    deg = (indptr[1:] - indptr[:-1]).long()
    rows = torch.repeat_interleave(torch.arange(num_nodes, device=indptr.device, dtype=torch.int64), deg)
# ... 161 lines not shown
        return "csr"
    from ..jit_kernels.spmm import tune_space_mode

    if (feat.dtype == torch.float32 and os.getenv(FP32_MODE_FLAG, "auto") == "fp16") or tune_space_mode() in ("none", "stream"):
        return "block"
    key = (int(feat.shape[1]), str(feat.dtype))
    if key in csr.choice:
        return csr.choice[key]
    if torch.cuda.is_current_stream_capturing():
        return "block"
    from ..jit_kernels import jit_tuner
    from ..jit_kernels.spmm import feature_hash

    tagged = isinstance(getattr(hspa_packed, "hash_tag", None), str)
    signature = ("spmm_csr_path", f"{{'device': '{torch.cuda.get_device_name(hspa_packed.device)}', 'dtype': '{key[1]}', "
                                  f"'embedding_dim': {key[0]}, 'feature_hash': '{feature_hash(hspa_packed) if tagged else ''}'}}")
    if tagged:
        stored = jit_tuner._load_store().get(f"{signature[0]}|{signature[1]}")
        if stored in ("csr", "block"):
            csr.choice[key] = stored
            return stored
    times = {}
    _CSR_DEPTH[0] += 1
    try:
        for name, fn in (("block", lambda: spmm(blk_offsets, hspa_packed, hind, num_nodes, num_edges, feat)),
                         ("csr", lambda: _spmm_csr(csr, feat))):
            fn()
            fn()
            start, end = torch.cuda.Event(enable_timing=True), torch.cuda.Event(enable_timing=True)
            start.record()
            for _ in range(3):
                fn()
            end.record()
            end.synchronize()
            times[name] = start.elapsed_time(end) / 3
    finally:
        _CSR_DEPTH[0] -= 1
    best = "csr" if times["csr"] < (1.0 - CSR_MIN_GAIN) * times["block"] else "block"
    if os.getenv("VOLTRIX_PRINT_AUTO_TUNE") or os.getenv("VOLTRIX_JIT_DEBUG"):
        print(f"voltrix.spmm path for width {key[0]} {key[1]}: {times} -> {best}")
    csr.choice[key] = best
    if tagged:
        jit_tuner._save_choice(signature, best)
    return best


def _choose_format(hspa_packed, key, window, two_level) -> str:
    from ..jit_kernels import jit_tuner
    from ..jit_kernels.spmm import feature_hash

    signature = ("spmm_format", f"{{'device': '{torch.cuda.get_device_name(hspa_packed.device)}', 'dtype': '{key[1]}', "
                                f"'embedding_dim': {key[0]}, 'feature_hash': '{feature_hash(hspa_packed)}'}}")
    stored = jit_tuner._load_store().get(f"{signature[0]}|{signature[1]}")
    if stored in ("two-level", "window") and hasattr(hspa_packed, "hash_tag"):
        return stored
    times = {}
    for name, fn in (("window", window), ("two-level", two_level)):
        fn()
        start, end = torch.cuda.Event(enable_timing=True), torch.cuda.Event(enable_timing=True)
        start.record()
        for _ in range(3):
            fn()
        end.record()
        end.synchronize()
        times[name] = start.elapsed_time(end)
    best = min(times, key=times.get)
    if os.getenv("VOLTRIX_PRINT_AUTO_TUNE") or os.getenv("VOLTRIX_JIT_DEBUG"):
        print(f"voltrix.spmm format for width {key[0]} {key[1]}: {times} -> {best}")
    if hasattr(hspa_packed, "hash_tag"):
        jit_tuner._save_choice(signature, best)
    return best


def _run_two_level(two, operand, output, out_scale, tag_source=None, concurrent=True):
    if two.fused is not None and hybrid.fused_enabled():
        hybrid.launch_fused(two.plan, two.fused, operand, output, out_scale=out_scale)
        return
    resid = two.hspa_packed
    if getattr(resid, "hash_tag", None) is None:
        tag = two.hash_tag or getattr(tag_source, "hash_tag", None)
        if isinstance(tag, str):
            resid.hash_tag = tag + "/residual"

    def run_window(atomic):
        return spmm_kernel(two.blk_offsets, resid, two.hind, num_nodes=two.num_nodes,
                           num_edges=two.plan.num_resid_edges, embedding_dim=operand.shape[1], input=operand,
                           output=output, out_scale=out_scale, atomic_out=atomic,
                           beside_panel=two.plan.num_ksteps > 0, defer_combine=True, xcd_ptr=two.window_xcd_ptr)

    hybrid.run_two_level(two.plan, operand, output, run_window, out_scale=out_scale, concurrent=concurrent)


def spmm_two_level(handle: "hybrid.TwoLevelHandle", feat: torch.Tensor, concurrent: bool = True):
    assert isinstance(handle, hybrid.TwoLevelHandle)
    num_feats = feat.shape[1]
    operand, out_scale, padded, exact = _operand(feat)
    assert not (exact and handle.plan.num_ksteps > 0), \
        "the panel kernel takes a 16-bit operand (unset VOLTRIX_FP32_MODE=exact or use csr_preprocess)"
    output = torch.empty((handle.num_nodes, padded), dtype=torch.float32, device=feat.device)
    _run_two_level(handle, operand, output, out_scale, concurrent=concurrent)
    return output if padded == num_feats else output[:, :num_feats].contiguous()
```

Measured before the change: 21500.

## Add ticket-based output writes for concurrent two-level panel and window kernels

Adds a ticket mode (accumulate==3 / atomic_out==2) where the panel kernel and the residual window kernel, running concurrently, coordinate through per-row tickets. This lets them write output directly instead of using atomic accumulation or a separate zero-fill and combine ordering. It only applies when the tuner already holds a tuned point whose tile is in the AOT set. The cost is extra ticket memory and a more complex synchronisation protocol. The handshake can go wrong and needs embedding_dim no larger than FS for the panel path.

```diff
diff --git a/include/voltrix_capi.h b/include/voltrix_capi.h
--- a/include/voltrix_capi.h
+++ b/include/voltrix_capi.h
@@ -124,6 +124,30 @@
 void voltrix_launch_combine_panel_partials(void* cuts, int num_cuts, void* partials, void* output, int num_nodes,
                                            int embedding_dim, int panel_rows, int accumulate, void* stream, int* return_code);
 
+void voltrix_launch_spmm_f16_sched_ticket(void* blk_offsets, void* hspa_packed, void* hind, int num_nodes, int num_edges,
+                                          int embedding_dim, void* input, void* output, int fs, int depth, int waves,
+                                          void* out_scale, void* units, void* unit_ptr, int max_units_per_xcd, void* partials,
+                                          int units_per_wave, void* tickets, void* stream, int* return_code);
+void voltrix_launch_spmm_bf16_sched_ticket(void* blk_offsets, void* hspa_packed, void* hind, int num_nodes, int num_edges,
+                                           int embedding_dim, void* input, void* output, int fs, int depth, int waves,
+                                           void* out_scale, void* units, void* unit_ptr, int max_units_per_xcd, void* partials,
+                                           int units_per_wave, void* tickets, void* stream, int* return_code);
+void voltrix_launch_combine_partials_ticket(void* cuts, int num_cuts, void* partials, void* output, int num_nodes,
+                                            int embedding_dim, void* tickets, void* stream, int* return_code);
+void voltrix_launch_spmm_panel_ticket_f16(void* panel_ptr, void* panel_cols, void* panel_bits, void* panel_order, void* parts,
+                                          int num_parts, void* xcd_ptr, int max_per_xcd, void* partials, void* tickets,
+                                          int num_nodes, int embedding_dim, void* input, int64_t input_rows, void* output, int fs,
+                                          int depth, int waves, int row_blocks, int ksteps, int slab_policy, void* out_scale,
+                                          void* stream, int* return_code);
+void voltrix_launch_spmm_panel_ticket_bf16(void* panel_ptr, void* panel_cols, void* panel_bits, void* panel_order, void* parts,
+                                           int num_parts, void* xcd_ptr, int max_per_xcd, void* partials, void* tickets,
+                                           int num_nodes, int embedding_dim, void* input, int64_t input_rows, void* output, int fs,
+                                           int depth, int waves, int row_blocks, int ksteps, int slab_policy, void* out_scale,
+                                           void* stream, int* return_code);
+void voltrix_launch_combine_panel_partials_ticket(void* cuts, int num_cuts, void* partials, void* output, int num_nodes,
+                                                  int embedding_dim, int panel_rows, void* tickets, void* stream,
+                                                  int* return_code);
+
 void voltrix_launch_xcd_ranges_of_work(void* work, int num_items, int align, void* xcd_ptr, void* stream, int* return_code);
 void voltrix_launch_xcd_ranges_of_windows(void* blk_offsets, int num_nodes, int align, void* xcd_ptr, void* stream,
                                           int* return_code);
diff --git a/voltrix-spmm_amd/csrc/capi_common.hpp b/voltrix-spmm_amd/csrc/capi_common.hpp
--- a/voltrix-spmm_amd/csrc/capi_common.hpp
+++ b/voltrix-spmm_amd/csrc/capi_common.hpp
@@ -54,13 +54,14 @@
 inline int launch_if_ok(const int* blk_offsets, const uint32_t* hspa_packed, const int* hind, int num_nodes,
                         int embedding_dim, const In* input, float* output, hipStream_t stream, const int* order,
                         const float* out_scale, int atomic_out, const int* units, const int* unit_ptr,
-                        int max_units_per_xcd, float* partials, const int* row_map, int units_per_wave) {
+                        int max_units_per_xcd, float* partials, const int* row_map, int units_per_wave,
+                        int* tickets) {
   if constexpr (tile_ok<FS, D, W, EB>()) {
     return voltrix::launch_spmm_tc16<voltrix::SpmmTile<FS, D, W, EB, BF16>>(blk_offsets, hspa_packed, hind, num_nodes,
                                                                        embedding_dim, input, output, stream, order,
                                                                        out_scale, atomic_out, units, unit_ptr,
                                                                        max_units_per_xcd, partials, row_map, nullptr,
-                                                                       units_per_wave);
+                                                                       units_per_wave, 0, 0, 0, voltrix::kSlabAuto, tickets);
   } else {
     return voltrix::kErrBadConfig;
   }
@@ -72,10 +73,10 @@
                          hipStream_t stream, const int* order, const float* out_scale = nullptr,
                          int atomic_out = 0, const int* units = nullptr, const int* unit_ptr = nullptr,
                          int max_units_per_xcd = 0, float* partials = nullptr, const int* row_map = nullptr,
-                         int units_per_wave = 1) {
+                         int units_per_wave = 1, int* tickets = nullptr ) {
 #define X(FS, D, W)                                  \
   if (fs == FS && depth == D && waves == W)          \
-    return launch_if_ok<FS, D, W, EB, In, BF16>(blk_offsets, hspa_packed, hind, num_nodes, embedding_dim, input, output, stream, order, out_scale, atomic_out, units, unit_ptr, max_units_per_xcd, partials, row_map, units_per_wave);
+    return launch_if_ok<FS, D, W, EB, In, BF16>(blk_offsets, hspa_packed, hind, num_nodes, embedding_dim, input, output, stream, order, out_scale, atomic_out, units, unit_ptr, max_units_per_xcd, partials, row_map, units_per_wave, tickets);
   VOLTRIX_TILE_SPACE(X)
 #undef X
   return voltrix::kErrBadConfig;
diff --git a/voltrix-spmm_amd/csrc/capi_spmm_bf16.hip b/voltrix-spmm_amd/csrc/capi_spmm_bf16.hip
--- a/voltrix-spmm_amd/csrc/capi_spmm_bf16.hip
+++ b/voltrix-spmm_amd/csrc/capi_spmm_bf16.hip
@@ -32,6 +32,19 @@
                                             units_per_wave);
 }
 
+void voltrix_launch_spmm_bf16_sched_ticket(void* blk_offsets, void* hspa_packed, void* hind, int num_nodes, int num_edges,
+                                           int embedding_dim, void* input, void* output, int fs, int depth, int waves,
+                                           void* out_scale, void* units, void* unit_ptr, int max_units_per_xcd, void* partials,
+                                           int units_per_wave, void* tickets, void* stream, int* return_code) {
+  (void)num_edges;
+  *return_code = dispatch_spmm<2, voltrix::bfloat16_bits, true>(
+      fs, depth, waves, static_cast<const int*>(blk_offsets), static_cast<const uint32_t*>(hspa_packed),
+      static_cast<const int*>(hind), num_nodes, embedding_dim, static_cast<const voltrix::bfloat16_bits*>(input),
+      static_cast<float*>(output), static_cast<hipStream_t>(stream), nullptr, static_cast<const float*>(out_scale),
+      2, static_cast<const int*>(units), static_cast<const int*>(unit_ptr), max_units_per_xcd,
+      static_cast<float*>(partials), nullptr, units_per_wave, static_cast<int*>(tickets));
+}
+
 void voltrix_launch_spmm_bf16(void* blk_offsets, void* hspa_packed, void* hind, int num_nodes, int num_edges,
                               int embedding_dim, void* input, void* output, void* stream, int* return_code) {
   const TileId t = default_tile(embedding_dim, true);
diff --git a/voltrix-spmm_amd/csrc/capi_spmm_f16.hip b/voltrix-spmm_amd/csrc/capi_spmm_f16.hip
--- a/voltrix-spmm_amd/csrc/capi_spmm_f16.hip
+++ b/voltrix-spmm_amd/csrc/capi_spmm_f16.hip
@@ -39,6 +39,30 @@
   *return_code = voltrix::combine_partials(static_cast<const int*>(cuts), num_cuts, static_cast<const float*>(partials),
                                            static_cast<float*>(output), num_nodes, embedding_dim, accumulate,
                                            static_cast<hipStream_t>(stream), static_cast<const int*>(row_map));
+}
+
+void voltrix_launch_spmm_f16_sched_ticket(void* blk_offsets, void* hspa_packed, void* hind, int num_nodes, int num_edges,
+                                          int embedding_dim, void* input, void* output, int fs, int depth, int waves,
+                                          void* out_scale, void* units, void* unit_ptr, int max_units_per_xcd, void* partials,
+                                          int units_per_wave, void* tickets, void* stream, int* return_code) {
+  (void)num_edges;
+  *return_code = dispatch_spmm<2, _Float16>(fs, depth, waves, static_cast<const int*>(blk_offsets),
+                                            static_cast<const uint32_t*>(hspa_packed), static_cast<const int*>(hind),
+                                            num_nodes, embedding_dim, static_cast<const _Float16*>(input),
+                                            static_cast<float*>(output), static_cast<hipStream_t>(stream), nullptr,
+                                            static_cast<const float*>(out_scale), 2,
+                                            static_cast<const int*>(units), static_cast<const int*>(unit_ptr),
+                                            max_units_per_xcd, static_cast<float*>(partials), nullptr, units_per_wave,
+                                            static_cast<int*>(tickets));
+}
+
+void voltrix_launch_combine_partials_ticket(void* cuts, int num_cuts, void* partials, void* output, int num_nodes,
+                                            int embedding_dim, void* tickets, void* stream, int* return_code) {
+  *return_code = tickets == nullptr
+                     ? voltrix::kErrBadShape
+                     : voltrix::combine_partials(static_cast<const int*>(cuts), num_cuts, static_cast<const float*>(partials),
+                                                 static_cast<float*>(output), num_nodes, embedding_dim, 1,
+                                                 static_cast<hipStream_t>(stream), nullptr, static_cast<int*>(tickets));
 }
 
 void voltrix_launch_spmm_f16(void* blk_offsets, void* hspa_packed, void* hind, int num_nodes, int num_edges,
diff --git a/voltrix-spmm_amd/csrc/capi_spmm_panel.hip b/voltrix-spmm_amd/csrc/capi_spmm_panel.hip
--- a/voltrix-spmm_amd/csrc/capi_spmm_panel.hip
+++ b/voltrix-spmm_amd/csrc/capi_spmm_panel.hip
@@ -22,19 +22,21 @@
              const uint32_t* panel_bits, const int* panel_order, int num_nodes, int embedding_dim, const void* input,
              float* output, int accumulate, const float* out_scale, hipStream_t stream, int64_t input_rows,
              int slab_policy, const int* xcd_ptr, int max_panels_per_xcd, const int* parts = nullptr, int num_parts = 0,
-             float* partials = nullptr) {
+             float* partials = nullptr, int* tickets = nullptr) {
 #define X(FS, D, W, RB, KS)                                                                                          \
   if (fs == FS && depth == D && waves == W && rb == RB && ks == KS)                                                  \
     return voltrix::launch_spmm_panel<voltrix::PanelTile<FS, D, W, RB, KS, BF16>>(                                   \
         panel_ptr, panel_cols, panel_bits, panel_order, num_nodes, embedding_dim, input, output, accumulate, out_scale, \
-        stream, 0, 0, input_rows, slab_policy, xcd_ptr, max_panels_per_xcd, parts, num_parts, partials);
+        stream, 0, 0, input_rows, slab_policy, xcd_ptr, max_panels_per_xcd, parts, num_parts, partials, \
+        tickets);
   VOLTRIX_PANEL_SPACE(X)
 #undef X
 #define X(FS, D, W, RB)                                                                                              \
   if (fs == FS && depth == D && waves == W && rb == RB && ks == kPipelined)                                           \
     return voltrix::launch_spmm_panel<voltrix::PanelTile<FS, D, W, RB, 1, BF16, true>>(                               \
         panel_ptr, panel_cols, panel_bits, panel_order, num_nodes, embedding_dim, input, output, accumulate, out_scale, \
-        stream, 0, 0, input_rows, slab_policy, xcd_ptr, max_panels_per_xcd, parts, num_parts, partials);
+        stream, 0, 0, input_rows, slab_policy, xcd_ptr, max_panels_per_xcd, parts, num_parts, partials, \
+        tickets);
   VOLTRIX_PANEL_PIPE_SPACE(X)
 #undef X
   return voltrix::kErrBadConfig;
@@ -106,6 +108,33 @@
                                                         static_cast<hipStream_t>(stream));
 }
 
+#define VOLTRIX_PANEL_TICKET(NAME, BF16)                                                                                      \
+  void NAME(void* panel_ptr, void* panel_cols, void* panel_bits, void* panel_order, void* parts, int num_parts, void* xcd_ptr, \
+            int max_per_xcd, void* partials, void* tickets, int num_nodes, int embedding_dim, void* input, int64_t input_rows, \
+            void* output, int fs, int depth, int waves, int row_blocks, int ksteps, int slab_policy, void* out_scale,         \
+            void* stream, int* return_code) {                                                                                 \
+    *return_code = dispatch<BF16>(fs, depth, waves, row_blocks, ksteps, static_cast<const int*>(panel_ptr),                   \
+                                  static_cast<const int*>(panel_cols), static_cast<const uint32_t*>(panel_bits),              \
+                                  parts != nullptr ? nullptr : static_cast<const int*>(panel_order), num_nodes, embedding_dim, \
+                                  input, static_cast<float*>(output), 3, static_cast<const float*>(out_scale), \
+                                  static_cast<hipStream_t>(stream), input_rows, slab_policy, static_cast<const int*>(xcd_ptr), \
+                                  max_per_xcd, static_cast<const int*>(parts), num_parts, static_cast<float*>(partials),      \
+                                  static_cast<int*>(tickets));                                                                \
+  }
+VOLTRIX_PANEL_TICKET(voltrix_launch_spmm_panel_ticket_f16, false)
+VOLTRIX_PANEL_TICKET(voltrix_launch_spmm_panel_ticket_bf16, true)
+#undef VOLTRIX_PANEL_TICKET
+
+void voltrix_launch_combine_panel_partials_ticket(void* cuts, int num_cuts, void* partials, void* output, int num_nodes,
+                                                  int embedding_dim, int panel_rows, void* tickets, void* stream,
+                                                  int* return_code) {
+  *return_code = tickets == nullptr ? voltrix::kErrBadShape
+                                    : voltrix::launch_combine_panel_partials(
+                                          static_cast<const int*>(cuts), num_cuts, static_cast<const float*>(partials),
+                                          static_cast<float*>(output), num_nodes, embedding_dim, panel_rows, 1,
+                                          static_cast<hipStream_t>(stream), static_cast<int*>(tickets));
+}
+
 void voltrix_launch_panel_order(void* panel_ptr, int num_panels, int group, void* xcd_ptr, void* order_out, void* stream,
                                 int* return_code) {
   *return_code = voltrix::panel_order(static_cast<const int*>(panel_ptr), num_panels, group, static_cast<int*>(order_out),
diff --git a/voltrix-spmm_amd/voltrix/capi.py b/voltrix-spmm_amd/voltrix/capi.py
--- a/voltrix-spmm_amd/voltrix/capi.py
+++ b/voltrix-spmm_amd/voltrix/capi.py
@@ -38,6 +38,12 @@
     "voltrix_launch_spmm_panel_parts_f16": (None, [_P, _P, _P, _P, _I, _P, _I, _P, _I, _I, _P, _L, _P, _I, _I, _I, _I, _I, _I, _I, _P, _P, _RC_P]),
     "voltrix_launch_spmm_panel_parts_bf16": (None, [_P, _P, _P, _P, _I, _P, _I, _P, _I, _I, _P, _L, _P, _I, _I, _I, _I, _I, _I, _I, _P, _P, _RC_P]),
     "voltrix_launch_combine_panel_partials": (None, [_P, _I, _P, _P, _I, _I, _I, _I, _P, _RC_P]),
+    "voltrix_launch_spmm_f16_sched_ticket": (None, [_P, _P, _P, _I, _I, _I, _P, _P, _I, _I, _I, _P, _P, _P, _I, _P, _I, _P, _P, _RC_P]),
+    "voltrix_launch_spmm_bf16_sched_ticket": (None, [_P, _P, _P, _I, _I, _I, _P, _P, _I, _I, _I, _P, _P, _P, _I, _P, _I, _P, _P, _RC_P]),
+    "voltrix_launch_combine_partials_ticket": (None, [_P, _I, _P, _P, _I, _I, _P, _P, _RC_P]),
+    "voltrix_launch_spmm_panel_ticket_f16": (None, [_P, _P, _P, _P, _P, _I, _P, _I, _P, _P, _I, _I, _P, _L, _P, _I, _I, _I, _I, _I, _I, _P, _P, _RC_P]),
+    "voltrix_launch_spmm_panel_ticket_bf16": (None, [_P, _P, _P, _P, _P, _I, _P, _I, _P, _P, _I, _I, _P, _L, _P, _I, _I, _I, _I, _I, _I, _P, _P, _RC_P]),
+    "voltrix_launch_combine_panel_partials_ticket": (None, [_P, _I, _P, _P, _I, _I, _I, _P, _P, _RC_P]),
     "voltrix_launch_xcd_ranges_of_work": (None, [_P, _I, _I, _P, _P, _RC_P]),
     "voltrix_launch_xcd_ranges_of_windows": (None, [_P, _I, _I, _P, _P, _RC_P]),
     "voltrix_launch_xcd_ranges_of_panels": (None, [_P, _P, _I, _I, _I, _P, _P, _P, _RC_P]),
@@ -266,9 +272,14 @@
 @_timed("spmm")
 def launch_spmm_sched(blk_offsets, hspa_packed, hind, num_nodes, num_edges, embedding_dim, input_ptr, output_ptr, tile,
                       stream, window_order=0, out_scale=0, atomic_out=False, bf16=False, table=None, partials=0,
-                      row_map=0, units_per_wave=1) -> int:
+                      row_map=0, units_per_wave=1, tickets=0) -> int:
     units, unit_ptr, max_units = (table.units.data_ptr(), table.unit_ptr.data_ptr(), table.max_units_per_xcd) if table is not None \
         else (None, None, 0)
+    if tickets:
+        assert not window_order and not row_map, "the ticket join takes neither a window order nor a row map"
+        return _call("voltrix_launch_spmm_bf16_sched_ticket" if bf16 else "voltrix_launch_spmm_f16_sched_ticket", blk_offsets,
+                     hspa_packed, hind, num_nodes, num_edges, embedding_dim, input_ptr, output_ptr, tile[0], tile[1], tile[2],
+                     out_scale, units, unit_ptr, max_units, partials, int(units_per_wave), tickets, stream)
     return _call("voltrix_launch_spmm_bf16_sched" if bf16 else "voltrix_launch_spmm_f16_sched", blk_offsets, hspa_packed, hind,
                  num_nodes, num_edges, embedding_dim, input_ptr, output_ptr, tile[0], tile[1], tile[2], window_order, out_scale,
                  int(atomic_out), units, unit_ptr, max_units, partials, row_map, int(units_per_wave), stream)
@@ -276,7 +287,11 @@
 
 @_timed("combine_partials")
 def launch_combine_partials(table, partials_ptr, output_ptr, num_nodes, embedding_dim, accumulate, stream,
-                            row_map=0) -> int:
+                            row_map=0, tickets=0) -> int:
+    if tickets:
+        assert not row_map
+        return _call("voltrix_launch_combine_partials_ticket", table.cuts.data_ptr(), table.num_cuts, partials_ptr, output_ptr,
+                     num_nodes, embedding_dim, tickets, stream)
     return _call("voltrix_launch_combine_partials", table.cuts.data_ptr(), table.num_cuts, partials_ptr, output_ptr, num_nodes,
                  embedding_dim, int(accumulate), row_map, stream)
 
@@ -397,8 +412,17 @@
 
 @_timed("spmm_panel")
 def launch_spmm_panel(plan, input_ptr, output_ptr, embedding_dim, accumulate, bf16, tile, out_scale, stream,
-                      input_rows: int = 0, slab_policy: int = SLAB_AUTO, partials_ptr: int = 0) -> int:
+                      input_rows: int = 0, slab_policy: int = SLAB_AUTO, partials_ptr: int = 0, tickets: int = 0) -> int:
     panel = (plan.panel_ptr.data_ptr(), plan.panel_cols.data_ptr(), plan.panel_bits.data_ptr())
+    if int(accumulate) == 3:
+        parts, xcd_ptr = getattr(plan, "parts", None), getattr(plan, "xcd_ptr", None)
+        if parts is not None:
+            table = (None, parts.parts.data_ptr(), parts.num_parts, parts.xcd_ptr.data_ptr(), parts.max_parts_per_xcd)
+        else:
+            table = (_opt(plan.panel_order), None, 0, _opt(xcd_ptr), plan.max_panels_per_xcd if xcd_ptr is not None else 0)
+        return _call("voltrix_launch_spmm_panel_ticket_bf16" if bf16 else "voltrix_launch_spmm_panel_ticket_f16", *panel, *table,
+                     partials_ptr, tickets, plan.num_nodes, embedding_dim, input_ptr, input_rows, output_ptr, tile[0], tile[1],
+                     plan.waves, plan.row_blocks, tile[2], slab_policy, out_scale, stream)
     launch = (plan.num_nodes, embedding_dim, input_ptr, input_rows, output_ptr, int(accumulate), tile[0], tile[1], plan.waves,
               plan.row_blocks, tile[2], slab_policy, out_scale, stream)
     parts = getattr(plan, "parts", None)
@@ -411,7 +435,10 @@
 
 
 def launch_combine_panel_partials(parts, partials_ptr, output_ptr, num_nodes, embedding_dim, panel_rows, accumulate,
-                                  stream) -> int:
+                                  stream, tickets: int = 0) -> int:
+    if tickets:
+        return _call("voltrix_launch_combine_panel_partials_ticket", parts.cuts.data_ptr(), parts.num_cuts, partials_ptr,
+                     output_ptr, num_nodes, embedding_dim, panel_rows, tickets, stream)
     return _call("voltrix_launch_combine_panel_partials", parts.cuts.data_ptr(), parts.num_cuts, partials_ptr, output_ptr, num_nodes,
                  embedding_dim, panel_rows, int(accumulate), stream)
 
diff --git a/voltrix-spmm_amd/voltrix/hybrid.py b/voltrix-spmm_amd/voltrix/hybrid.py
--- a/voltrix-spmm_amd/voltrix/hybrid.py
+++ b/voltrix-spmm_amd/voltrix/hybrid.py
@@ -433,8 +433,38 @@
     return _SIDE_STREAMS[key]
 
 
+JOIN_MODES = ("atomic", "ticket", "add")
+TICKET_HEADER = 4
+DEFAULT_JOIN = "ticket"
+LAST_JOIN = {"mode": None, "tickets": None}
+
+
+def join_mode(plan: PanelPlan, operand: torch.Tensor, concurrent: bool = True, row_map=None, window_fs: int = None,
+              panel_fs: int = None, binary: bool = True, forced: str = None) -> str:
+    want = forced if forced is not None else os.getenv("VOLTRIX_TWO_LEVEL_JOIN", DEFAULT_JOIN)
+    assert want in JOIN_MODES, f"VOLTRIX_TWO_LEVEL_JOIN={want!r}: one of {JOIN_MODES}"
+    if not concurrent or want == "add":
+        return "add"
+    if want != "ticket":
+        return "atomic"
+    f = operand.shape[1]
+    eligible = (binary and row_map is None and operand.dtype in (torch.float16, torch.bfloat16)
+                and window_fs is not None and panel_fs is not None and window_fs == panel_fs and f <= window_fs and f % 8 == 0)
+    return "ticket" if eligible else "atomic"
+
+
+def new_tickets(num_nodes: int, device) -> torch.Tensor:
+    words = TICKET_HEADER + (num_nodes + 15) // 16
+    return torch.zeros((words + 3) // 4 * 4, dtype=torch.int32, device=device)
+
+
+def join_error_word() -> int:
+    tickets = LAST_JOIN["tickets"]
+    return 0 if tickets is None else int(tickets[0].item())
+
+
 def run_two_level(plan: PanelPlan, operand: torch.Tensor, output: torch.Tensor, run_window, out_scale=None,
-                  tile=None, concurrent: bool = True) -> None:
+                  tile=None, concurrent: bool = True, window_fs: int = None) -> None:
     def finish(pending):
         if pending is not None:
             pending.run()
@@ -442,7 +472,9 @@
     if plan.num_ksteps == 0:
         finish(run_window(False))
         return
-    if not concurrent:
+    panel_tile = tile or default_panel_tile(operand.shape[1], plan.waves, plan.row_blocks)
+    mode = join_mode(plan, operand, concurrent, window_fs=window_fs, panel_fs=panel_tile[0] if panel_tile else None)
+    if mode == "add":
         finish(run_window(False))
         launch_panel(plan, operand, output, accumulate=1, out_scale=out_scale, tile=tile)
         return
@@ -450,16 +482,22 @@
 
     main = torch.cuda.current_stream()
     side = side_stream(operand.device)
-    with timed_launch("zero_fill", main):
-        output.zero_()
+    tickets = None
+    if mode == "ticket":
+        with timed_launch("zero_fill", main):
+            tickets = new_tickets(plan.num_nodes, operand.device)
+    else:
+        with timed_launch("zero_fill", main):
+            output.zero_()
+    LAST_JOIN["mode"], LAST_JOIN["tickets"] = mode, tickets
     fork = torch.cuda.Event()
     fork.record(main)
     side.wait_event(fork)
-    pending_panel = launch_panel(plan, operand, output, accumulate=2, out_scale=out_scale, tile=tile,
-                                 stream=side.cuda_stream, defer_combine=True)
+    pending_panel = launch_panel(plan, operand, output, accumulate=3 if tickets is not None else 2, out_scale=out_scale,
+                                 tile=tile, stream=side.cuda_stream, defer_combine=True, tickets=tickets)
     join = torch.cuda.Event()
     join.record(side)
-    pending = run_window(True)
+    pending = run_window(True, tickets) if tickets is not None else run_window(True)
     main.wait_event(join)
     finish(pending)
     finish(pending_panel)
@@ -467,8 +505,9 @@
 
 class PendingPanelCombine:
 
-    def __init__(self, plan, partials, output, num_feats, accumulate):
+    def __init__(self, plan, partials, output, num_feats, accumulate, tickets=None):
         self.plan, self.partials, self.output, self.num_feats, self.accumulate = plan, partials, output, num_feats, accumulate
+        self.tickets = tickets
 
     def run(self, raw_stream: int = None):
         from .utils import timed_launch
@@ -477,13 +516,14 @@
         with timed_launch("combine_panel_partials", current) if raw_stream is None else contextlib.nullcontext():
             rc = capi.launch_combine_panel_partials(self.plan.parts, self.partials.data_ptr(), self.output.data_ptr(),
                                                     self.plan.num_nodes, self.num_feats, self.plan.panel_rows,
-                                                    self.accumulate, current.cuda_stream if raw_stream is None else raw_stream)
+                                                    self.accumulate, current.cuda_stream if raw_stream is None else raw_stream,
+                                                    tickets=self.tickets.data_ptr() if self.tickets is not None else 0)
         capi.check(rc, "voltrix_launch_combine_panel_partials")
         self.partials = None
 
 
 def launch_panel(plan: PanelPlan, feat: torch.Tensor, output: torch.Tensor, accumulate, out_scale=None,
-                 tile=None, stream=None, slab_policy: int = None, defer_combine: bool = False):
+                 tile=None, stream=None, slab_policy: int = None, defer_combine: bool = False, tickets: torch.Tensor = None):
     assert feat.is_cuda and feat.is_contiguous() and feat.dtype in (torch.float16, torch.bfloat16)
     assert output.is_cuda and output.is_contiguous() and output.dtype == torch.float32
     f = feat.shape[1]
@@ -502,11 +542,12 @@
     rc = capi.launch_spmm_panel(plan, feat.data_ptr(), output.data_ptr(), f, int(accumulate),
                                 feat.dtype == torch.bfloat16, tile, out_scale.data_ptr() if out_scale is not None else 0,
                                 stream, input_rows=feat.shape[0], slab_policy=slab_policy,
-                                partials_ptr=partials.data_ptr() if partials is not None else 0)
+                                partials_ptr=partials.data_ptr() if partials is not None else 0,
+                                tickets=tickets.data_ptr() if tickets is not None else 0)
     capi.check(rc, "voltrix_launch_spmm_panel")
     if partials is None:
         return None
-    pending = PendingPanelCombine(plan, partials, output, f, 1 if int(accumulate) else 0)
+    pending = PendingPanelCombine(plan, partials, output, f, 1 if int(accumulate) else 0, tickets=tickets)
     if defer_combine:
         return pending
     pending.run(None if stream == torch.cuda.current_stream().cuda_stream else stream)
diff --git a/voltrix-spmm_amd/voltrix/include/voltrix/spmm_kernels.hpp b/voltrix-spmm_amd/voltrix/include/voltrix/spmm_kernels.hpp
--- a/voltrix-spmm_amd/voltrix/include/voltrix/spmm_kernels.hpp
+++ b/voltrix-spmm_amd/voltrix/include/voltrix/spmm_kernels.hpp
@@ -191,6 +191,82 @@
   return v;
 }
 
+template <int I, int N, class Fn>
+__device__ __forceinline__ void static_for(Fn&& fn) {
+  if constexpr (I < N) {
+    fn(std::integral_constant<int, I>{});
+    static_for<I + 1, N>(fn);
+  }
+}
+
+constexpr int kTicketHeader = 4;
+constexpr int kTicketPollBound = 1 << 16;
+
+__device__ __forceinline__ int ticket_claim(int* tickets, int block, int lane) {
+  int old = 0;
+  if (lane == 0)
+    old = __hip_atomic_fetch_add(tickets + kTicketHeader + block, 1, __ATOMIC_RELAXED, __HIP_MEMORY_SCOPE_AGENT);
+  return __builtin_amdgcn_readfirstlane(old);
+}
+
+__device__ __forceinline__ void ticket_publish(int* tickets, int block, int lane) {
+  asm volatile("s_waitcnt vmcnt(0)" ::: "memory");
+  if (lane == 0) __hip_atomic_fetch_add(tickets + kTicketHeader + block, 1, __ATOMIC_RELAXED, __HIP_MEMORY_SCOPE_AGENT);
+}
+
+__device__ __forceinline__ void ticket_wait(int* tickets, int block, int lane) {
+  __builtin_amdgcn_s_setprio(0);
+  int seen = 2;
+  for (int spin = 0; spin < kTicketPollBound && seen < 3; ++spin) {
+    __builtin_amdgcn_s_sleep(8);
+    int v = 0;
+    if (lane == 0) v = __hip_atomic_load(tickets + kTicketHeader + block, __ATOMIC_RELAXED, __HIP_MEMORY_SCOPE_AGENT);
+    seen = __builtin_amdgcn_readfirstlane(v);
+  }
+  if (seen < 3 && lane == 0) __hip_atomic_fetch_or(tickets, 1, __ATOMIC_RELAXED, __HIP_MEMORY_SCOPE_AGENT);
+}
+
+template <int OFF>
+__device__ __forceinline__ void lds_write_f32_off(unsigned addr, float v) {
+  asm volatile("ds_write_b32 %0, %1 offset:%2" ::"v"(addr), "v"(v), "n"(OFF) : "memory");
+}
+template <int OFF>
+__device__ __forceinline__ float4_t lds_read_f32x4_off(unsigned addr) {
+  float4_t v;
+  asm volatile("ds_read_b128 %0, %1 offset:%2" : "=v"(v) : "v"(addr), "n"(OFF) : "memory");
+  return v;
+}
+__device__ __forceinline__ void store_f32x4_sc1(float* dst, const float4_t v) {
+  asm volatile("global_store_dwordx4 %0, %1, off sc1\n\ts_nop 1" ::"v"(dst), "v"(v) : "memory");
+}
+
+template <int FS>
+constexpr int ticket_tile_lds_bytes() { return 4 * (FS + 16) * 4; }
+
+template <int FS, class Value>
+__device__ __forceinline__ void store_tile_sc1(const Value& value, const unsigned lds, float* const output, const int row0,
+                                               const int num_nodes, const int F, const int lane) {
+  constexpr int SLOTS = FS / 16, STRIDE = FS + 16, LPR = FS / 4;
+  constexpr int NR = FS >= 64 ? FS / 64 : 1;
+  const unsigned waddr = lds + (unsigned)(((lane >> 4) * STRIDE + (lane & 15)) * 4);
+  static_for<0, 4>([&](auto jc) {
+    constexpr int J = decltype(jc)::value;
+    static_for<0, SLOTS>([&](auto sc) {
+      constexpr int S = decltype(sc)::value;
+      lds_write_f32_off<64 * S>(waddr, value(S, J));
+    });
+    static_for<0, NR>([&](auto rc) {
+      constexpr int R = decltype(rc)::value;
+      const int idx = R * 64 + lane;
+      const int g = idx / LPR < 4 ? idx / LPR : 3;
+      const float4_t v = lds_read_f32x4_off<0>(lds + (unsigned)((g * STRIDE + 4 * (idx % LPR)) * 4));
+      wait_lgkmcnt0();
+      const int row = row0 + 4 * (idx / LPR) + J, col = 4 * (idx % LPR);
+      if (idx / LPR < 4 && row < num_nodes && col < F) store_f32x4_sc1(output + ((long long)row * F + col), v);
+    });
+  });
+}
+
 template <class Tag = void>
 inline int ensure_dynamic_lds(const void* kernel, int bytes) {
   if (bytes <= 64 * 1024) return kOk;
@@ -238,15 +314,9 @@
   int slab_first;
   int meta_nt;
   int atomic_out;
+  int* tickets;
 };
 
-template <int I, int N, class Fn>
-__device__ __forceinline__ void static_for(Fn&& fn) {
-  if constexpr (I < N) {
-    fn(std::integral_constant<int, I>{});
-    static_for<I + 1, N>(fn);
-  }
-}
 
 template <class T, int NU>
 __device__ __forceinline__ void spmm_tc16_body(const SpmmArgs<T>& a) {
@@ -621,9 +691,56 @@
   }
   const float oscale = ((EB == 2 && !T::WEIGHTED) ? kAScaleInv : 1.0f) * (a.out_scale ? *a.out_scale : 1.0f);
   const int ocol0 = fs0 + (lane & 15);
+  int drawn[NU];
+#pragma unroll
+  for (int p = 0; p < NU; ++p) drawn[p] = -1;
+  if constexpr (EB == 2 && !T::WEIGHTED) {
+    if (a.atomic_out == 2) {
+      auto store_unit = [&](auto pc) {
+        constexpr int P = decltype(pc)::value;
+        const bool dead = NU > 1 && nst_u[P] == 0;
+        store_tile_sc1<FS>([&](int s, int j) { return dead ? 0.f : acc[P][s][j] * oscale; }, lds0, a.output, w[P] * kBlkH,
+                           a.num_nodes, F, lane);
+        ticket_publish(a.tickets, w[P], lane);
+      };
+      auto add_unit = [&](auto pc) {
+        constexpr int P = decltype(pc)::value;
+        const bool dead = NU > 1 && nst_u[P] == 0;
+        const int orow0 = w[P] * kBlkH + 4 * (lane >> 4);
+#pragma unroll
+        for (int s = 0; s < SLOTS; ++s) {
+          const int col = ocol0 + 16 * s;
+          if (col < F) {
+#pragma unroll
+            for (int j = 0; j < 4; ++j)
+              if (orow0 + j < a.num_nodes)
+                unsafeAtomicAdd(a.output + ((long long)(orow0 + j) * F + col), dead ? 0.f : acc[P][s][j] * oscale);
+          }
+        }
+      };
+#pragma unroll
+      for (int p = 0; p < NU; ++p)
+        if (present[p] && slot[p] < 0) drawn[p] = ticket_claim(a.tickets, w[p], lane);
+      if (drawn[0] == 0) store_unit(std::integral_constant<int, 0>{});
+      if constexpr (NU == 2) {
+        if (drawn[1] == 0) store_unit(std::integral_constant<int, 1>{});
+        if (drawn[1] >= 2) add_unit(std::integral_constant<int, 1>{});
+      }
+      if (drawn[0] >= 1) {
+        if (drawn[0] == 1) ticket_wait(a.tickets, w[0], lane);
+        add_unit(std::integral_constant<int, 0>{});
+      }
+      if constexpr (NU == 2) {
+        if (drawn[1] == 1) {
+          ticket_wait(a.tickets, w[1], lane);
+          add_unit(std::integral_constant<int, 1>{});
+        }
+      }
+    }
+  }
 #pragma unroll
   for (int p = 0; p < NU; ++p) {
-    if (!present[p]) continue;
+    if (!present[p] || drawn[p] >= 0) continue;
     const bool dead = NU > 1 && nst_u[p] == 0;
     if (slot[p] >= 0) {
       float* const tile = a.partials + (long long)slot[p] * (kBlkH * (long long)F) + (long long)(4 * (lane >> 4)) * F;
@@ -705,10 +822,17 @@
                             int units_per_wave = 1 ,
                             int slab_first = 0, int slab_count = 0 ,
                             long long input_rows = 0 ,
-                            int slab_policy = kSlabAuto) {
-  if (num_nodes < 0 || embedding_dim < 0) return kErrBadShape;
+                            int slab_policy = kSlabAuto,
+                            int* tickets = nullptr ) {
+  if (num_nodes < 0 || embedding_dim < 0 || atomic_out < 0 || atomic_out > 2) return kErrBadShape;
   if (num_nodes == 0 || embedding_dim == 0) return kOk;
   if (embedding_dim % (16 / T::EB) != 0) return kErrBadShape;
+  if (atomic_out == 2) {
+    if (T::EB != 2 || T::WEIGHTED || tickets == nullptr || row_map != nullptr || embedding_dim > T::FS || embedding_dim % 4 != 0 ||
+        ((uintptr_t)output & 15))
+      return kErrBadShape;
+    static_assert(T::EB != 2 || ticket_tile_lds_bytes<T::FS>() <= T::WAVE_LDS, "the tile transpose uses the wave's own ring");
+  }
   if (((uintptr_t)input & 15) || ((uintptr_t)hspa_packed & 15)) return kErrBadShape;
   SpmmArgs<T> a;
   a.blk_offsets = blk_offsets;
@@ -738,6 +862,7 @@
   a.window_order = window_order;
   a.out_scale = out_scale;
   a.atomic_out = atomic_out;
+  a.tickets = tickets;
   a.meta_nt = total_slabs == 1;
   a.slab_major = slab_major_order(a.num_slabs, T::FS * T::EB);
   a.units = reinterpret_cast<const int4*>(units);
@@ -777,8 +902,12 @@
                                                                      const float* __restrict__ partials,
                                                                      float* __restrict__ output, const int num_nodes,
                                                                      const int F, const int accumulate,
-                                                                     const int* __restrict__ row_map) {
+                                                                     const int* __restrict__ row_map,
+                                                                     int* __restrict__ tickets) {
   const int4 c = cuts[blockIdx.x];
+  const bool fresh = tickets != nullptr && tickets[kTicketHeader + c.x] == 0;
+  if (tickets != nullptr) __syncthreads();
+  if (fresh && threadIdx.x == 0) tickets[kTicketHeader + c.x] = 2;
   const int f4 = F / 4;
   const long long tile4 = (long long)kBlkH * f4;
   const float4* src = reinterpret_cast<const float4*>(partials) + (long long)c.y * tile4;
@@ -808,7 +937,7 @@
       sum.w += p.w;
     }
     float4* const dst = reinterpret_cast<float4*>(output + (long long)row * F) + (i % f4);
-    if (accumulate) {
+    if (accumulate && !fresh) {
       const float4 d = *dst;
       sum.x += d.x;
       sum.y += d.y;
@@ -820,12 +949,15 @@
 }
 
 inline int combine_partials(const int* cuts, int num_cuts, const float* partials, float* output, int num_nodes,
-                            int embedding_dim, int accumulate, hipStream_t stream, const int* row_map = nullptr) {
+                            int embedding_dim, int accumulate, hipStream_t stream, const int* row_map = nullptr,
+                            int* tickets = nullptr ) {
+  if (tickets != nullptr && row_map != nullptr) return kErrBadShape;
   if (num_cuts < 0 || num_nodes < 0 || embedding_dim < 0 || (embedding_dim % 4) != 0) return kErrBadShape;
   if (num_cuts == 0 || num_nodes == 0 || embedding_dim == 0) return kOk;
   if (((uintptr_t)cuts & 15) || ((uintptr_t)partials & 15) || ((uintptr_t)output & 15)) return kErrBadShape;
   hipLaunchKernelGGL(combine_partials_kernel, dim3((unsigned)num_cuts), dim3(256), 0, stream,
-                     reinterpret_cast<const int4*>(cuts), partials, output, num_nodes, embedding_dim, accumulate, row_map);
+                     reinterpret_cast<const int4*>(cuts), partials, output, num_nodes, embedding_dim, accumulate, row_map,
+                     tickets);
   return hipGetLastError() == hipSuccess ? kOk : kErrLaunch;
 }
 
diff --git a/voltrix-spmm_amd/voltrix/include/voltrix/spmm_panel_kernels.hpp b/voltrix-spmm_amd/voltrix/include/voltrix/spmm_panel_kernels.hpp
--- a/voltrix-spmm_amd/voltrix/include/voltrix/spmm_panel_kernels.hpp
+++ b/voltrix-spmm_amd/voltrix/include/voltrix/spmm_panel_kernels.hpp
@@ -44,6 +44,8 @@
   static constexpr int BLOCK_LDS = DATA_LDS + META_SLOTS * META_BYTES;
   static_assert(BLOCK_LDS <= 160 * 1024, "LDS per CU");
   static_assert(VM_PER_STEP * (DEPTH - 2) <= 63, "vmcnt is a 6-bit counter on gfx9");
+  static constexpr bool TICKET_OK = DATA_LDS / WAVES >= ticket_tile_lds_bytes<FS>() && (DATA_LDS / WAVES) % 16 == 0;
+  static_assert(TICKET_OK, "a wave's slice of the ring holds four padded rows of the tile");
 };
 
 __device__ __forceinline__ half8_t adjacency_to_half8_x2(unsigned w, int p0) {
@@ -76,6 +78,7 @@
   int meta_nt;
   int slab_first;
   int accumulate;
+  int* tickets;
 };
 
 template <class T>
@@ -411,6 +414,35 @@
     return;
   }
   const int prow0 = panel * T::PANEL_ROWS + wave * (RB * 16) + 4 * (lane >> 4);
+  if (a.accumulate == 3) {
+    if constexpr (T::TICKET_OK) {
+      __syncthreads();
+      const unsigned tlds = data0 + (unsigned)wave * (unsigned)(T::DATA_LDS / T::WAVES);
+      const int lane = (int)__builtin_amdgcn_mbcnt_hi(~0u, __builtin_amdgcn_mbcnt_lo(~0u, 0u));
+      const int prow0 = panel * T::PANEL_ROWS + wave * (RB * 16) + 4 * (lane >> 4), ocol0 = fs0 + (lane & 15);
+      static_for<0, RB>([&](auto jc) {
+        constexpr int J = decltype(jc)::value;
+        const int brow0 = panel * T::PANEL_ROWS + wave * (RB * 16) + 16 * J;
+        if (brow0 >= a.num_nodes) return;
+        const int drawn = ticket_claim(a.tickets, brow0 / 16, lane);
+        if (drawn == 0) {
+          store_tile_sc1<FS>([&](int s, int i) { return acc[J][s][i] * oscale; }, tlds, a.output, brow0, a.num_nodes, F, lane);
+          ticket_publish(a.tickets, brow0 / 16, lane);
+          return;
+        }
+        if (drawn == 1) ticket_wait(a.tickets, brow0 / 16, lane);
+#pragma unroll
+        for (int s = 0; s < SLOTS; ++s) {
+#pragma unroll
+          for (int i = 0; i < 4; ++i) {
+            const int row = prow0 + 16 * J + i, col = ocol0 + 16 * s;
+            if (col < F && row < a.num_nodes) unsafeAtomicAdd(a.output + ((long long)row * F + col), acc[J][s][i] * oscale);
+          }
+        }
+      });
+    }
+    return;
+  }
   if (a.accumulate == 2) {
 #pragma unroll
     for (int j = 0; j < RB; ++j) {
@@ -450,9 +482,14 @@
 static __global__ __launch_bounds__(256) void combine_panel_partials_kernel(const int* __restrict__ cuts,
                                                                             const float* __restrict__ partials,
                                                                             float* __restrict__ output, int num_nodes, int F,
-                                                                            int panel_rows, int accumulate) {
+                                                                            int panel_rows, int accumulate,
+                                                                            int* __restrict__ tickets) {
   const int4_t cut = *reinterpret_cast<const int4_t*>(cuts + 4 * (long long)blockIdx.x);
   const int panel = cut[0], first = cut[1], pieces = cut[2];
+  const long long block = (long long)panel * (panel_rows / 16) + blockIdx.y;
+  const bool fresh = tickets != nullptr && block * 16 < num_nodes && tickets[kTicketHeader + block] == 0;
+  if (tickets != nullptr) __syncthreads();
+  if (fresh && threadIdx.x == 0) tickets[kTicketHeader + block] = 2;
   const int f4 = F / 4;
   const long long tile = (long long)panel_rows * F;
   for (int e = threadIdx.x; e < 16 * f4; e += 256) {
@@ -463,17 +500,18 @@
     float4_t sum = *reinterpret_cast<const float4_t*>(src);
     for (int j = 1; j < pieces; ++j) sum += *reinterpret_cast<const float4_t*>(src + j * tile);
     float4_t* dst = reinterpret_cast<float4_t*>(output + row * F + c);
-    *dst = accumulate ? *dst + sum : sum;
+    *dst = (accumulate && !fresh) ? *dst + sum : sum;
   }
 }
 
 inline int launch_combine_panel_partials(const int* cuts, int num_cuts, const float* partials, float* output, int num_nodes,
-                                         int embedding_dim, int panel_rows, int accumulate, hipStream_t stream) {
+                                         int embedding_dim, int panel_rows, int accumulate, hipStream_t stream,
+                                         int* tickets = nullptr ) {
   if (num_cuts < 0 || num_nodes < 0 || embedding_dim < 0 || panel_rows < 16 || panel_rows % 16 != 0) return kErrBadShape;
   if (num_cuts == 0 || num_nodes == 0 || embedding_dim == 0) return kOk;
   if (embedding_dim % 4 != 0 || cuts == nullptr || partials == nullptr || output == nullptr) return kErrBadShape;
   hipLaunchKernelGGL(combine_panel_partials_kernel, dim3((unsigned)num_cuts, (unsigned)(panel_rows / 16)), dim3(256), 0, stream,
-                     cuts, partials, output, num_nodes, embedding_dim, panel_rows, accumulate);
+                     cuts, partials, output, num_nodes, embedding_dim, panel_rows, accumulate, tickets);
   return hipGetLastError() == hipSuccess ? kOk : kErrLaunch;
 }
 
@@ -486,8 +524,11 @@
                              int slab_policy = kSlabAuto, const int* xcd_ptr = nullptr ,
                              int max_panels_per_xcd = 0 ,
                              const int* parts = nullptr , int num_parts = 0,
-                             float* partials = nullptr) {
-  if (num_nodes < 0 || embedding_dim < 0 || accumulate < 0 || accumulate > 2) return kErrBadShape;
+                             float* partials = nullptr,
+                             int* tickets = nullptr ) {
+  if (num_nodes < 0 || embedding_dim < 0 || accumulate < 0 || accumulate > 3) return kErrBadShape;
+  if (accumulate == 3 && (tickets == nullptr || embedding_dim > T::FS || embedding_dim % 4 != 0 || ((uintptr_t)output & 15)))
+    return kErrBadShape;
   if (parts != nullptr && num_parts < 1) return kErrBadShape;
   if (num_nodes == 0 || embedding_dim == 0) return kOk;
   if (embedding_dim % 8 != 0 || ((uintptr_t)input & 15)) return kErrBadShape;
@@ -513,6 +554,7 @@
   }
   a.F = embedding_dim;
   a.accumulate = accumulate;
+  a.tickets = tickets;
   const int total_slabs = (embedding_dim + T::FS - 1) / T::FS;
   if (slab_first < 0 || slab_count < 0 || slab_first + slab_count > total_slabs) return kErrBadShape;
   if (const int group = slab_count == 0 ? slab_launch_group(total_slabs, T::ROW_BYTES,
diff --git a/voltrix-spmm_amd/voltrix/jit_kernels/spmm.py b/voltrix-spmm_amd/voltrix/jit_kernels/spmm.py
--- a/voltrix-spmm_amd/voltrix/jit_kernels/spmm.py
+++ b/voltrix-spmm_amd/voltrix/jit_kernels/spmm.py
@@ -378,9 +378,10 @@
 
 class PendingCombine:
 
-    def __init__(self, table, partials, output, num_nodes, embedding_dim, accumulate, row_map=None):
+    def __init__(self, table, partials, output, num_nodes, embedding_dim, accumulate, row_map=None, tickets=None):
         self.table, self.partials, self.output, self.row_map = table, partials, output, row_map
         self.num_nodes, self.embedding_dim, self.accumulate = num_nodes, embedding_dim, accumulate
+        self.tickets = tickets
 
     def run(self, stream=None):
         from .. import capi
@@ -388,7 +389,8 @@
         stream = torch.cuda.current_stream().cuda_stream if stream is None else stream
         rc = capi.launch_combine_partials(self.table, self.partials.data_ptr(), self.output.data_ptr(), self.num_nodes,
                                           self.embedding_dim, self.accumulate, stream,
-                                          self.row_map.data_ptr() if self.row_map is not None else 0)
+                                          self.row_map.data_ptr() if self.row_map is not None else 0,
+                                          tickets=self.tickets.data_ptr() if self.tickets is not None else 0)
         capi.check(rc, "voltrix_launch_combine_partials")
 
 
@@ -471,6 +473,72 @@
         return None
 
 
+def tuner_keys(hspa_packed, embedding_dim: int, input, beside_panel: bool, weighted: bool = False, row_map: bool = False) -> dict:
+    keys = {
+        "feature_hash": feature_hash(hspa_packed),
+        "embedding_dim": embedding_dim,
+        "dtype": str(input.dtype),
+        "device": torch.cuda.get_device_name(input.device),
+        "two_level": bool(beside_panel),
+        "weighted": weighted,
+    }
+    if row_map:
+        keys["row_map"] = True
+    return keys
+
+
+_AOT_TILES = []
+
+
+def ticket_point(hspa_packed, embedding_dim: int, input, beside_panel: bool):
+    memo_key = (embedding_dim, input.dtype, bool(beside_panel), getattr(hspa_packed, "hash_tag", None), jit_tuner.generation)
+    memo = getattr(hspa_packed, "_voltrix_ticket_point", None)
+    if memo is not None and memo[0] == memo_key:
+        return memo[1]
+    with warnings.catch_warnings():
+        warnings.simplefilter("ignore")
+        keys = tuner_keys(hspa_packed, embedding_dim, input, beside_panel)
+    if not jit_tuner.is_tuned("spmm_kernel", keys):
+        return None
+    point = jit_tuner.tuned_point("spmm_kernel", keys)
+    if not _AOT_TILES:
+        from .. import capi
+
+        _AOT_TILES.extend(capi.tiles(True))
+    ok = (point.get("SCHED") in (0, SCHED_UNITS, SCHED_PAIRS) and point.get("EB") == 2
+          and (point.get("FS"), point.get("DEPTH"), point.get("WAVES")) in _AOT_TILES)
+    point = dict(point) if ok else None
+    try:
+        hspa_packed._voltrix_ticket_point = (memo_key, point)
+    except AttributeError:
+        pass
+    return point
+
+
+def spmm_kernel_ticket(point, blk_offsets, hspa_packed, hind, num_nodes, num_edges, embedding_dim, input, output, tickets,
+                       out_scale=None, xcd_ptr=None):
+    from .. import capi
+
+    sched = point["SCHED"]
+    table = TABLE_SCHEDULES[sched].handle_table(blk_offsets, hspa_packed, hind, num_nodes, xcd_ptr) if sched in TABLE_SCHEDULES else None
+    partials = None
+    if table is not None and table.num_slots > 0:
+        partials = torch.empty(table.num_slots * 16 * embedding_dim, dtype=torch.float32, device=input.device)
+    from ..utils import timed_launch
+
+    stream = _raw_stream(input.device)
+    with timed_launch("spmm_kernel", stream):
+        rc = capi.launch_spmm_sched.__wrapped__(
+            blk_offsets.data_ptr(), hspa_packed.data_ptr(), hind.data_ptr(), num_nodes, num_edges, embedding_dim, input.data_ptr(),
+            output.data_ptr(), (point["FS"], point["DEPTH"], point["WAVES"]), stream, 0,
+            (out_scale if out_scale is not None else unit_scale(input.device)).data_ptr(), False, input.dtype == torch.bfloat16, table,
+            partials.data_ptr() if partials is not None else 0, 0, 2 if sched == SCHED_PAIRS else 1, tickets=tickets.data_ptr())
+    capi.check(rc, "voltrix_launch_spmm_sched_ticket")
+    if partials is None or table.num_cuts == 0:
+        return None
+    return PendingCombine(table, partials, output, num_nodes, embedding_dim, True, None, tickets=tickets)
+
+
 def spmm_kernel(blk_offsets, hspa_packed, hind, num_nodes, num_edges, embedding_dim, input, output, out_scale=None,
                 atomic_out=False, beside_panel=False, defer_combine=False, row_map=None, values=None, xcd_ptr=None):
     from ..utils import KernelTimer
@@ -509,16 +577,7 @@
                        TWO_LEVEL_LDS_BUDGET if beside_panel else None, weighted=values is not None,
                        stream_ok=not atomic_out and row_map is None and (short_windows or tune_space_mode() == "stream"),
                        shallow_ok=short_windows)
-    keys = {
-        "feature_hash": feature_hash(hspa_packed),
-        "embedding_dim": embedding_dim,
-        "dtype": str(input.dtype),
-        "device": torch.cuda.get_device_name(input.device),
-        "two_level": bool(beside_panel),
-        "weighted": values is not None,
-    }
-    if row_map is not None:
-        keys["row_map"] = True
+    keys = tuner_keys(hspa_packed, embedding_dim, input, beside_panel, weighted=values is not None, row_map=row_map is not None)
     chosen = jit_tuner.tuned_point("spmm_kernel", keys).get("SCHED") if jit_tuner.is_tuned("spmm_kernel", keys) else None
     tables = {sched: desc.handle_table(blk_offsets, hspa_packed, hind, num_nodes, xcd_ptr) for sched, desc in TABLE_SCHEDULES.items()
               if (chosen == sched if chosen is not None else any(p["SCHED"] == sched for p in space))}
diff --git a/voltrix-spmm_amd/voltrix/spmm/spmm.py b/voltrix-spmm_amd/voltrix/spmm/spmm.py
--- a/voltrix-spmm_amd/voltrix/spmm/spmm.py
+++ b/voltrix-spmm_amd/voltrix/spmm/spmm.py
@@ -11,6 +11,7 @@
     spmm_kernel,
 )
 from .. import capi, hybrid, sidecar
+from ..jit_kernels.spmm import spmm_kernel_ticket, ticket_point
 from ..project import CSR_PATH_FLAG, FP32_MODE_FLAG, PREPROCESS_FLAG
 from ..utils import aligned16, padded_last_dim, piece_width
 
@@ -338,13 +339,21 @@
         if isinstance(tag, str):
             resid.hash_tag = tag + "/residual"
 
-    def run_window(atomic):
+    beside = two.plan.num_ksteps > 0
+
+    point = ticket_point(resid, operand.shape[1], operand, beside) if beside and concurrent else None
+
+    def run_window(atomic, tickets=None):
+        if tickets is not None:
+            return spmm_kernel_ticket(point, two.blk_offsets, resid, two.hind, two.num_nodes, two.plan.num_resid_edges,
+                                      operand.shape[1], operand, output, tickets, out_scale=out_scale, xcd_ptr=two.window_xcd_ptr)
         return spmm_kernel(two.blk_offsets, resid, two.hind, num_nodes=two.num_nodes,
                            num_edges=two.plan.num_resid_edges, embedding_dim=operand.shape[1], input=operand,
                            output=output, out_scale=out_scale, atomic_out=atomic,
-                           beside_panel=two.plan.num_ksteps > 0, defer_combine=True, xcd_ptr=two.window_xcd_ptr)
-
-    hybrid.run_two_level(two.plan, operand, output, run_window, out_scale=out_scale, concurrent=concurrent)
+                           beside_panel=beside, defer_combine=True, xcd_ptr=two.window_xcd_ptr)
+
+    hybrid.run_two_level(two.plan, operand, output, run_window, out_scale=out_scale, concurrent=concurrent,
+                         window_fs=point["FS"] if point is not None else None)
 
 
 def spmm_two_level(handle: "hybrid.TwoLevelHandle", feat: torch.Tensor, concurrent: bool = True):
```

After: 21960, median of 6. 1.02x the previous value.
